# guxm2021/SVT_SpeechBrain

Hardware: AMD Instinct MI355X
Metric: 10s@16kHz clips/sec encoder+CTC forward, wav2vec2-base, 1/2/4/8 MI355X (higher is better)
Workload: dtype bf16; 1 GPU; wav2vec2-base audio-only AMT forward (encoder + 20-way head + frame decode), 32 x 10 s @16 kHz mono clips per GPU; global_batch=32, per_gpu_batch=32, samples_per_clip=160000, frames_per_clip=499, parallelism=clips sharded over 1 rank(s), streams=2, inputs=resident in HBM

## Files before the change

include/svt_mi355.h:

```cpp
#ifndef SVT_MI355_H
#define SVT_MI355_H

#include <stddef.h>
#include <stdint.h>

#ifdef __cplusplus
extern "C" {
#endif

#define SVT_ABI_VERSION 1
#define SVT_MAX_CONV_LAYERS 8

typedef enum {
  SVT_OK = 0,
  SVT_ERR_INVALID = -1,
  SVT_ERR_KEY = -2,
  SVT_ERR_STATE = -3,
  SVT_ERR_WORKSPACE = -4,
  SVT_ERR_HIP = -5,
  SVT_ERR_NO_DEVICE = -6
} svt_status;

typedef enum { SVT_PREC_FP32 = 0, SVT_PREC_BF16 = 1, SVT_PREC_BF16X3 = 2, SVT_PREC_FP16X3 = 3 } svt_precision;
typedef enum { SVT_NORM_GROUP = 0, SVT_NORM_LAYER = 1 } svt_feat_norm;
// ... 12 lines not shown
  int32_t feat_extract_norm;
  int32_t conv_bias;
  int32_t stable_layer_norm;
  int32_t feat_proj_layer_norm;
  int32_t pos_conv_kernel;
  int32_t pos_conv_groups;
  float layer_norm_eps;
  int32_t normalize_wav;
  int32_t output_norm;
  int32_t precision;
  int32_t pos_conv_depth;
  int32_t rel_pos_buckets;
  int32_t rel_pos_max_distance;
  int32_t pos_conv_batch_norm;
} svt_encoder_config;

typedef struct svt_encoder svt_encoder;
typedef struct svt_linear svt_linear;
typedef struct svt_rca svt_rca;

typedef struct svt_frame {
  float p_on;
  float p_off;
  int32_t octave;
  int32_t pitch_class;
} svt_frame;

const char* svt_last_error(void);
int svt_abi_version(void);
int svt_operand_type(void);
int svt_device_count(void);

int svt_encoder_create(const svt_encoder_config* cfg, int device, svt_encoder** out);
void svt_encoder_destroy(svt_encoder* e);

typedef int (*svt_norm_reduce_fn)(double* sums_dev, int32_t n_doubles, void* stream, void* user);
int svt_encoder_set_norm_reduce(svt_encoder* enc, svt_norm_reduce_fn fn, void* user, int64_t global_clips);
int svt_encoder_load_param(svt_encoder* e, const char* key, const void* data_host, int dtype,
                           const int64_t* shape, int ndim);
int svt_encoder_finalize(svt_encoder* e);
int svt_encoder_get_param(svt_encoder* e, const char* key, void* out_host, int64_t capacity_elems);
int64_t svt_encoder_num_frames(const svt_encoder* e, int64_t n_samples);
int64_t svt_encoder_workspace_bytes(const svt_encoder* e, int32_t batch, int64_t n_samples);
int svt_encoder_forward(svt_encoder* e, const float* wav_dev, int32_t batch, int64_t n_samples,
                        float* feats_dev, void* workspace_dev, size_t workspace_bytes, void* stream);
int svt_encoder_forward_ex(svt_encoder* e, const float* wav_dev, int32_t batch, int64_t n_samples,
                           float* feats_dev, void* workspace_dev, size_t workspace_bytes, void* stream,
                           int32_t clips_per_norm_group);

int svt_encoder_forward_head(svt_encoder* enc, const svt_linear* head, const float* wav_dev, int32_t batch,
                             int64_t n_samples, float* logits_out_dev, svt_frame* frames_out_dev, int32_t n_octave,
                             int32_t n_class, void* workspace_dev, size_t workspace_bytes, void* stream,
                             int32_t clips_per_norm_group);

int svt_linear_create(int32_t in_features, int32_t out_features, int has_bias, int device, svt_linear** out);
void svt_linear_destroy(svt_linear* l);
int svt_linear_load(svt_linear* l, const float* weight_host , const float* bias_host );
int svt_linear_forward(svt_linear* l, const float* x_dev, int64_t rows, float* y_dev, void* stream);
int svt_decode_frames(const float* logits_dev, int64_t rows, int32_t n_out, int32_t n_octave,
                      int32_t n_class, svt_frame* frames_dev, int device, void* stream);
int svt_frames_to_notes(const svt_frame* frames_host, int32_t batch, int64_t frames_per_clip, const int64_t* n_frames,
                        float onset_thres, float offset_thres, double frame_size, int32_t n_octave, int32_t n_class,
                        double* t_on, double* t_off, int32_t* pitch, int32_t* lo, int32_t* hi, int64_t capacity_per_clip,
                        int64_t* n_notes);

int svt_rca_create(int32_t d_model, int32_t nhead, int32_t d_ffn, float alpha, int32_t max_len,
                   int32_t precision, int device, svt_rca** out);
void svt_rca_destroy(svt_rca* r);
int svt_rca_load_param(svt_rca* r, const char* key, const void* data_host, int dtype,
                       const int64_t* shape, int ndim);
int svt_rca_finalize(svt_rca* r);
int64_t svt_rca_workspace_bytes(const svt_rca* r, int32_t batch, int32_t t_audio);
int svt_rca_forward(svt_rca* r, const float* audio_dev, int32_t t_audio, const float* video_dev,
                    int32_t t_video, int32_t batch, float* out_dev, void* workspace_dev,
                    size_t workspace_bytes, void* stream);
int svt_rca_refresh_params(svt_rca* r, const float* const* params_dev, int32_t n, void* stream);
int64_t svt_rca_train_workspace_bytes(const svt_rca* r, int32_t batch, int32_t t_audio);
int svt_rca_forward_train(svt_rca* r, const float* audio_dev, int32_t t_audio, const float* video_dev, int32_t t_video, int32_t batch,
                          float* out_dev, void* workspace_dev, size_t workspace_bytes, void* stream);
int svt_rca_backward(svt_rca* r, const float* dout_dev, int32_t batch, int32_t t_audio, float* const* grads_dev, void* workspace_dev,
                     size_t workspace_bytes, void* stream);

int svt_ctc_greedy(const float* probs_dev, int32_t batch, int32_t t, int32_t v, const float* rel_lens_dev,
                   int32_t blank, int32_t* tokens_dev, int32_t* out_lens_dev, int device, void* stream);

int64_t svt_fbank_workspace_bytes(int32_t batch, int64_t n_samples, int32_t n_fft, int32_t hop, int32_t n_mels);
int svt_fbank(const float* wav_dev, int32_t batch, int64_t n_samples, int32_t sample_rate, int32_t n_fft,
              int32_t win_length, int32_t hop_length, int32_t n_mels, float f_min, float f_max, float top_db,
              float* out_dev, void* workspace_dev, size_t workspace_bytes, int device, void* stream);

int svt_debug_gemm(int32_t precision, const void* a_dev, const void* w_dev, void* c_dev, const float* bias_dev,
                   const float* resid_dev, int32_t m, int32_t n, int32_t k, int32_t a_rpb, int64_t a_bstride,
                   int64_t a_rstride, int64_t ldw, int32_t act, int32_t out_f32, int device, void* stream);

int svt_debug_gemm_pairs(int32_t precision, const float* a_dev, int64_t a_elems, const float* w_dev, float* c_dev, const float* bias_dev,
                         int32_t m, int32_t n, int32_t k, int32_t a_rpb, int64_t a_bstride, int64_t a_rstride, int32_t act,
                         int32_t out_kind, int device, void* stream, int32_t time_iters, float* ms_out);

typedef struct svt_video svt_video;
int svt_video_create(int32_t embed_dim, int32_t precision, int device, svt_video** out);
void svt_video_destroy(svt_video* v);
int svt_video_load_param(svt_video* v, const char* key, const void* data_host, int dtype, const int64_t* shape, int ndim);
int svt_video_finalize(svt_video* v);
int64_t svt_video_workspace_bytes(const svt_video* v, int32_t batch, int32_t t, int32_t h, int32_t w);
int svt_video_keep_workspace(svt_video* v, int keep);
int svt_video_forward(svt_video* v, const float* video_dev, int32_t batch, int32_t t, int32_t h, int32_t w, float* out_dev,
                      void* workspace_dev, size_t workspace_bytes, void* stream);
int svt_video_forward_ex(svt_video* v, const float* video_dev, int32_t batch, int32_t t, int32_t h, int32_t w, float* out_dev, int64_t out_ld,
                         int32_t zero_left, void* workspace_dev, size_t workspace_bytes, void* stream);
typedef struct svt_video_transform { double sub0, div0, mean, std; int32_t crop_h, crop_w; } svt_video_transform;
int svt_video_forward_u8(svt_video* v, const uint8_t* roi_dev, int32_t batch, int32_t t, int32_t h_in, int32_t w_in,
                         const svt_video_transform* tf, float* out_dev, int64_t out_ld, int32_t zero_left, void* workspace_dev,
                         size_t workspace_bytes, void* stream);

int svt_deltas(const float* x_dev, int64_t ldx, int32_t batch, int32_t t, int32_t c, int32_t window_length, float* out_dev,
               int64_t ldo, int device, void* stream);
int svt_context_window(const float* x_dev, int32_t batch, int32_t t, int32_t c, int32_t left_frames, int32_t right_frames,
                       float* out_dev, int device, void* stream);

int svt_bce_loss(const float* logits_dev, int64_t batch, int64_t t_pred, const float* targets_dev, int64_t t_tgt,
                 const float* rel_len_dev, const float* pos_weight_dev, int32_t allowed_len_diff, int32_t reduction,
                 float* out_dev, void* workspace_dev, size_t workspace_bytes, int device, void* stream);
int svt_nll_loss(const float* log_probs_dev, int64_t batch, int64_t t_pred, int32_t n_class, const int64_t* targets_dev,
                 int64_t t_tgt, const float* rel_len_dev, float label_smoothing, int32_t allowed_len_diff,
                 int32_t reduction, float* out_dev, void* workspace_dev, size_t workspace_bytes, int device, void* stream);
int svt_softmax(const float* x_dev, int64_t rows, int32_t n, int32_t apply_log, float* y_dev, int device, void* stream);

int svt_amt_objective_grad(const float* logits_dev, int64_t batch, int64_t t_pred, int32_t n_out, int32_t pitch_octave_num,
                           const float* onset_targets_dev, const float* offset_targets_dev, const int64_t* octave_targets_dev,
                           const int64_t* class_targets_dev, int64_t t_tgt, const float* rel_len_dev, float onset_pos_weight,
                           int32_t allowed_len_diff, float label_smoothing, float* terms_dev, float* terms_host, float* dlogits_dev,
                           void* workspace_dev, size_t* workspace_bytes, int device, void* stream);
int svt_linear_backward(const float* x_dev, const float* dy_dev, int64_t rows, int32_t in_features, int32_t out_features,
                        float* dweight_dev, float* dbias_dev, void* workspace_dev, size_t* workspace_bytes, int device, void* stream);
int svt_linear_backward_data(const float* dy_dev, const float* weight_dev, int64_t rows, int32_t in_features, int32_t out_features,
                             float* dx_dev, int device, void* stream);
int svt_clip_adadelta_step(int32_t n_tensors, float* const* params_dev, float* const* grads_dev, float* const* square_avg_dev,
                           float* const* acc_delta_dev, const int64_t* numels, float lr, double rho, float eps, float weight_decay,
                           int32_t maximize, float max_norm, float* total_norm_dev, void* workspace_dev, size_t* workspace_bytes,
                           int device, void* stream);

int svt_debug_attention(int32_t precision, const void* q, const void* k, const void* v, void* o, int32_t batch, int32_t t,
                        int32_t heads, int32_t head_dim, int64_t ldq, int64_t ldkv, int64_t ldo, float scale, int device,
                        void* stream);
int svt_debug_attention_bias(const void* q, const void* k, const void* v, void* o, int32_t batch, int32_t t, int32_t heads, int64_t ldq,
                             int64_t ldkv, int64_t ldo, float scale, const float* gate_dev, const float* pos_bias_dev, int device,
                             void* stream);
int svt_debug_rca_wgrad(int32_t precision, const float* dy0, int64_t ldy0, const void* x0, const float* dy1, int64_t ldy1, const void* x1,
                        int64_t rows, int32_t n_out, int32_t n_in, float* dw, float* db, void* workspace_dev, size_t* workspace_bytes,
                        int device, void* stream);
int svt_debug_rca_attn_bwd(int32_t precision, const void* qkv, const void* qc, const void* o_self, const void* o_cross,
                           const float* dblend, float alpha, int32_t batch, int32_t t, int32_t heads, int32_t head_dim, float* dqkv,
                           float* dqc, void* workspace_dev, size_t* workspace_bytes, int device, void* stream);
int svt_debug_set(int key, int value);

int svt_prof_enable(int on);
int svt_prof_reset(void);
int svt_prof_read(int kind, int64_t* launches, double* total_ms, double* total_flops, double* total_bytes);
int svt_debug_clock(int64_t* out_dev, int device, void* stream);
int svt_debug_alloc(void** out, size_t bytes, int device);
int svt_debug_encoder_layout(const svt_encoder* e, int32_t batch, int64_t n_samples, int64_t* offsets, int n);
int svt_debug_free(void* p, int device);

#ifdef __cplusplus
}
#endif
#endif
```

svt_speechbrain_amd/_lib.py:

```python
from __future__ import annotations

import ctypes as C
import os
from typing import Optional

_HERE = os.path.dirname(os.path.abspath(__file__))
LIB_PATH = os.environ.get("SVT_LIB_PATH") or os.path.join(_HERE, "libsvt_mi355.so")
MAX_CONV = 8


class SvtError(RuntimeError):
    pass


class EncoderConfigC(C.Structure):
    _fields_ = [
        ("struct_size", C.c_int32),
        ("hidden_size", C.c_int32),
        ("num_layers", C.c_int32),
        ("num_heads", C.c_int32),
        ("intermediate_size", C.c_int32),
        ("num_conv_layers", C.c_int32),
        ("conv_dim", C.c_int32 * MAX_CONV),
        ("conv_kernel", C.c_int32 * MAX_CONV),
        ("conv_stride", C.c_int32 * MAX_CONV),
        ("feat_extract_norm", C.c_int32),
        ("conv_bias", C.c_int32),
        ("stable_layer_norm", C.c_int32),
        ("feat_proj_layer_norm", C.c_int32),
        ("pos_conv_kernel", C.c_int32),
        ("pos_conv_groups", C.c_int32),
        ("layer_norm_eps", C.c_float),
        ("normalize_wav", C.c_int32),
        ("output_norm", C.c_int32),
        ("precision", C.c_int32),
        ("pos_conv_depth", C.c_int32),
        ("rel_pos_buckets", C.c_int32),
        ("rel_pos_max_distance", C.c_int32),
        ("pos_conv_batch_norm", C.c_int32),
    ]


class VideoTransformC(C.Structure):
    _fields_ = [("sub0", C.c_double), ("div0", C.c_double), ("mean", C.c_double), ("std", C.c_double), ("crop_h", C.c_int32), ("crop_w", C.c_int32)]


class FrameC(C.Structure):
    _fields_ = [("p_on", C.c_float), ("p_off", C.c_float), ("octave", C.c_int32), ("pitch_class", C.c_int32)]


_P = C.c_void_p
_I64P = C.POINTER(C.c_int64)
NORM_REDUCE_FN = C.CFUNCTYPE(C.c_int, C.c_void_p, C.c_int32, C.c_void_p, C.c_void_p)

SYMBOLS = {
    "svt_last_error": (C.c_char_p, []),
    "svt_abi_version": (C.c_int, []),
    "svt_device_count": (C.c_int, []),
    "svt_encoder_create": (C.c_int, [C.POINTER(EncoderConfigC), C.c_int, C.POINTER(_P)]),
    "svt_encoder_destroy": (None, [_P]),
    "svt_encoder_load_param": (C.c_int, [_P, C.c_char_p, _P, C.c_int, _I64P, C.c_int]),
    "svt_encoder_finalize": (C.c_int, [_P]),
    "svt_encoder_get_param": (C.c_int, [_P, C.c_char_p, _P, C.c_int64]),
    "svt_encoder_num_frames": (C.c_int64, [_P, C.c_int64]),
    "svt_encoder_workspace_bytes": (C.c_int64, [_P, C.c_int32, C.c_int64]),
    "svt_encoder_forward": (C.c_int, [_P, _P, C.c_int32, C.c_int64, _P, _P, C.c_size_t, _P]),
    "svt_encoder_forward_ex": (C.c_int, [_P, _P, C.c_int32, C.c_int64, _P, _P, C.c_size_t, _P, C.c_int32]),
    "svt_encoder_forward_head": (C.c_int, [_P, _P, _P, C.c_int32, C.c_int64, _P, _P, C.c_int32, C.c_int32, _P, C.c_size_t, _P, C.c_int32]),
    "svt_linear_create": (C.c_int, [C.c_int32, C.c_int32, C.c_int, C.c_int, C.POINTER(_P)]),
    "svt_linear_destroy": (None, [_P]),
    "svt_linear_load": (C.c_int, [_P, _P, _P]),
    "svt_linear_forward": (C.c_int, [_P, _P, C.c_int64, _P, _P]),
    "svt_decode_frames": (C.c_int, [_P, C.c_int64, C.c_int32, C.c_int32, C.c_int32, _P, C.c_int, _P]),
    "svt_rca_create": (C.c_int, [C.c_int32, C.c_int32, C.c_int32, C.c_float, C.c_int32, C.c_int32, C.c_int, C.POINTER(_P)]),
    "svt_rca_destroy": (None, [_P]),
    "svt_rca_load_param": (C.c_int, [_P, C.c_char_p, _P, C.c_int, _I64P, C.c_int]),
    "svt_rca_finalize": (C.c_int, [_P]),
    "svt_rca_workspace_bytes": (C.c_int64, [_P, C.c_int32, C.c_int32]),
    "svt_rca_forward": (C.c_int, [_P, _P, C.c_int32, _P, C.c_int32, C.c_int32, _P, _P, C.c_size_t, _P]),
    "svt_rca_refresh_params": (C.c_int, [_P, C.POINTER(_P), C.c_int32, _P]),
    "svt_rca_train_workspace_bytes": (C.c_int64, [_P, C.c_int32, C.c_int32]),
    "svt_rca_forward_train": (C.c_int, [_P, _P, C.c_int32, _P, C.c_int32, C.c_int32, _P, _P, C.c_size_t, _P]),
    "svt_rca_backward": (C.c_int, [_P, _P, C.c_int32, C.c_int32, C.POINTER(_P), _P, C.c_size_t, _P]),
    "svt_ctc_greedy": (C.c_int, [_P, C.c_int32, C.c_int32, C.c_int32, _P, C.c_int32, _P, _P, C.c_int, _P]),
    "svt_fbank_workspace_bytes": (C.c_int64, [C.c_int32, C.c_int64, C.c_int32, C.c_int32, C.c_int32]),
    "svt_fbank": (C.c_int, [_P, C.c_int32, C.c_int64, C.c_int32, C.c_int32, C.c_int32, C.c_int32, C.c_int32,
                            C.c_float, C.c_float, C.c_float, _P, _P, C.c_size_t, C.c_int, _P]),
    "svt_debug_gemm": (C.c_int, [C.c_int32, _P, _P, _P, _P, _P, C.c_int32, C.c_int32, C.c_int32, C.c_int32, C.c_int64,
                                 C.c_int64, C.c_int64, C.c_int32, C.c_int32, C.c_int, _P]),
    "svt_debug_gemm_pairs": (C.c_int, [C.c_int32, _P, C.c_int64, _P, _P, _P, C.c_int32, C.c_int32, C.c_int32, C.c_int32, C.c_int64,
                                       C.c_int64, C.c_int32, C.c_int32, C.c_int, _P, C.c_int32, C.POINTER(C.c_float)]),
    "svt_video_create": (C.c_int, [C.c_int32, C.c_int32, C.c_int, C.POINTER(C.c_void_p)]),
    "svt_video_destroy": (None, [C.c_void_p]),
    "svt_video_load_param": (C.c_int, [C.c_void_p, C.c_char_p, C.c_void_p, C.c_int, C.POINTER(C.c_int64), C.c_int]),
    "svt_video_finalize": (C.c_int, [C.c_void_p]),
    "svt_video_keep_workspace": (C.c_int, [C.c_void_p, C.c_int]),
    "svt_video_workspace_bytes": (C.c_int64, [C.c_void_p, C.c_int32, C.c_int32, C.c_int32, C.c_int32]),
    "svt_video_forward": (C.c_int, [C.c_void_p, C.c_void_p, C.c_int32, C.c_int32, C.c_int32, C.c_int32, C.c_void_p, C.c_void_p,
                                    C.c_size_t, C.c_void_p]),
    "svt_video_forward_ex": (C.c_int, [C.c_void_p, C.c_void_p, C.c_int32, C.c_int32, C.c_int32, C.c_int32, C.c_void_p, C.c_int64, C.c_int32,
                                       C.c_void_p, C.c_size_t, C.c_void_p]),
    "svt_video_forward_u8": (C.c_int, [C.c_void_p, C.c_void_p, C.c_int32, C.c_int32, C.c_int32, C.c_int32, C.POINTER(VideoTransformC),
                                       C.c_void_p, C.c_int64, C.c_int32, C.c_void_p, C.c_size_t, C.c_void_p]),
    "svt_deltas": (C.c_int, [C.c_void_p, C.c_int64, C.c_int32, C.c_int32, C.c_int32, C.c_int32, C.c_void_p, C.c_int64, C.c_int, C.c_void_p]),
    "svt_context_window": (C.c_int, [C.c_void_p, C.c_int32, C.c_int32, C.c_int32, C.c_int32, C.c_int32, C.c_void_p, C.c_int, C.c_void_p]),
    "svt_bce_loss": (C.c_int, [C.c_void_p, C.c_int64, C.c_int64, C.c_void_p, C.c_int64, C.c_void_p, C.c_void_p, C.c_int32,
                               C.c_int32, C.c_void_p, C.c_void_p, C.c_size_t, C.c_int, C.c_void_p]),
    "svt_nll_loss": (C.c_int, [C.c_void_p, C.c_int64, C.c_int64, C.c_int32, C.c_void_p, C.c_int64, C.c_void_p, C.c_float,
                               C.c_int32, C.c_int32, C.c_void_p, C.c_void_p, C.c_size_t, C.c_int, C.c_void_p]),
    "svt_softmax": (C.c_int, [C.c_void_p, C.c_int64, C.c_int32, C.c_int32, C.c_void_p, C.c_int, C.c_void_p]),
    "svt_amt_objective_grad": (C.c_int, [_P, C.c_int64, C.c_int64, C.c_int32, C.c_int32, _P, _P, _P, _P, C.c_int64, _P, C.c_float,
                                         C.c_int32, C.c_float, _P, C.POINTER(C.c_float), _P, _P, C.POINTER(C.c_size_t), C.c_int, _P]),
    "svt_linear_backward": (C.c_int, [_P, _P, C.c_int64, C.c_int32, C.c_int32, _P, _P, _P, C.POINTER(C.c_size_t), C.c_int, _P]),
    "svt_linear_backward_data": (C.c_int, [_P, _P, C.c_int64, C.c_int32, C.c_int32, _P, C.c_int, _P]),
    "svt_clip_adadelta_step": (C.c_int, [C.c_int32, C.POINTER(_P), C.POINTER(_P), C.POINTER(_P), C.POINTER(_P), _I64P, C.c_float,
                                         C.c_double, C.c_float, C.c_float, C.c_int32, C.c_float, _P, _P, C.POINTER(C.c_size_t), C.c_int,
                                         _P]),
    "svt_debug_attention": (C.c_int, [C.c_int32, C.c_void_p, C.c_void_p, C.c_void_p, C.c_void_p, C.c_int32, C.c_int32,
                                      C.c_int32, C.c_int32, C.c_int64, C.c_int64, C.c_int64, C.c_float, C.c_int, C.c_void_p]),
    "svt_debug_attention_bias": (C.c_int, [C.c_void_p, C.c_void_p, C.c_void_p, C.c_void_p, C.c_int32, C.c_int32, C.c_int32, C.c_int64,
                                           C.c_int64, C.c_int64, C.c_float, C.c_void_p, C.c_void_p, C.c_int, C.c_void_p]),
    "svt_debug_rca_wgrad": (C.c_int, [C.c_int32, _P, C.c_int64, _P, _P, C.c_int64, _P, C.c_int64, C.c_int32, C.c_int32, _P, _P, _P,
                                      C.POINTER(C.c_size_t), C.c_int, _P]),
    "svt_debug_rca_attn_bwd": (C.c_int, [C.c_int32, _P, _P, _P, _P, _P, C.c_float, C.c_int32, C.c_int32, C.c_int32, C.c_int32, _P, _P,
                                         _P, C.POINTER(C.c_size_t), C.c_int, _P]),
    "svt_debug_set": (C.c_int, [C.c_int, C.c_int]),
    "svt_debug_clock": (C.c_int, [C.c_void_p, C.c_int, C.c_void_p]),
    "svt_debug_encoder_layout": (C.c_int, [C.c_void_p, C.c_int32, C.c_int64, C.POINTER(C.c_int64), C.c_int]),
    "svt_operand_type": (C.c_int, []),
    "svt_encoder_set_norm_reduce": (C.c_int, [_P, C.c_void_p, C.c_void_p, C.c_int64]),
    "svt_frames_to_notes": (C.c_int, [C.c_void_p, C.c_int32, C.c_int64, C.c_void_p, C.c_float, C.c_float, C.c_double, C.c_int32, C.c_int32,
                                      C.c_void_p, C.c_void_p, C.c_void_p, C.c_void_p, C.c_void_p, C.c_int64, C.c_void_p]),
    "svt_debug_alloc": (C.c_int, [C.POINTER(C.c_void_p), C.c_size_t, C.c_int]),
    "svt_debug_free": (C.c_int, [C.c_void_p, C.c_int]),
    "svt_prof_enable": (C.c_int, [C.c_int]),
    "svt_prof_reset": (C.c_int, []),
    "svt_prof_read": (C.c_int, [C.c_int, _I64P, C.POINTER(C.c_double), C.POINTER(C.c_double), C.POINTER(C.c_double)]),
}

_lib: Optional[C.CDLL] = None
_libs: dict = {}


def load(variant: str = None) -> C.CDLL:
    global _lib
    key = variant or ""
    if key in _libs:
        return _libs[key]
    if not variant and os.environ.get("SVT_LIB_SUFFIX"):
        variant_path = LIB_PATH.replace("libsvt_mi355.so", f"libsvt_mi355_{os.environ['SVT_LIB_SUFFIX']}.so")
        if not os.path.exists(variant_path):
            raise SvtError(f"SVT_LIB_SUFFIX: {variant_path} not found")
        globals()["LIB_PATH"] = variant_path
    root, ext = os.path.splitext(LIB_PATH)
    path = LIB_PATH if not variant else f"{root}_{variant}{ext}"
    if not os.path.exists(path):
        raise SvtError(
            f"{path} not found: build it with `python -c 'import __graft_entry__ as g; g.build()'` "
            "(or `make -C svt_speechbrain_amd/csrc`). The MI355X path has no CPU fallback.")
    lib = C.CDLL(path)
    for name, (res, args) in SYMBOLS.items():
        fn = getattr(lib, name)
        fn.restype = res
        fn.argtypes = args
    if lib.svt_abi_version() != 1:
        raise SvtError(f"{os.path.basename(path)} ABI version mismatch")
    if lib.svt_operand_type() != (1 if variant == "f16" else 0):
        raise SvtError(f"{os.path.basename(path)} was built for another operand type")
    _libs[key] = lib
    if not variant:
        _lib = lib
    return lib


def last_error(lib: C.CDLL = None) -> str:
    return ((lib or load()).svt_last_error() or b"").decode("utf-8", "replace")


def check(rc: int, what: str = "", lib: C.CDLL = None) -> None:
    if rc != 0:
        raise SvtError(f"{what}: {last_error(lib)} (status {rc})")


def require_gpu() -> None:
    lib = load()
    if lib.svt_device_count() < 1:
        raise SvtError("no gfx950 (MI355X) device is visible: the HIP path cannot run and there is no CPU fallback")


def stream_ptr(device) -> int:
    import torch
    return int(torch.cuda.current_stream(device).cuda_stream)


def dev_index(device) -> int:
    import torch
    d = torch.device(device)
    if d.type != "cuda":
        raise SvtError(f"tensors must live on a ROCm device ('cuda:N'), got {d}")
    return d.index if d.index is not None else torch.cuda.current_device()


def ptr(t) -> int:
    return int(t.data_ptr())
```

svt_speechbrain_amd/csrc/api.hip:

```cpp
#include "../../include/svt_mi355.h"
#include "api.h"
#include "common.h"
#include "host.h"

#include <atomic>
#include <cmath>
#include <cstring>
#include <map>
#include <mutex>
#include <string>
#include <vector>

namespace svt {

int hip_fail(hipError_t e, const char* what, const char* file, int line) {
  set_error(std::string("HIP error ") + hipGetErrorName(e) + " (" + hipGetErrorString(e) + ") at " + file + ":" +
          std::to_string(line) + " in " + what);
  return SVT_ERR_HIP;
}

struct ProfState {
  bool on = false;
  int every = 1;
  unsigned tick = 0;
// ... 227 lines not shown
    set_error(std::string(who) + ": workspace too small (need " + std::to_string(need) + " bytes)");
    return SVT_ERR_WORKSPACE;
  }
  return SVT_OK;
}

int g_debug_keep_split = 0;

}

using namespace svt;

extern "C" {

int svt_abi_version(void) { return SVT_ABI_VERSION; }
int svt_operand_type(void) {
#ifdef SVT_OPERAND_F16
  return 1;
#else
  return 0;
#endif
}
int svt_device_count(void) {
  int n = 0;
  if (hipGetDeviceCount(&n) != hipSuccess) return 0;
  int ok = 0;
  for (int i = 0; i < n; ++i) {
    hipDeviceProp_t prop;
    if (hipGetDeviceProperties(&prop, i) == hipSuccess && std::string(prop.gcnArchName).find("gfx950") != std::string::npos) ++ok;
  }
  return ok;
}

int svt_debug_gemm(int32_t precision, const void* a, const void* w, void* c, const float* bias, const float* resid,
                   int32_t m, int32_t n, int32_t k, int32_t a_rpb, int64_t a_bstride, int64_t a_rstride, int64_t ldw,
                   int32_t act, int32_t out_f32, int device, void* stream) {
  if (!a || !w || !c) { set_error("svt_debug_gemm: null argument"); return SVT_ERR_INVALID; }
  SVT_HIP(hipSetDevice(device));
  GemmArgs g;
  g.A = a; g.W = w; g.C = c; g.bias = bias; g.resid = resid;
  g.M = m; g.N = n; g.K = k; g.a_rpb = a_rpb; g.a_bstride = a_bstride; g.a_rstride = a_rstride;
  g.ldw = ldw; g.ldc = n; g.act = act; g.out_f32 = out_f32;
  static const void* s_kept = nullptr;
  const bool split = precision >= 2 && ldw == k && k % 32 == 0;
  if (split && !(g_debug_keep_split && s_kept == w)) {
    if (split_weights_register(w, n, k, precision, (hipStream_t)stream)) return SVT_ERR_HIP;
    s_kept = w;
  }
  const int rc = launch_gemm(precision, g, (hipStream_t)stream);
  if (split && !g_debug_keep_split) {
    SVT_HIP(hipStreamSynchronize((hipStream_t)stream));
    split_weights_forget(w);
    s_kept = nullptr;
  }
  return rc ? SVT_ERR_INVALID : SVT_OK;
}

int svt_debug_gemm_pairs(int32_t precision, const float* a, int64_t a_elems, const float* w, float* c, const float* bias, int32_t m,
                         int32_t n, int32_t k, int32_t a_rpb, int64_t a_bstride, int64_t a_rstride, int32_t act, int32_t out_kind,
                         int device, void* stream, int32_t time_iters, float* ms_out) {
  if (!a || !w || !c) { set_error("svt_debug_gemm_pairs: null argument"); return SVT_ERR_INVALID; }
  if ((precision != SVT_PREC_BF16X3 && precision != SVT_PREC_FP16X3) || !valid_precision(precision)) {
    set_error("svt_debug_gemm_pairs: split-operand precisions only (they live in libsvt_mi355.so, not in the IEEE-half build)"); return SVT_ERR_INVALID; }
  if (out_kind < 0 || out_kind > 2 || a_elems % 32 || ((int64_t)m * n) % 32) { set_error("svt_debug_gemm_pairs: out_kind / sizes"); return SVT_ERR_INVALID; }
  SVT_HIP(hipSetDevice(device));
  hipStream_t s = (hipStream_t)stream;
  void *ap = nullptr, *cp = nullptr;
  hipEvent_t e0 = nullptr, e1 = nullptr;
  static std::mutex s_mu;
  static const void* s_kept = nullptr;
  std::lock_guard<std::mutex> lock(s_mu);
  bool registered = false;
  auto hip_ok = [](hipError_t e, const char* what) -> int {
    if (e == hipSuccess) return 0;
    set_error(std::string(what) + ": " + hipGetErrorString(e));
    return 1;
  };
  int rc = dev_alloc(&ap, (size_t)a_elems * 4);
  if (!rc && out_kind) rc = dev_alloc(&cp, (size_t)m * n * 4);
  if (!rc) rc = launch_f32_to_pairs(precision, a, ap, a_elems, s);
  if (!rc && !(g_debug_keep_split && s_kept == w)) {
    rc = split_weights_register(w, n, k, precision, s);
    if (!rc) { s_kept = w; registered = true; }
  } else if (!rc) {
    registered = true;
  }
  if (!rc) {
    GemmArgs g;
    g.A = ap; g.W = w; g.C = out_kind == 1 ? cp : (void*)c; g.bias = bias;
    g.M = m; g.N = n; g.K = k; g.a_rpb = a_rpb; g.a_bstride = a_bstride; g.a_rstride = a_rstride;
    g.ldw = k; g.ldc = n; g.act = act; g.out_f32 = 1; g.a_pairs = 1; g.c_pairs = out_kind == 1;
    if (out_kind == 2) { g.planes = (unsigned short*)cp; g.plane_stride = (long)m * n; }
    rc = launch_gemm(precision, g, s);
    if (!rc && time_iters > 0 && ms_out) {
      rc = hip_ok(hipEventCreate(&e0), "hipEventCreate") || hip_ok(hipEventCreate(&e1), "hipEventCreate") ||
           hip_ok(hipEventRecord(e0, s), "hipEventRecord");
      for (int i = 0; i < time_iters && !rc; ++i) rc = launch_gemm(precision, g, s);
      float ms = 0.f;
      if (!rc) rc = hip_ok(hipEventRecord(e1, s), "hipEventRecord") || hip_ok(hipEventSynchronize(e1), "hipEventSynchronize") ||
                    hip_ok(hipEventElapsedTime(&ms, e0, e1), "hipEventElapsedTime");
      if (!rc) *ms_out = ms / (float)time_iters;
    }
  }
  if (!rc && out_kind == 1) rc = launch_pairs_to_f32(precision, cp, nullptr, c, (int64_t)m * n, s);
  if (!rc && out_kind == 2) rc = launch_pairs_to_f32(precision, cp, (const unsigned short*)cp + (size_t)m * n, c, (int64_t)m * n, s);
  (void)hipStreamSynchronize(s);
  if (e0) (void)hipEventDestroy(e0);
  if (e1) (void)hipEventDestroy(e1);
  if (registered && !g_debug_keep_split) { split_weights_forget(w); s_kept = nullptr; }
  if (ap) dev_free(ap);
  if (cp) dev_free(cp);
  return rc ? SVT_ERR_INVALID : SVT_OK;
}

int svt_debug_attention(int32_t precision, const void* q, const void* k, const void* v, void* o, int32_t batch, int32_t t,
                        int32_t heads, int32_t head_dim, int64_t ldq, int64_t ldkv, int64_t ldo, float scale, int device,
                        void* stream) {
  if (!q || !k || !v || !o) { set_error("svt_debug_attention: null argument"); return SVT_ERR_INVALID; }
  if (!(precision >= 1 && precision <= 3) || !(head_dim == 64 || head_dim == 128)) {
    set_error("svt_debug_attention: only the fused kernels (bf16, or the split-operand modes on fp32 inputs; head_dim 64 / 128) are exposed"); return SVT_ERR_INVALID; }
  if (int r = check_device(device)) return r;
  SVT_HIP(hipSetDevice(device));
  if (precision >= 2) {
    const long D = (long)heads * head_dim, rows = (long)batch * t;
    if ((const float*)k != (const float*)q + D || (const float*)v != (const float*)q + 2 * D || ldq != 3 * D || ldkv != 3 * D) {
      set_error("svt_debug_attention: the split-operand kernel is exposed for a packed q|k|v projection"); return SVT_ERR_INVALID; }
    void* planes = nullptr;
    if (int r = dev_alloc(&planes, (size_t)rows * 3 * D * 4)) return r;
    AttnBufs ab{};
    ab.pl_qkv = planes;
    const int rc = attention_scores_path(0, q, ldq, k, v, ldkv, batch, t, heads, head_dim, scale, ab, false, o, ldo, (hipStream_t)stream,
                                         nullptr, nullptr, precision);
    (void)hipStreamSynchronize((hipStream_t)stream);
    dev_free(planes);
    return rc ? SVT_ERR_INVALID : SVT_OK;
  }
  if (launch_flash_attention(q, ldq, (long)t * ldq, k, v, ldkv, (long)t * ldkv, o, ldo, (long)t * ldo, batch, t, heads,
                             head_dim, scale, (hipStream_t)stream)) return SVT_ERR_INVALID;
  return SVT_OK;
}

int svt_debug_attention_bias(const void* q, const void* k, const void* v, void* o, int32_t batch, int32_t t, int32_t heads, int64_t ldq,
                             int64_t ldkv, int64_t ldo, float scale, const float* gate_dev, const float* pos_bias_dev, int device,
                             void* stream) {
  if (!q || !k || !v || !o || !gate_dev || !pos_bias_dev) { set_error("svt_debug_attention_bias: null argument"); return SVT_ERR_INVALID; }
  if (batch < 1 || t < 1 || heads < 1) { set_error("svt_debug_attention_bias: batch, t and heads must be positive"); return SVT_ERR_INVALID; }
  if (int r = check_device(device)) return r;
  SVT_HIP(hipSetDevice(device));
  if (launch_flash_attention(q, ldq, (long)t * ldq, k, v, ldkv, (long)t * ldkv, o, ldo, (long)t * ldo, batch, t, heads, 64, scale,
                             (hipStream_t)stream, gate_dev, pos_bias_dev)) return SVT_ERR_INVALID;
  return SVT_OK;
}

int svt_debug_set(int key, int value) {
  if (key == 0) g_gemm_dbg = value;
  else if (key == 1) g_gemm_force_bm = value;
  else if (key == 2) g_gemm_ring = value;
  else if (key == 3) g_gemm_variant = value;
  else if (key == 5) {  }
  else if (key == 6) g_gemm_skinny = value;
  else if (key == 7) g_gemm_skinny_max_tiles = value;
  else if (key == 8) g_flash_wide = value;
  else if (key == 9) g_conv_ln_bf16 = value;
  else if (key == 10) {  }
  else if (key == 11) g_gemm_x3 = value;
  else if (key == 12) g_debug_keep_split = value;
  else if (key == 13) g_guard_alloc = value;
  else if (key == 15) g_stamp_ends = value;
  else if (key == 16) {  }
  else if (key == 18) {  }
  else if (key == 19) g_x3_pairs = value;
  else if (key == 20) g_ln_two_rows = value;
  else if (key == 21) {
    if (value != 0 && value != 3) { set_error("svt_debug_set(21): the attention A/B arms are retired"); return SVT_ERR_INVALID; }
  }
  else if (key == 22) g_conv0_mfma = value;
  else if (key == 23) g_conv3x3_c64 = value;
  else if (key == 24) return g_conv3x3_c64_launches;
  else if (key == 25) g_conv3x3_c64_form = value;
  else if (key == 26) g_stem_pool_fused = value;
  else if (key == 27) g_conv_down_fused = value;
  else if (key == 28) {
    if (value != 0) { set_error("svt_debug_set(28): the two-slot schedule is retired"); return SVT_ERR_INVALID; }
  }
  else if (key == 29) g_gemm_p1w = value;
  else if (key == 30) {
#ifndef SVT_DIAG
    if (value != 0) { set_error("svt_debug_set(30): gemm_p1x_kernel is built by `make DIAG=1` only"); return SVT_ERR_INVALID; }
#endif
    g_gemm_p1x = value;
  }
  else if (key == 31) return g_dev_frees.load(std::memory_order_relaxed);
  else if (key == 32) return set_ticket_fenced(value);
  else if (key == 33) g_gemm_skinny_small_tiles = value;
  else if (key == 34) g_gemm_walk = value;
  else if (key == 35) g_conv_kperm = value;
  else if (key == 36) g_ffn2_ksplit = value;
  else if (key == 37) { if (value < 8 || value > 256 || value % 8) { set_error("svt_debug_set(37): 8 .. 256, a multiple of 8"); return SVT_ERR_INVALID; } g_gemm_persist_wgs = value; }
  else if (key == 38) return g_flash_kernel_id;
  else if (key == 39) return g_gemm_kernel_id;
  else { set_error("svt_debug_set: unknown key"); return SVT_ERR_INVALID; }
  return SVT_OK;
}

int svt_debug_alloc(void** out, size_t bytes, int device) {
  if (!out) { set_error("svt_debug_alloc: null argument"); return SVT_ERR_INVALID; }
  if (int r = check_device(device)) return r;
  SVT_HIP(hipSetDevice(device));
  return dev_alloc(out, bytes);
}
int svt_debug_free(void* p, int device) {
  if (int r = check_device(device)) return r;
  SVT_HIP(hipSetDevice(device));
  dev_free(p);
  return SVT_OK;
}

int svt_debug_clock(int64_t* out_dev, int device, void* stream) {
  if (!out_dev) { set_error("svt_debug_clock: null argument"); return SVT_ERR_INVALID; }
  SVT_HIP(hipSetDevice(device));
  return launch_clock_stamp((long long*)out_dev, (hipStream_t)stream) ? SVT_ERR_HIP : SVT_OK;
}

int svt_prof_enable(int on) { g_prof.on = on != 0; g_prof.every = on > 1 ? on : 1; g_prof.tick = 0; return SVT_OK; }
int svt_prof_reset(void) {
  g_prof.used = 0;
  for (int k = 0; k < 3; ++k) g_prof.flops[k] = g_prof.bytes[k] = 0;
  return SVT_OK;
}
int svt_prof_read(int kind, int64_t* launches, double* total_ms, double* total_flops, double* total_bytes) {
  if (kind < 0 || kind > 2) { set_error("svt_prof_read: kind must be 0..2"); return SVT_ERR_INVALID; }
  double ms = 0;
  int64_t n = 0;
  for (size_t i = 0; i < g_prof.used; ++i) {
    if (g_prof.kind[i] != kind) continue;
    SVT_HIP(hipEventSynchronize(g_prof.ev[i].second));
    float t = 0;
    SVT_HIP(hipEventElapsedTime(&t, g_prof.ev[i].first, g_prof.ev[i].second));
    ms += t;
    ++n;
  }
  if (launches) *launches = n;
  if (total_ms) *total_ms = ms;
  if (total_flops) *total_flops = g_prof.flops[kind];
  if (total_bytes) *total_bytes = g_prof.bytes[kind];
  return SVT_OK;
}

}
```

svt_speechbrain_amd/csrc/api_encoder.hip:

```cpp
#include "../../include/svt_mi355.h"
#include "api.h"
#include "common.h"
#include "host.h"

#include <cmath>
#include <cstring>
#include <string>
#include <vector>

using namespace svt;

int svt::g_conv_ln_bf16 = 1;

struct ConvLayerW {
  DevBuf w;
  DevBuf w_kperm;
  DevBuf bias;
  DevBuf gamma, beta;
};
struct EncLayerW {
  DevBuf wqkv, bqkv, wo, bo, ln1g, ln1b, w1, b1, w2, b2, ln2g, ln2b;
  DevBuf g_wab, g_bab, g_const;
};

// ... 379 lines not shown
  const svt_linear* head = nullptr;
  float* logits = nullptr;
  svt_frame* frames = nullptr;
  int n_oct = 0, n_cls = 0;
};

}

extern "C" {

int svt_debug_encoder_layout(const svt_encoder* e, int32_t batch, int64_t n_samples, int64_t* offsets, int n) {
  if (!e || batch < 1 || !offsets || n < 1) { set_error("svt_debug_encoder_layout: bad argument"); return SVT_ERR_INVALID; }
  if (svt_encoder_num_frames(e, n_samples) < 1) { set_error("waveform shorter than the receptive field"); return SVT_ERR_INVALID; }
  char* const fake = (char*)(uintptr_t)(1ull << 40);
  const EncWs w = carve_encoder(e, batch, n_samples, fake);
  const void* r[24] = {w.mom, w.coef, w.c0tab, w.act[0], w.act[1], w.convF, w.xln, w.hF, w.preF, w.xb, w.xF, w.xlo, w.posg, w.posy, w.qkv,
                       w.ab.S, w.ab.P, w.ab.Vt, w.ab.pl_qkv, w.attn_o, w.ffn, w.gate, w.relpb, w.dots};
  int k = 0;
  for (; k < 24 && k < n; ++k) offsets[k] = r[k] == nullptr ? -1 : (int64_t)((const char*)r[k] - fake);
  if (k < n) offsets[k++] = (int64_t)w.total;
  return k;
}

int64_t svt_encoder_workspace_bytes(const svt_encoder* e, int32_t batch, int64_t n_samples) {
  if (!e || batch < 1) { set_error("workspace_bytes: bad argument"); return -1; }
  if (svt_encoder_num_frames(e, n_samples) < 1) { set_error("waveform shorter than the receptive field"); return -1; }
  return (int64_t)carve_encoder(e, batch, n_samples, nullptr).total;
}

}

static int encoder_forward_impl(svt_encoder* e, const float* wav, int32_t B, int64_t L, const TailSpec& tail, void* workspace,
                                size_t workspace_bytes, void* stream, int32_t clips_per_norm_group);

extern "C" {

int svt_encoder_forward(svt_encoder* e, const float* wav, int32_t B, int64_t L, float* feats, void* workspace,
                        size_t workspace_bytes, void* stream) {
  return svt_encoder_forward_ex(e, wav, B, L, feats, workspace, workspace_bytes, stream, 0);
}

int svt_encoder_forward_ex(svt_encoder* e, const float* wav, int32_t B, int64_t L, float* feats, void* workspace,
                           size_t workspace_bytes, void* stream, int32_t clips_per_norm_group) {
  if (!feats) { set_error("encoder_forward: null argument"); return SVT_ERR_INVALID; }
  TailSpec t;
  t.feats = feats;
  return encoder_forward_impl(e, wav, B, L, t, workspace, workspace_bytes, stream, clips_per_norm_group);
}

int svt_encoder_forward_head(svt_encoder* e, const svt_linear* head, const float* wav, int32_t B, int64_t L, float* logits,
                             svt_frame* frames, int32_t n_octave, int32_t n_class, void* workspace, size_t workspace_bytes,
                             void* stream, int32_t clips_per_norm_group) {
  if (!head || !logits) { set_error("encoder_forward_head: null argument"); return SVT_ERR_INVALID; }
  if (!head->loaded) { set_error("encoder_forward_head: head weights not loaded"); return SVT_ERR_STATE; }
  if (!e || head->in_f != e->cfg.hidden_size || head->device != e->device) {
    set_error("encoder_forward_head: the head must take hidden_size inputs and live on the encoder's device"); return SVT_ERR_INVALID; }
  if (!linear_head_eligible(head->in_f, head->out_f)) {
    set_error("encoder_forward_head: the fused tail is built for hidden sizes 512 / 768 / 1024 and at most 32 outputs"); return SVT_ERR_INVALID; }
  if (frames && head->out_f != 2 + n_octave + 1 + n_class + 1) {
    set_error("encoder_forward_head: n_out != 2 + (n_octave+1) + (n_class+1)"); return SVT_ERR_INVALID; }
  TailSpec t;
  t.head = head; t.logits = logits; t.frames = frames; t.n_oct = n_octave; t.n_cls = n_class;
  return encoder_forward_impl(e, wav, B, L, t, workspace, workspace_bytes, stream, clips_per_norm_group);
}

}

static int encoder_forward_impl(svt_encoder* e, const float* wav, int32_t B, int64_t L, const TailSpec& tail, void* workspace,
                                size_t workspace_bytes, void* stream, int32_t clips_per_norm_group) {
  float* feats = tail.feats;
  if (!e || !wav || !workspace) { set_error("encoder_forward: null argument"); return SVT_ERR_INVALID; }
  if (!e->finalized) { set_error("encoder_forward: parameters not finalized"); return SVT_ERR_STATE; }
  if (B < 1) { set_error("encoder_forward: batch < 1"); return SVT_ERR_INVALID; }
  const int64_t T = svt_encoder_num_frames(e, L);
  if (T < 1) { set_error("encoder_forward: waveform shorter than the receptive field"); return SVT_ERR_INVALID; }
  const svt_encoder_config& c = e->cfg;
  const int prec = storage_prec(c.precision);
  const int gp = c.precision;
  EncWs w = carve_encoder(e, B, L, workspace);
  if (w.total > workspace_bytes) { set_error("encoder_forward: workspace too small (" + std::to_string(workspace_bytes) + " < " + std::to_string(w.total) + ")"); return SVT_ERR_WORKSPACE; }
  hipStream_t s = (hipStream_t)stream;
  SVT_HIP(hipSetDevice(e->device));
  const int cpg = clips_per_norm_group > 0 ? clips_per_norm_group : B;
  if (B % cpg) { set_error("encoder_forward: batch must be a multiple of clips_per_norm_group"); return SVT_ERR_INVALID; }
  const int groups = B / cpg;
  if (groups > 1 && c.num_conv_layers > 0 && (L & 3)) {
    set_error("encoder_forward: norm groups need a waveform length that is a multiple of 4 samples");
    return SVT_ERR_INVALID;
  }
  if (groups > 1 && c.num_conv_layers == 0 && c.normalize_wav) {
    set_error("encoder_forward: features-in mode has no input norm to group");
    return SVT_ERR_INVALID;
  }
  if (launch_zero_bytes(w.mom, w.mom_zero, s)) return SVT_ERR_HIP;
  double* wav_mom = c.normalize_wav ? w.mom : nullptr;
  double* out_mom = w.mom + 2 * (size_t)B;
  double* wm = w.mom + 4 * (size_t)B;
  int64_t n_wav = (int64_t)cpg * L;
  if (c.normalize_wav)
    if (int r = launch_moments(wav, n_wav, wav_mom, (char*)w.mom + w.mom_scr[0], B, s, groups)) return r;
  struct ReduceCtx { svt_encoder* e; double* mom; hipStream_t s; } rctx{e, nullptr, s};
  auto reduce_now = [](void* a) -> int {
    ReduceCtx* rc = (ReduceCtx*)a;
    if (rc->e->reduce_fn(rc->mom, 2, (void*)rc->s, rc->e->reduce_user)) { set_error("encoder_forward: the norm-reduce callback reported an error"); return SVT_ERR_INVALID; }
    return 0;
  };
  const bool global_norm = e->reduce_fn != nullptr;
  if (global_norm) {
    if (groups != 1) { set_error("encoder_forward: the cross-rank norm reduction applies to whole-batch norms (clips_per_norm_group = 0)"); return SVT_ERR_INVALID; }
    if (e->reduce_global_clips < B) { set_error("encoder_forward: global_clips of the norm reduction is smaller than this batch"); return SVT_ERR_INVALID; }
    if (c.normalize_wav) {
      rctx.mom = wav_mom;
      if (int r = reduce_now(&rctx)) return r;
      n_wav = e->reduce_global_clips * L;
    }
  }

  const int pk_mode = (gp >= 2 && g_x3_pairs && g_gemm_x3) ? gp : 0;
  auto x3q_fits = [&](const void* A, int M, int N, int K, int a_rpb, long a_bstride, long a_rstride, const void* Wp, int c_pairs, long ldc) -> bool {
    GemmArgs g;
    g.A = A; g.W = Wp; g.C = const_cast<void*>(A); g.M = M; g.N = N; g.K = K; g.a_rpb = a_rpb; g.a_bstride = a_bstride; g.a_rstride = a_rstride;
    g.ldw = K; g.ldc = ldc; g.a_pairs = 1; g.c_pairs = c_pairs;
    return gemm_x3q_eligible(g);
  };
  bool pk_front_ok = pk_mode != 0 && c.num_conv_layers >= 2 && c.conv_dim[0] % 32 == 0 && c.conv_dim[0] <= 512 && c.conv_stride[0] <= 5;
  if (pk_front_ok) {
    int64_t ti_ = (L - c.conv_kernel[0]) / c.conv_stride[0] + 1;
    for (int i = 1; i < c.num_conv_layers && pk_front_ok; ++i) {
      const int cin = c.conv_dim[i - 1], co = c.conv_dim[i], k = c.conv_kernel[i], st = c.conv_stride[i];
      const int64_t to_ = (ti_ - k) / st + 1;
      if ((int64_t)B * to_ > 2147483647LL) { pk_front_ok = false; break; }
      pk_front_ok = x3q_fits(w.act[0], (int)((int64_t)B * to_), co, k * cin, (int)to_, ti_ * cin, (long)st * cin, e->conv[i].w.p, 1, co) &&
                    (c.feat_extract_norm != SVT_NORM_LAYER || co == 512 || co == 768 || co == 1024);
      ti_ = to_;
    }
    const int Cl = c.conv_dim[c.num_conv_layers - 1];
    const int64_t rows_ = (int64_t)B * T;
    pk_front_ok = pk_front_ok && x3q_fits(w.xln, (int)rows_, c.hidden_size, Cl, (int)rows_, 0, Cl, e->proj_w.p, 0, c.hidden_size) &&
                  (!c.feat_proj_layer_norm || Cl == 512 || Cl == 768 || Cl == 1024);
  }
  const int pk_front = pk_front_ok ? pk_mode : 0;

  int64_t tin = L;
  int cur = 0;
  if (c.num_conv_layers == 0) {
    const int64_t n = (int64_t)B * L * c.conv_dim[0];
    if (prec) { if (int r = launch_f32_to_bf16(wav, (bf16_t*)w.act[0], n, s)) return r; }
    else if (launch_copy_f32(wav, (float*)w.act[0], n, s)) return SVT_ERR_HIP;
  } else {
  int64_t t1 = (L - c.conv_kernel[0]) / c.conv_stride[0] + 1;
  const ConvLayerW& c0 = e->conv[0];
  if (c.feat_extract_norm == SVT_NORM_GROUP) {
    if (int r = launch_conv0_window_moments(wav, B, L, c.conv_kernel[0], c.conv_stride[0], t1, wm, (char*)w.mom + w.mom_scr[2], s)) return r;
    if (int r = launch_conv0_group_coef(wav_mom, n_wav, wm, B, t1, c.conv_dim[0], c.conv_kernel[0], c0.w.as<float>(),
                                        c.conv_bias ? c0.bias.as<float>() : nullptr, c0.gamma.as<float>(),
                                        c0.beta.as<float>(), 1e-5f, 1e-5f, w.coef, s, cpg)) return r;
    if (conv0_mfma_ok(prec, pk_front, c.conv_kernel[0], c.conv_stride[0], c.conv_dim[0]) && w.c0tab) {
      if (int r = launch_conv0_mfma_group(wav, B, L, c.conv_stride[0], t1, w.coef, w.c0tab, w.act[0], s, pk_front)) return r;
    } else
    if (int r = launch_conv0_group_apply(prec, wav, B, L, c.conv_kernel[0], c.conv_stride[0], t1, c.conv_dim[0], w.coef,
                                         w.act[0], s, pk_front)) return r;
  } else {
    if (conv0_mfma_ok(prec, pk_front, c.conv_kernel[0], c.conv_stride[0], c.conv_dim[0]) && w.c0tab) {
      if (int r = launch_conv0_mfma_layer(wav, B, L, c.conv_stride[0], t1, wav_mom, n_wav, 1e-5f, c0.w.as<float>(),
                                          c.conv_bias ? c0.bias.as<float>() : nullptr, c0.gamma.as<float>(), c0.beta.as<float>(), 1e-5f,
                                          w.c0tab, w.act[0], s, cpg, pk_front)) return r;
    } else
    if (int r = launch_conv0_layer(prec, wav, B, L, c.conv_kernel[0], c.conv_stride[0], t1, c.conv_dim[0], wav_mom, n_wav,
                                   1e-5f, c0.w.as<float>(), c.conv_bias ? c0.bias.as<float>() : nullptr,
                                   c0.gamma.as<float>(), c0.beta.as<float>(), 1e-5f, w.act[0], s, cpg, pk_front)) return r;
  }
  tin = t1;
  }
  for (int i = 1; i < c.num_conv_layers; ++i) {
    const int cin = c.conv_dim[i - 1], co = c.conv_dim[i], k = c.conv_kernel[i], st = c.conv_stride[i];
    const int64_t tout = (tin - k) / st + 1;
    const ConvLayerW& Lw = e->conv[i];
    GemmArgs g;
    g.A = w.act[cur]; g.W = Lw.w.p;
    g.M = (int)((int64_t)B * tout); g.N = co; g.K = k * cin;
    g.a_rpb = (int)tout; g.a_bstride = tin * cin; g.a_rstride = (long)st * cin;
    g.ldw = g.K; g.ldc = co;
    if (Lw.w_kperm.p) { g.W_kperm = Lw.w_kperm.p; g.kperm_taps = k; g.kperm_cin = cin; }
    g.bias = c.conv_bias ? Lw.bias.as<float>() : nullptr;
    if ((int64_t)B * tout > 2147483647LL) { set_error("encoder_forward: batch*frames exceeds 2^31"); return SVT_ERR_INVALID; }
    g.a_pairs = pk_front ? 1 : 0;
    const bool pairs_out = pk_front && !(i + 1 == c.num_conv_layers && c.feat_proj_layer_norm);
    if (pk_front && c.feat_extract_norm == SVT_NORM_LAYER) {
      g.C = w.convF; g.out_f32 = 1; g.act = ACT_NONE;
      if (int r = launch_gemm(gp, g, s)) return r;
      if (int r = launch_layernorm(prec, w.convF, 1, (int64_t)B * tout, co, Lw.gamma.as<float>(), Lw.beta.as<float>(), 1e-5f, 1,
                                   pairs_out ? nullptr : w.act[cur ^ 1], nullptr, s, nullptr, nullptr, pairs_out ? w.act[cur ^ 1] : nullptr,
                                   pk_front)) return r;
    } else if (pk_front) {
      g.C = w.act[cur ^ 1]; g.act = ACT_GELU; g.out_f32 = 1; g.c_pairs = pairs_out ? 1 : 0;
      if (int r = launch_gemm(gp, g, s)) return r;
    } else
    if (c.feat_extract_norm == SVT_NORM_LAYER && prec && co == 512 && g_conv_ln_bf16) {
      g.C = w.act[cur ^ 1]; g.out_f32 = 0; g.act = ACT_NONE;
      if (int r = launch_gemm(gp, g, s)) return r;
      if (int r = launch_layernorm(prec, w.act[cur ^ 1], 0, (int64_t)B * tout, co, Lw.gamma.as<float>(), Lw.beta.as<float>(),
                                   1e-5f, 1, w.act[cur ^ 1], nullptr, s)) return r;
    } else if (c.feat_extract_norm == SVT_NORM_LAYER) {
      g.C = w.convF; g.out_f32 = 1; g.act = ACT_NONE;
      if (int r = launch_gemm(gp, g, s)) return r;
      if (int r = launch_layernorm(prec, w.convF, 1, (int64_t)B * tout, co, Lw.gamma.as<float>(), Lw.beta.as<float>(),
                                   1e-5f, 1, w.act[cur ^ 1], nullptr, s)) return r;
    } else {
      g.C = w.act[cur ^ 1]; g.act = ACT_GELU;
      if (int r = launch_gemm(gp, g, s)) return r;
    }
    cur ^= 1;
    tin = tout;
  }
  const int C = c.conv_dim[c.num_conv_layers > 0 ? c.num_conv_layers - 1 : 0];
  const int D = c.hidden_size, F = c.intermediate_size, H = c.num_heads, dh = D / H;
  const int64_t rows = (int64_t)B * T;
  const float eps = c.layer_norm_eps;

  const void* proj_in = w.act[cur];
  if (c.feat_proj_layer_norm) {
    if (int r = launch_layernorm(prec, w.act[cur], prec ? 0 : 1, rows, C, e->fp_g.as<float>(), e->fp_b.as<float>(), eps, 0,
                                 pk_front ? nullptr : w.xln, nullptr, s, nullptr, nullptr, pk_front ? w.xln : nullptr, pk_front)) return r;
    proj_in = w.xln;
  }
  {
    GemmArgs g;
    g.A = proj_in; g.W = e->proj_w.p; g.C = w.hF; g.bias = e->proj_b.as<float>();
    g.M = (int)rows; g.N = D; g.K = C; g.a_rpb = (int)rows; g.a_rstride = C; g.ldw = C; g.ldc = D; g.out_f32 = 1;
    g.a_pairs = pk_front ? 1 : 0;
    if (int r = launch_gemm(gp, g, s)) return r;
  }
  {
    const int kp = c.pos_conv_kernel, G = c.pos_conv_groups, cg = D / G;
    const int Pf = e->pos_P;
    const float* bn_sc = c.pos_conv_batch_norm ? e->pos_bn_sc.as<float>() : nullptr;
    const float* bn_sh = c.pos_conv_batch_norm ? e->pos_bn_sh.as<float>() : nullptr;
    if (c.pos_conv_depth > 1) {
      const float* cur = w.hF;
      float* lnout = w.xF;
      for (int i = 0; i < c.pos_conv_depth; ++i) {
        if (int r = launch_posconv_gather(prec, cur, B, (int)T, D, G, kp, (int)T + kp, w.posg, s)) return r;
        GemmArgs g;
        g.A = w.posg; g.W = e->pos_ws[i].p; g.C = w.preF; g.bias = e->pos_bs[i].as<float>();
        g.M = (int)T; g.N = cg; g.K = kp * cg;
        g.a_rpb = (int)T; g.a_rstride = cg;
        g.ldw = g.K; g.ldc = D;
        g.nz = B * G; g.nz2 = G;
        g.a_z1 = (long)G * (T + kp) * cg; g.a_z2 = (long)(T + kp) * cg;
        g.w_z1 = 0; g.w_z2 = (long)cg * g.K;
        g.c_z1 = (long)T * D; g.c_z2 = cg; g.bias_z2 = cg;
        g.act = ACT_NONE; g.out_f32 = 1;
        if (int r = launch_gemm(gp, g, s)) return r;
        if (int r = launch_layernorm(prec, w.preF, 1, rows, D, e->ones.as<float>(), e->zeros.as<float>(), 1e-5f, 1, nullptr,
                                     lnout, s)) return r;
        cur = lnout;
      }
      if (int r = launch_add_f32(w.hF, cur, w.preF, rows * (int64_t)D, s)) return r;
    } else if (Pf && (int64_t)B * ((T + Pf - 1) / Pf) >= 128) {
      const int Tq = (int)((T + Pf - 1) / Pf), Tp = Tq * Pf + kp;
      if (int r = launch_posconv_gather(prec, w.hF, B, (int)T, D, G, kp, Tp, w.posg, s, bn_sc, bn_sh)) return r;
      GemmArgs g;
      g.A = w.posg; g.W = e->pos_wP.p; g.C = w.posy; g.bias = e->pos_bP.as<float>();
      g.M = B * Tq; g.N = Pf * cg; g.K = (kp + Pf - 1) * cg;
      g.a_rpb = Tq; g.a_bstride = (long)G * Tp * cg; g.a_rstride = (long)Pf * cg;
      g.ldw = g.K; g.ldc = g.N;
      g.nz = G; g.nz2 = G;
      g.a_z2 = (long)Tp * cg; g.w_z2 = (long)g.N * g.K; g.c_z2 = (long)B * Tq * g.N; g.bias_z2 = g.N;
      g.act = ACT_GELU; g.out_f32 = 0;
      if (int r = launch_gemm(gp, g, s)) return r;
      if (int r = launch_posconv_scatter_add(w.hF, w.posy, B, (int)T, D, G, Pf, Tq, w.preF, s, prec ? 0 : 1)) return r;
    } else {
    if (int r = launch_posconv_gather(prec, w.hF, B, (int)T, D, G, kp, (int)T + kp, w.posg, s, bn_sc, bn_sh)) return r;
    GemmArgs g;
    g.A = w.posg; g.W = e->pos_w.p; g.C = w.preF; g.bias = e->pos_b.as<float>(); g.resid = w.hF;
    g.M = (int)T; g.N = cg; g.K = kp * cg;
    g.a_rpb = (int)T; g.a_rstride = cg;
    g.ldw = g.K; g.ldc = D;
    g.nz = B * G; g.nz2 = G;
    g.a_z1 = (long)G * (T + kp) * cg; g.a_z2 = (long)(T + kp) * cg;
    g.w_z1 = 0; g.w_z2 = (long)cg * g.K;
    g.c_z1 = (long)T * D; g.c_z2 = cg; g.bias_z2 = cg;
    g.act = ACT_GELU; g.out_f32 = 1;
    if (int r = launch_gemm(gp, g, s)) return r;
    }
  }
  const float scale = 1.0f / std::sqrt((float)dh);
  if (c.rel_pos_buckets)
    if (int r = launch_relpos_table(e->rel_embed.as<float>(), H, (int)T, c.rel_pos_buckets, c.rel_pos_max_distance, w.relpb, s)) return r;
  const bool qkv_planes = gp >= 2 && !c.rel_pos_buckets && flash_attention_x3_ok(dh) && w.ab.pl_qkv != nullptr;
  unsigned short* const qkv_pl = qkv_planes ? (unsigned short*)w.ab.pl_qkv : nullptr;
  const bool pk_enc_ok = pk_mode != 0 && qkv_planes && c.num_layers > 0 && (D == 512 || D == 768 || D == 1024) && dh % 32 == 0 &&
                         x3q_fits(w.xb, (int)rows, 3 * D, D, (int)rows, 0, D, e->layers[0].wqkv.p, 0, 3 * D) &&
                         x3q_fits(w.attn_o, (int)rows, D, D, (int)rows, 0, D, e->layers[0].wo.p, 0, D) &&
                         x3q_fits(w.xb, (int)rows, F, D, (int)rows, 0, D, e->layers[0].w1.p, 1, F) &&
                         x3q_fits(w.ffn, (int)rows, D, F, (int)rows, 0, F, e->layers[0].w2.p, 0, D);
  const int pk_enc = pk_enc_ok ? pk_mode : 0;
  if (!prec && !pk_enc) w.xF = (float*)w.xb;
  int cur_layer = 0;
  auto attention = [&](void) -> int {
    const float* gate = nullptr;
    if (c.rel_pos_buckets) {
      const EncLayerW& Lg = e->layers[cur_layer];
      if (int r = launch_relpos_gate(prec, w.xb, rows, (int)T, H, dh, Lg.g_wab.as<float>(), Lg.g_bab.as<float>(),
                                     Lg.g_const.as<float>(), w.gate, s)) return r;
      gate = w.gate;
    }
    ++cur_layer;
    return attention_scores_path(prec, w.qkv, 3L * D, (const char*)w.qkv + (size_t)D * esize(prec),
                                 (const char*)w.qkv + (size_t)2 * D * esize(prec), 3L * D, B, (int)T, H, dh, scale, w.ab,
                                 qkv_planes, w.attn_o, D, s, gate, w.relpb, gp, pk_enc ? 1 : 0);
  };
  auto gemm_rows = [&](const void* A, int K, const DevBuf& W, const DevBuf& bias, int N, void* Cout, int out_f32, int act,
                       const float* resid, unsigned short* planes = nullptr, int c_pairs = 0) -> int {
    GemmArgs g;
    g.A = A; g.W = W.p; g.C = Cout; g.bias = bias.as<float>(); g.resid = resid;
    g.M = (int)rows; g.N = N; g.K = K; g.a_rpb = (int)rows; g.a_rstride = K; g.ldw = K; g.ldc = N;
    g.out_f32 = out_f32; g.act = act;
    g.planes = planes; g.plane_stride = (long)rows * N;
    g.a_pairs = pk_enc ? 1 : 0; g.c_pairs = c_pairs;
    return launch_gemm(gp, g, s);
  };

  float* final_x = nullptr;
  float* tmp = w.hF;
  const bool vecD = (D == 512 || D == 768 || D == 1024);
  const int tmp_f32 = (prec && vecD) ? 0 : 1;
  if (!c.stable_layer_norm && prec && layernorm_hilo_ok(D) && c.num_layers > 0) {
    bf16_t* xh = (bf16_t*)w.xb;
    bf16_t* xl = (bf16_t*)w.xlo;
    if (int r = launch_layernorm_hilo(nullptr, nullptr, nullptr, w.preF, rows, D, e->enc_g.as<float>(), e->enc_b.as<float>(), eps,
                                      xh, xl, nullptr, s)) return r;
    bool ffn2_split = false;
    if (g_ffn2_ksplit && w.ksplit && gp == 1 && F % 256 == 0 && F >= 2048 && g_ln_two_rows) {
      GemmArgs g;
      g.A = w.ffn; g.W = e->layers[0].w2.p; g.C = tmp; g.M = (int)rows; g.N = D; g.K = F; g.a_rpb = (int)rows; g.a_rstride = F; g.ldw = F; g.ldc = D;
      ffn2_split = g_gemm_skinny && gemm_skinny_eligible(g) && (long)((rows + 31) / 32) * (D / 32) <= 256;
    }
    for (int l = 0; l < c.num_layers; ++l) {
      const EncLayerW& Lw = e->layers[l];
      const bool last = l + 1 == c.num_layers;
      if (int r = gemm_rows(w.xb, D, Lw.wqkv, Lw.bqkv, 3 * D, w.qkv, 0, ACT_NONE, nullptr, qkv_pl)) return r;
      if (int r = attention()) return r;
      if (int r = gemm_rows(w.attn_o, D, Lw.wo, Lw.bo, D, tmp, 0, ACT_NONE, nullptr)) return r;
      if (int r = launch_layernorm_hilo((const bf16_t*)tmp, xh, xl, nullptr, rows, D, Lw.ln1g.as<float>(), Lw.ln1b.as<float>(), eps,
                                        xh, xl, nullptr, s)) return r;
      if (int r = gemm_rows(w.xb, D, Lw.w1, Lw.b1, F, w.ffn, 0, ACT_GELU, nullptr)) return r;
      if (ffn2_split) {
        GemmArgs g;
        g.A = w.ffn; g.W = Lw.w2.p; g.C = w.ksplit; g.M = (int)rows; g.N = D; g.K = F; g.a_rpb = (int)rows; g.a_rstride = F; g.ldw = F; g.ldc = D;
        g.out_f32 = 1; g.ksplit = 4; g.ksplit_stride = (long)rows * D;
        if (int r = launch_gemm_skinny(g, s)) return r;
        if (int r = launch_layernorm_hilo_parts(w.ksplit, 4, (long)rows * D, Lw.b2.as<float>(), xh, xl, rows, D, Lw.ln2g.as<float>(), Lw.ln2b.as<float>(),
                                                eps, xh, xl, last ? w.xF : nullptr, s)) return r;
        continue;
      }
      if (int r = gemm_rows(w.ffn, F, Lw.w2, Lw.b2, D, tmp, 0, ACT_NONE, nullptr)) return r;
      if (int r = launch_layernorm_hilo((const bf16_t*)tmp, xh, xl, nullptr, rows, D, Lw.ln2g.as<float>(), Lw.ln2b.as<float>(), eps,
                                        xh, xl, last ? w.xF : nullptr, s)) return r;
    }
    final_x = w.xF;
  } else if (!c.stable_layer_norm && pk_enc) {
    const bool pair_resid = pk_enc == 3;
    float* const keepF = pair_resid ? nullptr : w.xF;
    if (int r = launch_layernorm(prec, w.preF, 1, rows, D, e->enc_g.as<float>(), e->enc_b.as<float>(), eps, 0, nullptr, keepF, s, nullptr,
                                 nullptr, w.xb, pk_enc)) return r;
    auto ln_resid = [&](const float* g_, const float* b_, bool want_f32) -> int {
      if (pair_resid)
        return launch_layernorm(prec, tmp, 1, rows, D, g_, b_, eps, 0, nullptr, want_f32 ? w.xF : nullptr, s, nullptr, nullptr, w.xb,
                                pk_enc, w.xb);
      return launch_layernorm(prec, tmp, 1, rows, D, g_, b_, eps, 0, nullptr, w.xF, s, w.xF, nullptr, w.xb, pk_enc, nullptr);
    };
    for (int l = 0; l < c.num_layers; ++l) {
      const EncLayerW& Lw = e->layers[l];
      const bool last = l + 1 == c.num_layers;
      if (int r = gemm_rows(w.xb, D, Lw.wqkv, Lw.bqkv, 3 * D, w.qkv, 0, ACT_NONE, nullptr, qkv_pl)) return r;
      if (int r = attention()) return r;
      if (int r = gemm_rows(w.attn_o, D, Lw.wo, Lw.bo, D, tmp, 1, ACT_NONE, nullptr)) return r;
      if (int r = ln_resid(Lw.ln1g.as<float>(), Lw.ln1b.as<float>(), false)) return r;
      if (int r = gemm_rows(w.xb, D, Lw.w1, Lw.b1, F, w.ffn, 1, ACT_GELU, nullptr, nullptr, 1)) return r;
      if (int r = gemm_rows(w.ffn, F, Lw.w2, Lw.b2, D, tmp, 1, ACT_NONE, nullptr)) return r;
      if (int r = ln_resid(Lw.ln2g.as<float>(), Lw.ln2b.as<float>(), last)) return r;
    }
    final_x = w.xF;
  } else if (!c.stable_layer_norm) {
    if (int r = launch_layernorm(prec, w.preF, 1, rows, D, e->enc_g.as<float>(), e->enc_b.as<float>(), eps, 0, w.xb,
                                 prec ? w.xF : nullptr, s)) return r;
    for (int l = 0; l < c.num_layers; ++l) {
      const EncLayerW& Lw = e->layers[l];
      if (int r = gemm_rows(w.xb, D, Lw.wqkv, Lw.bqkv, 3 * D, w.qkv, 0, ACT_NONE, nullptr, qkv_pl)) return r;
      if (int r = attention()) return r;
      if (int r = gemm_rows(w.attn_o, D, Lw.wo, Lw.bo, D, tmp, tmp_f32, ACT_NONE, nullptr)) return r;
      if (int r = launch_layernorm(prec, tmp, tmp_f32, rows, D, Lw.ln1g.as<float>(), Lw.ln1b.as<float>(), eps, 0, w.xb,
                                   prec ? w.xF : nullptr, s, w.xF)) return r;
      if (int r = gemm_rows(w.xb, D, Lw.w1, Lw.b1, F, w.ffn, 0, ACT_GELU, nullptr)) return r;
      if (int r = gemm_rows(w.ffn, F, Lw.w2, Lw.b2, D, tmp, tmp_f32, ACT_NONE, nullptr)) return r;
      if (int r = launch_layernorm(prec, tmp, tmp_f32, rows, D, Lw.ln2g.as<float>(), Lw.ln2b.as<float>(), eps, 0, w.xb,
                                   prec ? w.xF : nullptr, s, w.xF)) return r;
    }
    final_x = w.xF;
  } else {
    float* h = w.preF;
    const void* pending = nullptr;
    auto ln_add = [&](const float* g_, const float* b_, const void* branch, void* y_op, float* y_f32) -> int {
      if (pk_enc && y_op)
        return launch_layernorm(prec, h, 1, rows, D, g_, b_, eps, 0, nullptr, nullptr, s, (const float*)branch, branch ? h : nullptr, y_op, pk_enc);
      if (!branch) return launch_layernorm(prec, h, 1, rows, D, g_, b_, eps, 0, y_op, y_f32, s, nullptr, nullptr);
      if (!tmp_f32)
        return launch_layernorm(prec, branch, 0, rows, D, g_, b_, eps, 0, y_op, y_f32, s, h, y_op ? h : nullptr);
      return launch_layernorm(y_op ? prec : 0, h, 1, rows, D, g_, b_, eps, 0, y_op ? y_op : (void*)y_f32, nullptr, s,
                              (const float*)branch, y_op ? h : nullptr);
    };
    for (int l = 0; l < c.num_layers; ++l) {
      const EncLayerW& Lw = e->layers[l];
      if (int r = ln_add(Lw.ln1g.as<float>(), Lw.ln1b.as<float>(), pending, w.xb, nullptr)) return r;
      if (int r = gemm_rows(w.xb, D, Lw.wqkv, Lw.bqkv, 3 * D, w.qkv, 0, ACT_NONE, nullptr, qkv_pl)) return r;
      if (int r = attention()) return r;
      if (int r = gemm_rows(w.attn_o, D, Lw.wo, Lw.bo, D, tmp, tmp_f32, ACT_NONE, nullptr)) return r;
      if (int r = ln_add(Lw.ln2g.as<float>(), Lw.ln2b.as<float>(), tmp, w.xb, nullptr)) return r;
      if (int r = gemm_rows(w.xb, D, Lw.w1, Lw.b1, F, w.ffn, 0, ACT_GELU, nullptr, nullptr, pk_enc ? 1 : 0)) return r;
      if (int r = gemm_rows(w.ffn, F, Lw.w2, Lw.b2, D, tmp, tmp_f32, ACT_NONE, nullptr)) return r;
      pending = tmp;
    }
    float* fin = (float*)w.qkv;
    if (int r = ln_add(e->enc_g.as<float>(), e->enc_b.as<float>(), pending, nullptr, fin)) return r;
    final_x = fin;
  }
  const int64_t n_out = rows * D;
  const double n_out_stat = global_norm ? (double)e->reduce_global_clips * (double)(rows / B) * (double)D : 0.0;
  rctx.mom = out_mom;
  if (tail.head) {
    static_assert(sizeof(svt_frame) == sizeof(FrameOut), "frame layout");
    if (launch_head_fused(final_x, rows, D, tail.head->w.as<float>(), tail.head->wsum.as<float>(),
                          tail.head->has_bias ? tail.head->b.as<float>() : nullptr, tail.head->out_f, w.dots,
                          c.output_norm ? out_mom : nullptr, rows / groups, 1e-5f, tail.logits, (FrameOut*)tail.frames, tail.n_oct,
                          tail.n_cls, s, n_out_stat, global_norm && c.output_norm ? +reduce_now : nullptr, &rctx,
                          (char*)w.mom + w.mom_scr[3])) return SVT_ERR_HIP;
    return SVT_OK;
  }
  if (c.output_norm) {
    if (int r = launch_moments(final_x, n_out / groups, out_mom, (char*)w.mom + w.mom_scr[1], B, s, groups)) return r;
    if (global_norm) { if (int r = reduce_now(&rctx)) return r; }
    if (int r = launch_global_norm(final_x, feats, n_out / groups, out_mom, 1e-5f, s, groups, n_out_stat)) return r;
  } else {
    if (launch_copy_f32(final_x, feats, n_out, s)) return SVT_ERR_HIP;
  }
  return SVT_OK;
}
```

svt_speechbrain_amd/csrc/common.h:

```cpp
#pragma once
#include <hip/hip_runtime.h>
#include <stdint.h>
#include <string>

typedef __bf16 real_bf16x8 __attribute__((ext_vector_type(8)));
#ifdef SVT_OPERAND_F16
typedef _Float16 bf16_t;
#define SVT_MFMA_16x16x32(a, b, c) __builtin_amdgcn_mfma_f32_16x16x32_f16(a, b, c, 0, 0, 0)
#define SVT_MFMA_32x32x16(a, b, c) __builtin_amdgcn_mfma_f32_32x32x16_f16(a, b, c, 0, 0, 0)
#else
typedef __bf16 bf16_t;
#define SVT_MFMA_16x16x32(a, b, c) __builtin_amdgcn_mfma_f32_16x16x32_bf16(a, b, c, 0, 0, 0)
#define SVT_MFMA_32x32x16(a, b, c) __builtin_amdgcn_mfma_f32_32x32x16_bf16(a, b, c, 0, 0, 0)
#endif
typedef bf16_t bf16x8 __attribute__((ext_vector_type(8)));
typedef bf16_t bf16x4 __attribute__((ext_vector_type(4)));
typedef float f32x4 __attribute__((ext_vector_type(4)));

namespace svt {

#if defined(__HIPCC__)
__device__ __forceinline__ float gelu_fast(float x) {
  const float z = fabsf(x) * 0.70710678118654752440f;
  const float t = __builtin_amdgcn_rcpf(fmaf(0.3275911f, z, 1.0f));
// ... 103 lines not shown
    t[i].y = __builtin_amdgcn_fmed3f(x[i].y, -3.8f, 3.8f);
  }
#pragma unroll
  for (int i = 0; i < NP; ++i) u[i] = t[i] * t[i];
#pragma unroll
  for (int i = 0; i < NP; ++i) q[i] = u[i] * SVT_GELU_C6 + SVT_GELU_C5;
  constexpr float c[5] = {SVT_GELU_C4, SVT_GELU_C3, SVT_GELU_C2, SVT_GELU_C1, SVT_GELU_C0};
#pragma unroll
  for (int k = 0; k < 5; ++k) {
#pragma unroll
    for (int i = 0; i < NP; ++i) q[i] = q[i] * u[i] + c[k];
  }
#pragma unroll
  for (int i = 0; i < NP; ++i) x[i] = x[i] * (t[i] * q[i] + SVT_GELU_HALF);
}
#endif
__device__ __forceinline__ void gelu_bf16x2_x4(f32x2_t (&x)[4]) { gelu_bf16x2_xn<4>(x); }
#endif

void set_error(const std::string& msg);
int hip_fail(hipError_t e, const char* what, const char* file, int line);

#define SVT_HIP(expr)                                                        \
  do {                                                                       \
    hipError_t _e = (expr);                                                  \
    if (_e != hipSuccess) return svt::hip_fail(_e, #expr, __FILE__, __LINE__); \
  } while (0)

#define SVT_LAUNCH_CHECK() SVT_HIP(hipGetLastError())

enum Act { ACT_NONE = 0, ACT_GELU = 1, ACT_RELU = 2, ACT_PRELU = 3 };

struct GemmArgs {
  const void* A = nullptr;
  const void* W = nullptr;
  void* C = nullptr;
  const float* bias = nullptr;
  const float* resid = nullptr;
  int M = 0, N = 0, K = 0;
  int a_rpb = 1;
  long a_bstride = 0, a_rstride = 0;
  long ldw = 0, ldc = 0;
  int nz = 1, nz2 = 1;
  long a_z1 = 0, a_z2 = 0, w_z1 = 0, w_z2 = 0, c_z1 = 0, c_z2 = 0, bias_z2 = 0;
  float alpha = 1.f;
  int act = ACT_NONE;
  int out_f32 = 0;
  int dbg = 0;
  int k_taps = 1, k_cin = 0;
  const void* W_kperm = nullptr;
  int kperm_taps = 0, kperm_cin = 0;
  int ksplit = 1;
  long ksplit_stride = 0;
  int walk_pm = 0;
  int c_vec = 1;
  int raster_gm = 8;
  int gen = 0;
  int a_d1 = 1, a_d2 = 1;
  long a_e1 = 0, a_e2 = 0;
  int kseg = 0;
  long kseg_stride = 0;
  int c_d1 = 1, c_d2 = 1;
  long c_e1 = 0, c_e2 = 0, c_base = 0;
  int c_nsplit = 0;
  long c_nstride = 0;
  const float* slope = nullptr;
  int resid_first = 0;
  int resid_op_type = 0;
  unsigned short* planes = nullptr;
  long plane_stride = 0;
  int planes_f16 = 0;
  int a_pairs = 0;
  int c_pairs = 0;
  int stamp_ends = 0;
  long long* trace = nullptr;
};

int launch_gemm(int prec, const GemmArgs& a, hipStream_t s);
int launch_gemm_skinny(const GemmArgs& a, hipStream_t s);

bool gemm_dma_eligible(const GemmArgs& a);
bool gemm_pps_eligible(const GemmArgs& a);
int launch_gemm_pps(const GemmArgs& a, int bm, hipStream_t s);
int launch_gemm_p1w(const GemmArgs& a, int bm, hipStream_t s);
bool gemm_skinny_eligible(const GemmArgs& a);
int split_weights_register(const void* w_f32_dev, long n_rows, int K, int kind, hipStream_t s);
void split_weights_forget(const void* w_f32_dev);
bool gemm_x3p_eligible(const GemmArgs& a);
int launch_gemm_x3p(int kind, const GemmArgs& a, const void* packed, hipStream_t s);
bool gemm_x3q_eligible(const GemmArgs& a);
int launch_gemm_x3q(int kind, const GemmArgs& a, const void* packed, int bm, hipStream_t s);
int launch_gemm_p1x(int kind, const GemmArgs& a, const void* packed, int bm, hipStream_t s);
#pragma GCC visibility push(hidden)
int launch_gemm_staged(int prec, const GemmArgs& a, int bn, hipStream_t s);
int launch_gemm_pp8(const GemmArgs& a, int bm, int bn, hipStream_t s);
int launch_gemm_pers(const GemmArgs& a, int bm, hipStream_t s);
int launch_gemm_skinny_tile(const GemmArgs& a, int tile, hipStream_t s);
const void* split_weights_find(const void* W, int kind, int K, long rows_needed);
int launch_gemm_x3s(int kind, const GemmArgs& a, const void* packed, int nbs, int form, hipStream_t s);
inline bool tile_span_fits(const GemmArgs& a) {
  const unsigned long clips = 255 / (unsigned long)(a.a_rpb > 0 ? a.a_rpb : 1) + 1;
  const unsigned long bs = (unsigned long)(a.a_bstride > 0 ? a.a_bstride : 0), rs = (unsigned long)(a.a_rstride > 0 ? a.a_rstride : 0);
  return a.a_bstride >= 0 && a.a_rstride > 0 && (clips * bs + 256ul * rs + (unsigned long)a.K) * 4 < 0xF0000000ul &&
         (unsigned long)a.N * a.K * 4 < 0xF0000000ul;
}
inline int persistent_blocks(int ntiles, int cap) { return ntiles < cap ? ((ntiles + 7) / 8) * 8 : cap; }
#pragma GCC visibility pop

__device__ __forceinline__ void tile_walk(int logical, int tiles_m, int tiles_n, int pm, int& tile_m, int& tile_n) {
  if (pm <= 0) { tile_n = logical % tiles_n; tile_m = logical / tiles_n; return; }
  const int per_panel = pm * tiles_n;
  const int pnl = logical / per_panel, rem = logical - pnl * per_panel;
  const int rows = min(pm, tiles_m - pnl * pm);
  tile_n = rem / rows;
  tile_m = pnl * pm + (rem - tile_n * rows);
}

extern int g_gemm_dbg;
extern int g_gemm_force_bm;
extern int g_gemm_ring;
extern int g_gemm_variant;
extern int g_gemm_skinny;
extern int g_gemm_skinny_max_tiles;
extern int g_gemm_x3;
extern int g_stamp_ends;
extern int g_x3_pairs;
extern int g_gemm_p1w;
extern int g_gemm_p1x;
extern int g_gemm_skinny_small_tiles;
extern int g_gemm_walk;
extern int g_conv_kperm;
extern int g_gemm_persist_wgs;
extern int g_gemm_kernel_id;

extern int g_ln_two_rows;
extern int g_flash_wide;
extern int g_flash_kernel_id;
extern int g_ffn2_ksplit;
#pragma GCC visibility push(hidden)
extern int g_conv_ln_bf16;
extern int g_debug_keep_split;
extern int g_conv_down_fused;
#pragma GCC visibility pop

int ensure_dyn_lds(const void* kernel, int bytes);

int dev_alloc(void** out, size_t bytes);
void dev_free(void* p);
extern int g_guard_alloc;

void prof_begin(hipStream_t s);
void prof_end(hipStream_t s, double flops, double bytes, int kind = 1);

int set_ticket_fenced(int on);
int launch_moments(const float* x, int64_t n, double* moments, void* scratch, int groups_max, hipStream_t s, int groups = 1);
size_t moments_scratch_bytes(int groups_max);
int launch_global_norm(const float* x, float* y, int64_t n, const double* moments, float eps, hipStream_t s, int groups = 1,
                       double n_stat = 0);
int launch_conv0_window_moments(const float* wav, int B, int64_t L, int k, int stride, int64_t T1,
                                double* wm , void* scratch , hipStream_t s);
size_t conv0_window_moments_scratch_bytes(int B, int64_t T1);
int launch_conv0_group_coef(const double* wav_moments , int64_t n_wav, const double* wm, int B,
                            int64_t T1, int C, int k, const float* w0 , const float* b0 ,
                            const float* gamma, const float* beta, float eps_wav, float eps_gn,
                            float* coef , hipStream_t s, int clips_per_norm_group);
struct FrameOut { float p_on, p_off; int32_t octave, pitch_class; };
int launch_head_fused(const float* x, int64_t rows, int K, const float* w, const float* wsum, const float* b, int N, float* dots,
                      double* mom, int64_t rows_per_group, float eps, float* logits, FrameOut* frames, int n_oct, int n_cls,
                      hipStream_t s,
                      double n_stat = 0, int (*between)(void*) = nullptr, void* between_arg = nullptr, void* scratch = nullptr);
size_t head_scratch_bytes(int64_t rows, int groups_max);

int launch_layernorm(int prec, const void* x, int x_is_f32, int64_t rows, int D, const float* gamma,
                     const float* beta, float eps, int gelu, void* yT, float* yF, hipStream_t s,
                     const float* add = nullptr, float* sumF = nullptr,
                     void* yP = nullptr, int pair_kind = 0,
                     const void* addP = nullptr);
bool layernorm_hilo_ok(int D);
int launch_layernorm_hilo_parts(const float* parts, int nparts, long part_stride, const float* pbias, const bf16_t* rh, const bf16_t* rl, int64_t rows,
                                int D, const float* gamma, const float* beta, float eps, bf16_t* yh, bf16_t* yl, float* yF, hipStream_t s);
int launch_layernorm_hilo(const bf16_t* branch, const bf16_t* rh, const bf16_t* rl, const float* x32, int64_t rows, int D,
                          const float* gamma, const float* beta, float eps, bf16_t* yh, bf16_t* yl, float* yF, hipStream_t s);

int launch_conv0_group_apply(int prec, const float* wav, int B, int64_t L, int k, int stride, int64_t T1, int C,
                             const float* coef, void* out , hipStream_t s, int pair_kind = 0);
int launch_conv0_layer(int prec, const float* wav, int B, int64_t L, int k, int stride, int64_t T1, int C,
                       const double* wav_moments, int64_t n_wav, float eps_wav, const float* w0, const float* b0,
                       const float* gamma, const float* beta, float eps, void* out, hipStream_t s, int clips_per_norm_group,
                       int pair_kind = 0);
int launch_f32_to_pairs(int kind, const float* x, void* out, int64_t n, hipStream_t s);
int launch_pairs_to_f32(int kind, const void* in, const void* lo_plane, float* y, int64_t n, hipStream_t s);

bool conv0_mfma_ok(int prec, int pair_kind, int k, int stride, int C);
size_t conv0_mfma_table_bytes(int B);
int launch_conv0_mfma_group(const float* wav, int B, int64_t L, int stride, int64_t T1, const float* coef, void* table_ws, void* out,
                            hipStream_t s, int pair_kind = 0);
int launch_conv0_mfma_layer(const float* wav, int B, int64_t L, int stride, int64_t T1, const double* wav_moments, int64_t n_wav,
                            float eps_wav, const float* w0, const float* b0, const float* gamma, const float* beta, float eps, void* table_ws,
                            void* out, hipStream_t s, int clips_per_norm_group, int pair_kind = 0);
extern int g_conv0_mfma;

int launch_f32_to_bf16(const float* in, bf16_t* out, int64_t n, hipStream_t s);
int launch_zero_bytes(void* p, size_t bytes, hipStream_t s);
int launch_copy_f32(const float* in, float* out, int64_t n, hipStream_t s);
int launch_zero_cols(float* p, int64_t rows, int cols, int64_t ld, hipStream_t s);
int launch_posconv_gather(int prec, const float* h, int B, int T, int D, int G, int kp, int Tp, void* out, hipStream_t s,
                          const float* sc = nullptr, const float* sh = nullptr);
int launch_posconv_scatter_add(const float* h, const void* y, int B, int T, int D, int G, int P, int Tq, float* pre, hipStream_t s,
                               int y_f32 = 0);
int launch_softmax_rows(int prec, const float* S, int64_t rows, int T, int Tp, void* P, hipStream_t s);
int launch_transpose_v(int prec, const void* qkv, int B, int T, int H, int dh, long ld, long voff, int Tp,
                       void* Vt, hipStream_t s);
int launch_axpby(int prec, const void* x, const void* y, float a, float b, void* out, int64_t n, hipStream_t s);
int launch_add_pe(int prec, const float* x, int B, int T, int Tsrc, int D, const float* pe, float* outF, void* outT,
                  hipStream_t s);
int launch_add_f32(const float* a, const float* b, float* out, int64_t n, hipStream_t s);
int launch_relpos_table(const float* embed, int H, int T, int num_buckets, int max_distance, float* pb, hipStream_t s);
int launch_relpos_gate(int prec, const void* u, int64_t rows, int T, int H, int dh, const float* wab, const float* bab,
                       const float* cst, float* gate, hipStream_t s);
int launch_scores_add_relbias(float* S, int64_t BH, int H, int T, int Tp, const float* gate, const float* pb, hipStream_t s);
int launch_clock_stamp(long long* out16, hipStream_t s);

int launch_flash_attention(const void* Q, long ldq, long q_bstride, const void* K, const void* V, long ldk, long k_bstride,
                           void* O, long ldo, long o_bstride, int B, int T, int H, int dh, float scale, hipStream_t s,
                           const float* gate = nullptr, const float* pb = nullptr);

int launch_split_planes(int kind, const float* src, long ld_src, long rows, int cols, void* dst, long ld_dst, long plane, hipStream_t s);
bool flash_attention_x3_ok(int dh);
int launch_flash_attention_x3(int kind, const void* Q, long ldq, long q_bstride, long q_plane, const void* K, const void* V, long ldk,
                              long k_bstride, long k_plane, float* O, long ldo, long o_bstride, int B, int T, int H, int dh, float scale,
                              hipStream_t s, int o_pairs = 0);

int launch_linear_f32(const float* x, int64_t rows, int K, const float* w, const float* b, int N, float* y,
                      hipStream_t s);
bool linear_head_eligible(int K, int N);
int launch_linear_head(const float* x, int64_t rows, int K, const float* w, const float* b, int N, float* y, hipStream_t s);
int launch_bce_loss(const float* x, int64_t B, int64_t t_pred, const float* y, int64_t t_tgt, int64_t T, const float* rel_len,
                    const float* pos_weight, float* per_frame, double* sums, hipStream_t s);
int launch_nll_loss(const float* logp, int64_t B, int64_t t_pred, int C, const int64_t* tgt, int64_t t_tgt, int64_t T,
                    const float* rel_len, float* per_frame, double* sums, int* bad_target, hipStream_t s);
int launch_loss_reduce(const double* sums, int B, int reduction, float smoothing, float* out, hipStream_t s);
int launch_softmax_small(const float* x, int64_t rows, int n, int apply_log, float* y, hipStream_t s);
int launch_deltas(const float* x, long ldx, int B, int T, int C, int n, float inv_denom, float* out, long ldo, hipStream_t s);
int launch_context_window(const float* x, int B, int T, int C, int ctx, int lag, int pad, float* out, hipStream_t s);
int launch_fbank_frames(const float* wav, int B, int64_t L, int n_fft, int hop, int64_t nframes, const float* window,
                        float* frames , hipStream_t s);
int launch_power_spectrum(const float* reim , int64_t rows, int nb,
                          int imoff, int ld, float* power , int ldp, hipStream_t s);
int launch_fbank_db(float* fb, int B, int64_t per_seq, float top_db, hipStream_t s);
int launch_decode_frames(const float* logits, int64_t rows, int n_out, int n_oct, int n_cls, FrameOut* out,
                         hipStream_t s);
int launch_ctc_greedy(const float* probs, int B, int T, int V, const float* rel_lens, int blank, int32_t* tokens,
                      int32_t* out_lens, hipStream_t s);

int launch_video_pad(int prec, const float* v, int B, int T, int H, int W, int Hp, int Wp, void* out, hipStream_t s);
struct VideoTransform { double sub0, div0, mean, std; };
int launch_video_pad_u8(int prec, const unsigned char* v, int B, int T, int Hin, int Win, int dy, int dx, int H, int W, int Hp, int Wp,
                        const VideoTransform& tf, void* out, hipStream_t s);
int launch_conv3d_front(int prec, const void* vp, const void* w, const float* bias, const float* slope, long F, int T, int Hp,
                        int Wp, int H0, int W0, void* out, hipStream_t s);
int launch_maxpool_3x3s2(int prec, const void* in, long F, int H0, int W0, int C, int H1, int W1, void* out, hipStream_t s);
extern int g_stem_pool_fused;
bool conv3d_front_pool_ok(int prec, int Hp, int Wp, int W0);
int launch_conv3d_front_pool(const void* vp, const void* w, const float* bias, const float* slope, long F, int T, int Hp, int Wp, int H0,
                             int W0, int H1, int W1, void* out, hipStream_t s);
int launch_zero_halo(int prec, void* buf, long F, int Hp, int Wp, int C, hipStream_t s);
int launch_avgpool_interior(int prec, const void* in, long F, int H, int W, int C, void* out, hipStream_t s);
extern int g_conv3x3_c64, g_conv3x3_c64_launches, g_conv3x3_c64_form;
bool conv3x3_c64_ok(int prec, int Hs, int Ws);
int launch_conv3x3_c64(const void* in, const void* wimg, const float* bias, const float* slope, const void* resid, void* out, long F,
                       int Hs, int Ws, hipStream_t s);
bool conv3x3_c128_ok(int prec, int Hs, int Ws);
int launch_conv3x3_c128(const void* in, const void* wimg, const float* bias, const float* slope, const void* resid, void* out, long F,
                        int Hs, int Ws, hipStream_t s);
int launch_amt_objective_grad(const float* x, int64_t B, int64_t t_pred, int n_out, int n_oct_cols, const float* on_t,
                              const float* off_t, const int64_t* oct_t, const int64_t* cls_t, int64_t t_tgt, int64_t T,
                              const float* rel_len, float pos_weight, float smoothing, float* dx, float* terms, void* ws,
                              hipStream_t s);
size_t amt_objective_status_offset(int64_t B);
size_t amt_objective_workspace_bytes(int64_t B);
int64_t linear_wgrad_slabs(int64_t rows, int D);
size_t linear_wgrad_workspace_bytes(int64_t rows, int D, int N);
int launch_linear_wgrad(const float* x, const float* dy, int64_t rows, int D, int N, float* dw, float* db, void* ws, hipStream_t s);
constexpr int kAdaMaxTensors = 32;
constexpr int64_t kAdaChunk = 4096;
size_t ada_workspace_bytes(const int64_t* numels, int count);
int launch_clip_adadelta(int count, float* const* params, float* const* grads, float* const* square_avg, float* const* acc_delta,
                         const int64_t* numels, float lr, float rho, float one_minus_rho, float eps, float weight_decay, int maximize,
                         float max_norm, float* total_norm, void* ws, hipStream_t s);
struct RcaRefreshJob {
  const float* src;
  void* dst;
  int64_t rows, cols;
  int transpose, f32;
};
constexpr int kRcaMaxRefreshJobs = 32;
struct RcaRefreshJobs {
  RcaRefreshJob j[kRcaMaxRefreshJobs];
  int n;
};
int launch_rca_refresh(int prec, const RcaRefreshJobs& jobs, hipStream_t s);
int launch_rca_attn_lse(int prec, const void* Q, long ldq, const void* K, long ldk, int B, int T, int H, int dh, float scale, float* lse,
                        hipStream_t s);
struct RcaAttnBwd {
  const void *q[2], *k, *v, *o[2];
  long ldq[2], ldkv;
  const float* dbl;
  float coef[2];
  const float* lse;
  float* delta;
  float* dq[2];
  long lddq[2];
  float *dk, *dv;
  long lddkv;
  int B, T, H, dh;
  float scale;
};
int launch_rca_attn_bwd(int prec, const RcaAttnBwd& p, hipStream_t s);
size_t rca_ln_bwd_scratch_bytes(int64_t rows, int D);
int launch_rca_ln_bwd(int prec, const float* x, const float* add, const float* gamma, const float* dy, int64_t rows, int D, float eps,
                      float* dxF, void* dxT, float* dgamma, float* dbeta, void* scratch, hipStream_t s);
int launch_rca_relu_mask(int prec, float* dh, const void* h, int64_t n, void* dhT, hipStream_t s);
struct RcaWgrad {
  const float* dy[2];
  const void* x[2];
  long ldy[2], ldx[2];
  int nseg;
  int64_t rows;
  int N, C;
};
size_t rca_wgrad_scratch_bytes(int64_t vrows, int N, int C);
int launch_rca_wgrad(int prec, const RcaWgrad& w, float* dw, float* db, void* scratch, hipStream_t s);
int launch_linear_dgrad(const float* dy, const float* w, int64_t rows, int D, int N, float* dx, hipStream_t s);

}
```

svt_speechbrain_amd/csrc/conv0_mfma.hip:

```cpp
#include "common.h"

namespace svt {
namespace {

constexpr int K0 = 10, C0 = 512, TBL16 = 2048;

template <int PK> struct C0T { typedef bf16_t piece; };
template <> struct C0T<2> { typedef __bf16 piece; };
template <> struct C0T<3> { typedef _Float16 piece; };
template <int PK> __device__ __forceinline__ f32x4 c0_mma(const typename C0T<PK>::piece __attribute__((ext_vector_type(8))) & a, const uint4& b, const f32x4& c) {
  typedef typename C0T<PK>::piece P;
  typedef P P8 __attribute__((ext_vector_type(8)));
  if constexpr (PK == 3) return __builtin_amdgcn_mfma_f32_16x16x32_f16(a, __builtin_bit_cast(P8, b), c, 0, 0, 0);
  else if constexpr (PK == 2) return __builtin_amdgcn_mfma_f32_16x16x32_bf16(a, __builtin_bit_cast(P8, b), c, 0, 0, 0);
  else return SVT_MFMA_16x16x32(a, __builtin_bit_cast(P8, b), c);
}
template <int PK> __device__ __forceinline__ void c0_store8(void* out, int64_t e, f32x2_t (&p)[4]) {
  typedef typename C0T<PK>::piece P;
  typedef P P8 __attribute__((ext_vector_type(8)));
  if constexpr (PK == 0) {
    gelu_bf16x2_x4(p);
    P8 o;
#pragma unroll
    for (int i = 0; i < 4; ++i) { o[2 * i] = (P)p[i].x; o[2 * i + 1] = (P)p[i].y; }
    *(P8*)((P*)out + e) = o;
  } else {
    P8 hi, lo;
#pragma unroll
    for (int i = 0; i < 4; ++i) {
      const f32x2_t y = gelu_fast2(p[i]);
      hi[2 * i] = (P)y.x; lo[2 * i] = (P)(y.x - (float)hi[2 * i]);
      hi[2 * i + 1] = (P)y.y; lo[2 * i + 1] = (P)(y.y - (float)hi[2 * i + 1]);
    }
    char* d = (char*)out + (e >> 5) * 128 + (e & 31) * 2;
    *(P8*)d = hi;
    *(P8*)(d + 64) = lo;
  }
}

__global__ __launch_bounds__(256) void conv0_coef_exp_kernel(const float* __restrict__ coef, int* __restrict__ exps) {
  const int b = blockIdx.x;
  float mx = 0.f;
  for (int i = threadIdx.x; i < C0 * K0; i += 256) mx = fmaxf(mx, fabsf(coef[((long)b * C0 + i / K0) * (K0 + 1) + i % K0]));
#pragma unroll
  for (int o = 32; o > 0; o >>= 1) mx = fmaxf(mx, __shfl_xor(mx, o, 64));
  __shared__ float part[4];
  if ((threadIdx.x & 63) == 0) part[threadIdx.x >> 6] = mx;
  __syncthreads();
  if (threadIdx.x == 0) {
    mx = fmaxf(fmaxf(part[0], part[1]), fmaxf(part[2], part[3]));
    int e = 0;
    if (mx > 0.f && mx < 3e38f) (void)frexpf(mx, &e);
    exps[b] = e > 100 ? 100 : (e < -100 ? -100 : e);
  }
}

template <int PK>
__global__ void conv0_table_kernel(const float* __restrict__ w, long w_clip_stride, int w_row, const float* __restrict__ bias,
                                   void* __restrict__ table_, const int* __restrict__ tap_exp) {
  typedef typename C0T<PK>::piece bf16_t;
  typedef bf16_t bf16x8 __attribute__((ext_vector_type(8)));
  bf16_t* table = (bf16_t*)table_;
  const int b = blockIdx.y;
  const int idx = blockIdx.x * blockDim.x + threadIdx.x;
  if (idx >= TBL16) return;
  const int blk = idx >> 6, lane = idx & 63, q = blk >> 3, nb = blk & 7, g = lane >> 4, j = lane & 15;
  const int c = 128 * q + 8 * j + nb;
  const float* wc = w + (long)b * w_clip_stride + (long)c * w_row;
  const float bv = bias ? bias[c] : (w_row == K0 + 1 ? wc[K0] : 0.f);
  const float tap_scale = tap_exp ? ldexpf(1.f, -tap_exp[b]) : 1.f;
  bf16x8 o;
#pragma unroll
  for (int i = 0; i < 8; ++i) {
    const int k = 8 * g + i;
    const float src = k < 30 ? wc[k % 10] * tap_scale : bv;
    const bf16_t hi = (bf16_t)src;
    const bf16_t lo = (bf16_t)(src - (float)hi);
    o[i] = (k < 20 || k == 30) ? hi : lo;
  }
  *(bf16x8*)(table + ((long)b * TBL16 + idx) * 8) = o;
}

template <int MODE, int PK = 0>
__global__ __launch_bounds__(256) void conv0_mfma_kernel(const float* __restrict__ wav, int64_t L, int stride, int64_t T1,
                                                         const void* __restrict__ table_, long table_clip_stride,
                                                         const double* __restrict__ wav_mom, int64_t n_wav, float eps_wav,
                                                         const float* __restrict__ gamma, const float* __restrict__ beta, float eps, int cpg,
                                                         void* __restrict__ out, const int* __restrict__ tap_exp) {
  typedef typename C0T<PK>::piece bf16_t;
  typedef bf16_t bf16x8 __attribute__((ext_vector_type(8)));
  const bf16_t* table = (const bf16_t*)table_;
  constexpr int FPW = 64;
  __shared__ __attribute__((aligned(16))) uint4 tbl[TBL16];
  __shared__ float xs[4][FPW * 5 + 16];
  const int tid = threadIdx.x, lane = tid & 63, wave = tid >> 6;
  const int b = blockIdx.y;
  {
    const uint4* tg = (const uint4*)(table + (long)b * table_clip_stride);
    for (int i = tid; i < TBL16; i += 256) tbl[i] = tg[i];
  }
  float mu = 0.f, rn = 1.f, xscale = 1.f, bscale = 1.f;
  if (MODE == 1 && wav_mom) {
    const double* wm = wav_mom + 2 * (b / cpg);
    const double m = wm[0] / (double)n_wav;
    const double var = wm[1] / (double)n_wav - m * m;
    mu = (float)m;
    rn = (float)(1.0 / sqrt(var + (double)eps_wav));
  }
  const int64_t t0 = ((int64_t)blockIdx.x * 4 + wave) * FPW;
  const int64_t left = T1 - t0;
  const int nfr = left >= FPW ? FPW : (left > 0 ? (int)left : 0);
  if (nfr > 0) {
    const float* x = wav + (int64_t)b * L + t0 * stride;
    const int ns = (nfr - 1) * stride + K0;
    float amax = 0.f;
    for (int i = lane; i < ns; i += 64) {
      const float v = MODE == 1 ? (x[i] - mu) * rn : x[i];
      xs[wave][i] = v;
      amax = fmaxf(amax, fabsf(v));
    }
    if constexpr (MODE == 0) {
#pragma unroll
      for (int o = 32; o > 0; o >>= 1) amax = fmaxf(amax, __shfl_xor(amax, o, 64));
      int e = 0;
      if (amax > 0.f && amax < 3e38f) { (void)frexpf(amax, &e); }
      e = e > 100 ? 100 : (e < -100 ? -100 : e);
      int tot = -e - (tap_exp ? tap_exp[b] : 0);
      tot = tot > 15 ? 15 : (tot < -14 ? -14 : tot);
      xscale = ldexpf(1.f, -e);
      bscale = ldexpf(1.f, tot);
      xscale = ldexpf(1.f, tot + (tap_exp ? tap_exp[b] : 0));
    }
  }
  __syncthreads();
  if (nfr <= 0) return;
  const float unscale = 1.f / bscale;
  const int g = lane >> 4, j = lane & 15;
  const bf16_t one = (bf16_t)bscale;
  for (int chunk = 0; chunk * 16 < nfr; ++chunk) {
    bf16x8 a;
    {
      int f = chunk * 16 + j;
      if (f > nfr - 1) f = nfr - 1;
      const float* xp = &xs[wave][f * stride];
      bf16_t h[K0], l[K0];
#pragma unroll
      for (int i = 0; i < K0; ++i) {
        const float v = xp[i] * xscale;
        h[i] = (bf16_t)v;
        l[i] = (bf16_t)(v - (float)h[i]);
      }
      const bf16x8 a0 = {h[0], h[1], h[2], h[3], h[4], h[5], h[6], h[7]};
      const bf16x8 a1 = {h[8], h[9], l[0], l[1], l[2], l[3], l[4], l[5]};
      const bf16x8 a2 = {l[6], l[7], l[8], l[9], h[0], h[1], h[2], h[3]};
      const bf16x8 a3 = {h[4], h[5], h[6], h[7], h[8], h[9], one, one};
      a = g == 0 ? a0 : (g == 1 ? a1 : (g == 2 ? a2 : a3));
    }
    const int64_t e0 = ((int64_t)b * T1 + t0 + chunk * 16 + 4 * g) * C0 + 8 * j;
    const int fr0 = chunk * 16 + 4 * g;
    if constexpr (MODE == 0) {
#pragma unroll 1
      for (int q = 0; q < 4; ++q) {
        f32x4 acc[8];
#pragma unroll
        for (int nb = 0; nb < 8; ++nb) {
          acc[nb] = f32x4{0.f, 0.f, 0.f, 0.f};
          acc[nb] = c0_mma<PK>(a, tbl[(q * 8 + nb) * 64 + lane], acc[nb]);
        }
#pragma unroll
        for (int r = 0; r < 4; ++r) {
          f32x2_t p[4];
#pragma unroll
          for (int i = 0; i < 4; ++i) p[i] = f32x2_t{acc[2 * i][r], acc[2 * i + 1][r]} * unscale;
          if (fr0 + r < nfr) c0_store8<PK>(out, e0 + (int64_t)r * C0 + 128 * q, p);
        }
      }
    } else {
      f32x4 acc[32];
#pragma unroll
      for (int blk = 0; blk < 32; ++blk) {
        acc[blk] = f32x4{0.f, 0.f, 0.f, 0.f};
        acc[blk] = c0_mma<PK>(a, tbl[blk * 64 + lane], acc[blk]);
      }
      float mean[4], rstd[4];
#pragma unroll
      for (int r = 0; r < 4; ++r) {
        float s = 0.f;
#pragma unroll
        for (int blk = 0; blk < 32; ++blk) s += acc[blk][r];
#pragma unroll
        for (int o = 8; o > 0; o >>= 1) s += __shfl_xor(s, o, 64);
        mean[r] = s * (1.f / C0);
      }
#pragma unroll
      for (int r = 0; r < 4; ++r) {
        float qq = 0.f;
#pragma unroll
        for (int blk = 0; blk < 32; ++blk) { const float d = acc[blk][r] - mean[r]; qq = fmaf(d, d, qq); }
#pragma unroll
        for (int o = 8; o > 0; o >>= 1) qq += __shfl_xor(qq, o, 64);
        rstd[r] = rsqrtf(qq * (1.f / C0) + eps);
      }
#pragma unroll
      for (int q = 0; q < 4; ++q) {
        __builtin_amdgcn_sched_barrier(0);
        const float4 g0 = *(const float4*)(gamma + 128 * q + 8 * j), g1 = *(const float4*)(gamma + 128 * q + 8 * j + 4);
        const float4 b0 = *(const float4*)(beta + 128 * q + 8 * j), b1 = *(const float4*)(beta + 128 * q + 8 * j + 4);
        const float gg[8] = {g0.x, g0.y, g0.z, g0.w, g1.x, g1.y, g1.z, g1.w}, bb[8] = {b0.x, b0.y, b0.z, b0.w, b1.x, b1.y, b1.z, b1.w};
#pragma unroll
        for (int r = 0; r < 4; ++r) {
          f32x2_t p[4];
#pragma unroll
          for (int i = 0; i < 4; ++i)
            p[i] = f32x2_t{fmaf((acc[q * 8 + 2 * i][r] - mean[r]) * rstd[r], gg[2 * i], bb[2 * i]),
                           fmaf((acc[q * 8 + 2 * i + 1][r] - mean[r]) * rstd[r], gg[2 * i + 1], bb[2 * i + 1])};
          if (fr0 + r < nfr) c0_store8<PK>(out, e0 + (int64_t)r * C0 + 128 * q, p);
        }
      }
    }
  }
}

}

int g_conv0_mfma = 1;

bool conv0_mfma_ok(int prec, int pair_kind, int k, int stride, int C) {
  return g_conv0_mfma && (prec == 1 || pair_kind == 2 || pair_kind == 3) && k == K0 && stride >= 1 && stride <= 5 && C == C0;
}
size_t conv0_mfma_table_bytes(int B) { return (size_t)B * TBL16 * 16 + (((size_t)B * 4 + 255) & ~(size_t)255); }

#define SVT_C0_DISPATCH(PKV, STMT)                 \
  if ((PKV) == 3) { constexpr int PK_ = 3; STMT }  \
  else if ((PKV) == 2) { constexpr int PK_ = 2; STMT } \
  else { constexpr int PK_ = 0; STMT }

int launch_conv0_mfma_group(const float* wav, int B, int64_t L, int stride, int64_t T1, const float* coef, void* table_ws, void* out,
                            hipStream_t s, int pair_kind) {
  if (((uintptr_t)table_ws & 15) || ((uintptr_t)out & 127)) { set_error("conv0_mfma: alignment"); return -1; }
  dim3 grid((unsigned)((T1 + 255) / 256), B);
  int* exps = (int*)((char*)table_ws + (size_t)B * TBL16 * 16);
  hipLaunchKernelGGL(conv0_coef_exp_kernel, dim3(B), dim3(256), 0, s, coef, exps);
  SVT_C0_DISPATCH(pair_kind,
    hipLaunchKernelGGL((conv0_table_kernel<PK_>), dim3(TBL16 / 256, B), dim3(256), 0, s, coef, (long)C0 * (K0 + 1), K0 + 1, (const float*)nullptr,
                       table_ws, (const int*)exps);
    hipLaunchKernelGGL((conv0_mfma_kernel<0, PK_>), grid, dim3(256), 0, s, wav, L, stride, T1, (const void*)table_ws, (long)TBL16 * 8,
                       (const double*)nullptr, (int64_t)1, 0.f, (const float*)nullptr, (const float*)nullptr, 0.f, 1, out, (const int*)exps);)
  SVT_LAUNCH_CHECK();
  return 0;
}

int launch_conv0_mfma_layer(const float* wav, int B, int64_t L, int stride, int64_t T1, const double* wav_moments, int64_t n_wav,
                            float eps_wav, const float* w0, const float* b0, const float* gamma, const float* beta, float eps, void* table_ws,
                            void* out, hipStream_t s, int cpg, int pair_kind) {
  if (((uintptr_t)table_ws & 15) || ((uintptr_t)out & 127) || ((uintptr_t)gamma & 15) || ((uintptr_t)beta & 15)) { set_error("conv0_mfma: alignment"); return -1; }
  dim3 grid((unsigned)((T1 + 255) / 256), B);
  SVT_C0_DISPATCH(pair_kind,
    hipLaunchKernelGGL((conv0_table_kernel<PK_>), dim3(TBL16 / 256, 1), dim3(256), 0, s, w0, 0L, K0, b0, table_ws, (const int*)nullptr);
    hipLaunchKernelGGL((conv0_mfma_kernel<1, PK_>), grid, dim3(256), 0, s, wav, L, stride, T1, (const void*)table_ws, 0L, wav_moments, n_wav,
                       eps_wav, gamma, beta, eps, cpg, out, (const int*)nullptr);)
  SVT_LAUNCH_CHECK();
  return 0;
}
#undef SVT_C0_DISPATCH

}
```

svt_speechbrain_amd/csrc/device_util.h:

```cpp
#pragma once
#include "common.h"

namespace svt {
namespace {

template <typename V>
__device__ __forceinline__ V wave_sum(V v) {
#pragma unroll
  for (int o = 32; o > 0; o >>= 1) v += __shfl_xor(v, o, 64);
  return v;
}
__device__ __forceinline__ float wave_max(float v) {
#pragma unroll
  for (int o = 32; o > 0; o >>= 1) v = fmaxf(v, __shfl_xor(v, o, 64));
  return v;
}

template <typename T> __device__ __forceinline__ float ld(const T* p, long i);
template <> __device__ __forceinline__ float ld<float>(const float* p, long i) { return p[i]; }
template <> __device__ __forceinline__ float ld<bf16_t>(const bf16_t* p, long i) { return (float)p[i]; }
template <typename T> __device__ __forceinline__ void st(T* p, long i, float v);
template <> __device__ __forceinline__ void st<float>(float* p, long i, float v) { p[i] = v; }
template <> __device__ __forceinline__ void st<bf16_t>(bf16_t* p, long i, float v) { p[i] = (bf16_t)v; }

template <int PK> __device__ __forceinline__ void cut_piece(float x, unsigned short& hi, unsigned short& lo) {
  if constexpr (PK == 3) {
    const _Float16 a = (_Float16)x, b = (_Float16)(x - (float)a);
    hi = __builtin_bit_cast(unsigned short, a); lo = __builtin_bit_cast(unsigned short, b);
  } else {
    const __bf16 a = (__bf16)x, b = (__bf16)(x - (float)a);
    hi = __builtin_bit_cast(unsigned short, a); lo = __builtin_bit_cast(unsigned short, b);
  }
}
template <int PK, int N> __device__ __forceinline__ void store_pairs(void* base, int64_t e, const float (&v)[N]) {
  static_assert(N == 4 || N == 8, "pieces of 4 or 8 elements");
  unsigned short h[N], l[N];
#pragma unroll
  for (int i = 0; i < N; ++i) cut_piece<PK>(v[i], h[i], l[i]);
  char* d = (char*)base + (e >> 5) * 128 + (e & 31) * 2;
  if constexpr (N == 8) {
    *(uint4*)d = uint4{(unsigned)h[0] | ((unsigned)h[1] << 16), (unsigned)h[2] | ((unsigned)h[3] << 16), (unsigned)h[4] | ((unsigned)h[5] << 16), (unsigned)h[6] | ((unsigned)h[7] << 16)};
    *(uint4*)(d + 64) = uint4{(unsigned)l[0] | ((unsigned)l[1] << 16), (unsigned)l[2] | ((unsigned)l[3] << 16), (unsigned)l[4] | ((unsigned)l[5] << 16), (unsigned)l[6] | ((unsigned)l[7] << 16)};
  } else {
    *(uint2*)d = uint2{(unsigned)h[0] | ((unsigned)h[1] << 16), (unsigned)h[2] | ((unsigned)h[3] << 16)};
    *(uint2*)(d + 64) = uint2{(unsigned)l[0] | ((unsigned)l[1] << 16), (unsigned)l[2] | ((unsigned)l[3] << 16)};
  }
}

constexpr int K0 = 10;
constexpr int NWM = K0 + K0 * (K0 + 1) / 2;

inline int grid_for(int64_t n, int block = 256, int cap = 8192) {
  int64_t g = (n + block - 1) / block;
  if (g > cap) g = cap;
  if (g < 1) g = 1;
  return (int)g;
}
template <class... P> inline bool aligned(unsigned mask, P... p) { return !((... | (uintptr_t)p) & mask); }

}
}
```

svt_speechbrain_amd/csrc/layernorm.hip:

```cpp
#include "device_util.h"
#include <type_traits>

namespace svt {
namespace {
template <typename TI, typename TO>
__global__ __launch_bounds__(256) void layernorm_kernel(const TI* x, const float* add, float* sumF, int64_t rows, int D,
                                                        const float* gamma, const float* beta, float eps, int gelu,
                                                        TO* yT, float* yF) {
  const int lane = threadIdx.x & 63;
  const int64_t row = (int64_t)blockIdx.x * 4 + (threadIdx.x >> 6);
  if (row >= rows) return;
  const TI* xr = x + row * D;
  const float* ar = add ? add + row * D : nullptr;
  float s = 0.f;
  for (int i = lane; i < D; i += 64) s += ld<TI>(xr, i) + (ar ? ar[i] : 0.f);
  const float mean = wave_sum(s) / (float)D;
  float q = 0.f;
  for (int i = lane; i < D; i += 64) { const float d = ld<TI>(xr, i) + (ar ? ar[i] : 0.f) - mean; q += d * d; }
  const float rstd = rsqrtf(wave_sum(q) / (float)D + eps);
  for (int i = lane; i < D; i += 64) {
    const float xv = ld<TI>(xr, i) + (ar ? ar[i] : 0.f);
    if (sumF) sumF[row * D + i] = xv;
    float v = (xv - mean) * rstd * gamma[i] + beta[i];
    if (gelu) v = gelu_erf(v);
// ... 173 lines not shown
  }
  SVT_LAUNCH_CHECK();
  return 0;
}

namespace {
template <int VPT>
__global__ __launch_bounds__(256) void layernorm_hilo_kernel(const bf16_t* branch, const bf16_t* rh, const bf16_t* rl,
                                                             int64_t rows, const float* gamma, const float* beta, float eps,
                                                             bf16_t* yh, bf16_t* yl, float* yF) {
  constexpr int D = 64 * VPT, NV = VPT / 4;
  const int lane = threadIdx.x & 63;
  const int64_t row = (int64_t)blockIdx.x * 4 + (threadIdx.x >> 6);
  if (row >= rows) return;
  float v[VPT];
  float s = 0.f;
#pragma unroll
  for (int j = 0; j < NV; ++j) {
    const long o = row * D + (lane + 64 * j) * 4;
    const bf16x4 h = *(const bf16x4*)(rh + o), l = *(const bf16x4*)(rl + o);
    float4 t = float4{(float)h[0] + (float)l[0], (float)h[1] + (float)l[1], (float)h[2] + (float)l[2], (float)h[3] + (float)l[3]};
    if (branch) {
      const bf16x4 a = *(const bf16x4*)(branch + o);
      t.x += (float)a[0]; t.y += (float)a[1]; t.z += (float)a[2]; t.w += (float)a[3];
    }
    v[4 * j] = t.x; v[4 * j + 1] = t.y; v[4 * j + 2] = t.z; v[4 * j + 3] = t.w;
    s += (t.x + t.y) + (t.z + t.w);
  }
  const float mean = wave_sum(s) * (1.f / D);
  float q = 0.f;
#pragma unroll
  for (int i = 0; i < VPT; ++i) { v[i] -= mean; q = fmaf(v[i], v[i], q); }
  const float rstd = rsqrtf(wave_sum(q) * (1.f / D) + eps);
#pragma unroll
  for (int j = 0; j < NV; ++j) {
    const int c = (lane + 64 * j) * 4;
    const float4 g = *(const float4*)(gamma + c), b = *(const float4*)(beta + c);
    const float o[4] = {fmaf(v[4 * j] * rstd, g.x, b.x), fmaf(v[4 * j + 1] * rstd, g.y, b.y),
                        fmaf(v[4 * j + 2] * rstd, g.z, b.z), fmaf(v[4 * j + 3] * rstd, g.w, b.w)};
    bf16x4 oh, ol;
#pragma unroll
    for (int i = 0; i < 4; ++i) { oh[i] = (bf16_t)o[i]; ol[i] = (bf16_t)(o[i] - (float)oh[i]); }
    *(bf16x4*)(yh + row * D + c) = oh;
    *(bf16x4*)(yl + row * D + c) = ol;
    if (yF) *(float4*)(yF + row * D + c) = float4{o[0], o[1], o[2], o[3]};
  }
}

template <int D, bool PARTS = false>
__global__ __launch_bounds__(256) void layernorm_hilo2_kernel(const bf16_t* branch, const bf16_t* rh, const bf16_t* rl,
                                                              int64_t rows, const float* gamma, const float* beta, float eps,
                                                              bf16_t* yh, bf16_t* yl, float* yF, const float* parts = nullptr, int nparts = 0,
                                                              long part_stride = 0, const float* pbias = nullptr) {
  constexpr int NC = D / 256;
  const int lane = threadIdx.x & 63, sub = lane & 31;
  const int64_t row = (int64_t)blockIdx.x * 8 + (threadIdx.x >> 6) * 2 + (lane >> 5);
  if (row >= rows) return;
  float v[NC][8];
  float s = 0.f;
#pragma unroll
  for (int j = 0; j < NC; ++j) {
    const long o = row * D + (sub + 32 * j) * 8;
    const bf16x8 h = *(const bf16x8*)(rh + o), l = *(const bf16x8*)(rl + o);
#pragma unroll
    for (int i = 0; i < 8; ++i) v[j][i] = (float)h[i] + (float)l[i];
    if constexpr (PARTS) {
      float a[8];
      {
        const float4 t0 = *(const float4*)(parts + o), t1 = *(const float4*)(parts + o + 4);
        a[0] = t0.x; a[1] = t0.y; a[2] = t0.z; a[3] = t0.w; a[4] = t1.x; a[5] = t1.y; a[6] = t1.z; a[7] = t1.w;
      }
      for (int k = 1; k < nparts; ++k) {
        const float4 t0 = *(const float4*)(parts + k * part_stride + o), t1 = *(const float4*)(parts + k * part_stride + o + 4);
        a[0] += t0.x; a[1] += t0.y; a[2] += t0.z; a[3] += t0.w; a[4] += t1.x; a[5] += t1.y; a[6] += t1.z; a[7] += t1.w;
      }
      const int c = (sub + 32 * j) * 8;
      const float4 b0 = *(const float4*)(pbias + c), b1 = *(const float4*)(pbias + c + 4);
      const float bb[8] = {b0.x, b0.y, b0.z, b0.w, b1.x, b1.y, b1.z, b1.w};
#pragma unroll
      for (int i = 0; i < 8; ++i) v[j][i] += (float)(bf16_t)(a[i] + bb[i]);
    } else if (branch) {
      const bf16x8 a = *(const bf16x8*)(branch + o);
#pragma unroll
      for (int i = 0; i < 8; ++i) v[j][i] += (float)a[i];
    }
    s += ((v[j][0] + v[j][1]) + (v[j][2] + v[j][3])) + ((v[j][4] + v[j][5]) + (v[j][6] + v[j][7]));
  }
#pragma unroll
  for (int o = 16; o > 0; o >>= 1) s += __shfl_xor(s, o, 64);
  const float mean = s * (1.f / D);
  float q = 0.f;
#pragma unroll
  for (int j = 0; j < NC; ++j)
#pragma unroll
    for (int i = 0; i < 8; ++i) { v[j][i] -= mean; q = fmaf(v[j][i], v[j][i], q); }
#pragma unroll
  for (int o = 16; o > 0; o >>= 1) q += __shfl_xor(q, o, 64);
  const float rstd = rsqrtf(q * (1.f / D) + eps);
#pragma unroll
  for (int j = 0; j < NC; ++j) {
    const int c = (sub + 32 * j) * 8;
    const float4 g0 = *(const float4*)(gamma + c), g1 = *(const float4*)(gamma + c + 4);
    const float4 b0 = *(const float4*)(beta + c), b1 = *(const float4*)(beta + c + 4);
    const float gg[8] = {g0.x, g0.y, g0.z, g0.w, g1.x, g1.y, g1.z, g1.w}, bb[8] = {b0.x, b0.y, b0.z, b0.w, b1.x, b1.y, b1.z, b1.w};
    float o[8];
    bf16x8 oh, ol;
#pragma unroll
    for (int i = 0; i < 8; ++i) {
      o[i] = fmaf(v[j][i] * rstd, gg[i], bb[i]);
      oh[i] = (bf16_t)o[i];
      ol[i] = (bf16_t)(o[i] - (float)oh[i]);
    }
    *(bf16x8*)(yh + row * D + c) = oh;
    *(bf16x8*)(yl + row * D + c) = ol;
    if (yF) {
      *(float4*)(yF + row * D + c) = float4{o[0], o[1], o[2], o[3]};
      *(float4*)(yF + row * D + c + 4) = float4{o[4], o[5], o[6], o[7]};
    }
  }
}
template <int VPT>
__global__ __launch_bounds__(256) void layernorm_f32_to_hilo_kernel(const float* x, int64_t rows, const float* gamma,
                                                                    const float* beta, float eps, bf16_t* yh, bf16_t* yl) {
  constexpr int D = 64 * VPT, NV = VPT / 4;
  const int lane = threadIdx.x & 63;
  const int64_t row = (int64_t)blockIdx.x * 4 + (threadIdx.x >> 6);
  if (row >= rows) return;
  float v[VPT];
  float s = 0.f;
#pragma unroll
  for (int j = 0; j < NV; ++j) {
    const float4 t = ((const float4*)(x + row * D))[lane + 64 * j];
    v[4 * j] = t.x; v[4 * j + 1] = t.y; v[4 * j + 2] = t.z; v[4 * j + 3] = t.w;
    s += (t.x + t.y) + (t.z + t.w);
  }
  const float mean = wave_sum(s) * (1.f / D);
  float q = 0.f;
#pragma unroll
  for (int i = 0; i < VPT; ++i) { v[i] -= mean; q = fmaf(v[i], v[i], q); }
  const float rstd = rsqrtf(wave_sum(q) * (1.f / D) + eps);
#pragma unroll
  for (int j = 0; j < NV; ++j) {
    const int c = (lane + 64 * j) * 4;
    const float4 g = *(const float4*)(gamma + c), b = *(const float4*)(beta + c);
    const float o[4] = {fmaf(v[4 * j] * rstd, g.x, b.x), fmaf(v[4 * j + 1] * rstd, g.y, b.y),
                        fmaf(v[4 * j + 2] * rstd, g.z, b.z), fmaf(v[4 * j + 3] * rstd, g.w, b.w)};
    bf16x4 oh, ol;
#pragma unroll
    for (int i = 0; i < 4; ++i) { oh[i] = (bf16_t)o[i]; ol[i] = (bf16_t)(o[i] - (float)oh[i]); }
    *(bf16x4*)(yh + row * D + c) = oh;
    *(bf16x4*)(yl + row * D + c) = ol;
  }
}
}
bool layernorm_hilo_ok(int D) { return D == 512 || D == 768 || D == 1024; }
int launch_layernorm_hilo_parts(const float* parts, int nparts, long part_stride, const float* pbias, const bf16_t* rh, const bf16_t* rl, int64_t rows,
                                int D, const float* gamma, const float* beta, float eps, bf16_t* yh, bf16_t* yl, float* yF, hipStream_t s) {
  if (!parts || nparts < 1 || !pbias || !(D == 512 || D == 768 || D == 1024) || (part_stride & 3) || !aligned(15, parts, pbias, rh, rl, yh, yl, yF, gamma, beta)) { set_error("layernorm (K-split branch): D in {512, 768, 1024} and 16-byte aligned buffers"); return -1; }
  const dim3 grid2((unsigned)((rows + 7) / 8)), block(256);
  ln_width(D, [&](auto vpt) {
    hipLaunchKernelGGL((layernorm_hilo2_kernel<64 * decltype(vpt)::value, true>), grid2, block, 0, s, nullptr, rh, rl, rows, gamma, beta, eps, yh, yl, yF, parts, nparts, part_stride, pbias);
  });
  SVT_LAUNCH_CHECK();
  return 0;
}
int launch_layernorm_hilo(const bf16_t* branch, const bf16_t* rh, const bf16_t* rl, const float* x32, int64_t rows, int D,
                          const float* gamma, const float* beta, float eps, bf16_t* yh, bf16_t* yl, float* yF, hipStream_t s) {
  const dim3 grid((unsigned)((rows + 3) / 4)), grid2((unsigned)((rows + 7) / 8)), block(256);
  ln_width(D, [&](auto vpt) {
    constexpr int VPT = decltype(vpt)::value;
    if (x32) hipLaunchKernelGGL((layernorm_f32_to_hilo_kernel<VPT>), grid, block, 0, s, x32, rows, gamma, beta, eps, yh, yl);
    else if (g_ln_two_rows && aligned(15, branch, rh, rl, yh, yl, yF, gamma, beta)) hipLaunchKernelGGL((layernorm_hilo2_kernel<64 * VPT>), grid2, block, 0, s, branch, rh, rl, rows, gamma, beta, eps, yh, yl, yF);
    else hipLaunchKernelGGL((layernorm_hilo_kernel<VPT>), grid, block, 0, s, branch, rh, rl, rows, gamma, beta, eps, yh, yl, yF);
  });
  SVT_LAUNCH_CHECK();
  return 0;
}

}
```

svt_speechbrain_amd/csrc/stats.hip:

```cpp
#include "device_util.h"

namespace svt {
namespace {
__device__ __forceinline__ void st_partial(double* p, double v) {
  __hip_atomic_store((unsigned long long*)p, __builtin_bit_cast(unsigned long long, v), __ATOMIC_RELAXED, __HIP_MEMORY_SCOPE_AGENT);
}
__device__ int d_ticket_fenced = 0;
__device__ __forceinline__ bool last_workgroup(unsigned* ticket, unsigned n_groups) {
  __shared__ unsigned s_last;
  asm volatile("s_waitcnt vmcnt(0)" ::: "memory");
  __syncthreads();
  if (threadIdx.x == 0) {
    const unsigned t = d_ticket_fenced ? __hip_atomic_fetch_add(ticket, 1u, __ATOMIC_ACQ_REL, __HIP_MEMORY_SCOPE_AGENT)
                                       : __hip_atomic_fetch_add(ticket, 1u, __ATOMIC_RELAXED, __HIP_MEMORY_SCOPE_AGENT);
    s_last = t == n_groups - 1 ? 1u : 0u;
    if (s_last) __hip_atomic_store(ticket, 0u, __ATOMIC_RELAXED, __HIP_MEMORY_SCOPE_AGENT);
  }
  __syncthreads();
  return s_last != 0;
}
__device__ __forceinline__ double ld_partial(const double* p) {
  return __builtin_bit_cast(double, __hip_atomic_load((const unsigned long long*)p, __ATOMIC_RELAXED, __HIP_MEMORY_SCOPE_AGENT));
}
}
int set_ticket_fenced(int on) {
  const int v = on ? 1 : 0;
  SVT_HIP(hipMemcpyToSymbol(HIP_SYMBOL(d_ticket_fenced), &v, sizeof(int)));
  return 0;
}

namespace {
__global__ __launch_bounds__(256) void moments_kernel(const float* x, int64_t n, double* mom, double* part, unsigned* ticket) {
  __shared__ double sh[2][4];
  x += (int64_t)blockIdx.y * n;
  mom += 2 * blockIdx.y;
  part += (size_t)blockIdx.y * gridDim.x * 2;
  double s = 0.0, ss = 0.0;
  const int64_t n4 = n >> 2;
  const float4* x4 = (const float4*)x;
  int64_t i = (int64_t)blockIdx.x * blockDim.x + threadIdx.x;
  const int64_t stride = (int64_t)gridDim.x * blockDim.x;
  for (; i < n4; i += stride) {
    const float4 v = x4[i];
    const float a = (v.x + v.y) + (v.z + v.w);
    const float b = (v.x * v.x + v.y * v.y) + (v.z * v.z + v.w * v.w);
    s += (double)a;
    ss += (double)b;
  }
  if (blockIdx.x == 0 && threadIdx.x == 0) {
    for (int64_t j = n4 << 2; j < n; ++j) { s += (double)x[j]; ss += (double)x[j] * (double)x[j]; }
  }
  s = wave_sum(s);
  ss = wave_sum(ss);
  const int lane = threadIdx.x & 63, wave = threadIdx.x >> 6;
  if (lane == 0) { sh[0][wave] = s; sh[1][wave] = ss; }
  __syncthreads();
  if (threadIdx.x == 0) {
    st_partial(part + blockIdx.x * 2, sh[0][0] + sh[0][1] + sh[0][2] + sh[0][3]);
    st_partial(part + blockIdx.x * 2 + 1, sh[1][0] + sh[1][1] + sh[1][2] + sh[1][3]);
  }
  if (!last_workgroup(ticket + blockIdx.y, gridDim.x)) return;
  s = 0.0; ss = 0.0;
  for (unsigned b = threadIdx.x; b < gridDim.x; b += 256) { s += ld_partial(part + b * 2); ss += ld_partial(part + b * 2 + 1); }
  s = wave_sum(s);
  ss = wave_sum(ss);
  if (lane == 0) { sh[0][wave] = s; sh[1][wave] = ss; }
  __syncthreads();
  if (threadIdx.x == 0) {
    mom[0] = sh[0][0] + sh[0][1] + sh[0][2] + sh[0][3];
    mom[1] = sh[1][0] + sh[1][1] + sh[1][2] + sh[1][3];
  }
}

__global__ void global_norm_kernel(const float* x, float* y, int64_t n, const double* mom, float eps, double n_stat) {
  x += (int64_t)blockIdx.y * n;
  y += (int64_t)blockIdx.y * n;
  mom += 2 * blockIdx.y;
  const double mean = mom[0] / n_stat;
  const double var = mom[1] / n_stat - mean * mean;
  const float mu = (float)mean;
  const float rs = (float)(1.0 / sqrt(var + (double)eps));
  const int64_t n4 = n >> 2;
  int64_t i = (int64_t)blockIdx.x * blockDim.x + threadIdx.x;
  const int64_t stride = (int64_t)gridDim.x * blockDim.x;
  for (; i < n4; i += stride) {
    float4 v = ((const float4*)x)[i];
    v.x = (v.x - mu) * rs; v.y = (v.y - mu) * rs; v.z = (v.z - mu) * rs; v.w = (v.w - mu) * rs;
    ((float4*)y)[i] = v;
  }
  if (blockIdx.x == 0 && threadIdx.x == 0)
    for (int64_t j = n4 << 2; j < n; ++j) y[j] = (x[j] - mu) * rs;
}
}
static int moments_grid(int64_t n, int groups) {
  return groups > 1 ? grid_for(n / 4 + 1, 256, 512 / (groups < 64 ? groups : 64) + 1) : grid_for(n / 4 + 1, 256, 512);
}
static size_t moments_ticket_bytes(int groups) { return ((size_t)groups * 4 + 255) & ~(size_t)255; }
size_t moments_scratch_bytes(int groups_max) {
  const size_t wgs = (size_t)(groups_max < 64 ? 512 + groups_max : 576) + 9 * (size_t)groups_max;
  return moments_ticket_bytes(groups_max) + wgs * 2 * sizeof(double);
}

int launch_moments(const float* x, int64_t n, double* moments, void* scratch, int groups_max, hipStream_t s, int groups) {
  if (groups > 1 && (n & 3)) { set_error("moments: per-group length must be a multiple of 4 elements"); return -1; }
  if (groups > groups_max || !scratch || ((uintptr_t)scratch & 7)) { set_error("moments: scratch"); return -1; }
  const int gx = moments_grid(n, groups);
  if (moments_ticket_bytes(groups_max) + (size_t)gx * groups * 2 * sizeof(double) > moments_scratch_bytes(groups_max)) { set_error("moments: scratch too small"); return -1; }
  unsigned* ticket = (unsigned*)scratch;
  double* part = (double*)((char*)scratch + moments_ticket_bytes(groups_max));
  hipLaunchKernelGGL(moments_kernel, dim3(gx, groups), dim3(256), 0, s, x, n, moments, part, ticket);
  SVT_LAUNCH_CHECK();
  return 0;
}

int launch_global_norm(const float* x, float* y, int64_t n, const double* moments, float eps, hipStream_t s, int groups, double n_stat) {
  if (groups > 1 && (n & 3)) { set_error("global_norm: per-group length must be a multiple of 4 elements"); return -1; }
  hipLaunchKernelGGL(global_norm_kernel, dim3(grid_for(n / 4 + 1), groups), dim3(256), 0, s, x, y, n, moments, eps,
                     n_stat > 0 ? n_stat : (double)n);
  SVT_LAUNCH_CHECK();
  return 0;
}

namespace {
__global__ __launch_bounds__(256) void conv0_window_moments_kernel(const float* wav, int64_t L, int stride, int64_t T1,
                                                                   double* wm, double* part, unsigned* ticket) {
  __shared__ double sh[4][NWM];
  const int b = blockIdx.y;
  const float* x = wav + (int64_t)b * L;
  double acc[NWM];
#pragma unroll
  for (int i = 0; i < NWM; ++i) acc[i] = 0.0;
  constexpr int WPT = 8;
  const int64_t t0 = ((int64_t)blockIdx.x * blockDim.x + threadIdx.x) * WPT;
  for (int w = 0; w < WPT; ++w) {
    const int64_t t = t0 + w;
    if (t >= T1) break;
    float v[K0];
#pragma unroll
    for (int j = 0; j < K0; ++j) v[j] = x[t * stride + j];
    int idx = K0;
#pragma unroll
    for (int j = 0; j < K0; ++j) {
      acc[j] += (double)v[j];
#pragma unroll
      for (int j2 = j; j2 < K0; ++j2) acc[idx++] += (double)(v[j] * v[j2]);
    }
  }
  const int lane = threadIdx.x & 63, wave = threadIdx.x >> 6;
#pragma unroll
  for (int i = 0; i < NWM; ++i) {
    const double r = wave_sum(acc[i]);
    if (lane == 0) sh[wave][i] = r;
  }
  __syncthreads();
  part += (size_t)b * gridDim.x * NWM;
  if (threadIdx.x < NWM)
    st_partial(part + blockIdx.x * NWM + threadIdx.x, sh[0][threadIdx.x] + sh[1][threadIdx.x] + sh[2][threadIdx.x] + sh[3][threadIdx.x]);
  if (!last_workgroup(ticket + b, gridDim.x)) return;
  if (threadIdx.x < NWM) {
    double t = 0.0;
    unsigned k = 0;
    for (; k + 8 <= gridDim.x; k += 8) {
      double v[8];
#pragma unroll
      for (int j = 0; j < 8; ++j) v[j] = ld_partial(part + (k + j) * NWM + threadIdx.x);
#pragma unroll
      for (int j = 0; j < 8; ++j) t += v[j];
    }
    for (; k < gridDim.x; ++k) t += ld_partial(part + k * NWM + threadIdx.x);
    wm[b * NWM + threadIdx.x] = t;
  }
}

__global__ void conv0_group_coef_kernel(const double* wav_mom, int64_t n_wav, const double* wm, int64_t T1, int C,
                                        const float* w0, const float* b0, const float* gamma, const float* beta,
                                        float eps_wav, float eps_gn, float* coef, int cpg) {
  const int b = blockIdx.y;
  if (wav_mom) wav_mom += 2 * (b / cpg);
  const int c = blockIdx.x * blockDim.x + threadIdx.x;
  if (c >= C) return;
  double mu = 0.0, r = 1.0;
  if (wav_mom) {
    mu = wav_mom[0] / (double)n_wav;
    const double var = wav_mom[1] / (double)n_wav - mu * mu;
    r = 1.0 / sqrt(var + (double)eps_wav);
  }
  const double* m = wm + b * NWM;
  const double invT = 1.0 / (double)T1;
  double w[K0], mn[K0];
  double wsum = 0.0;
  for (int j = 0; j < K0; ++j) { w[j] = (double)w0[c * K0 + j]; wsum += w[j]; mn[j] = r * (m[j] * invT - mu); }
  const double bias = b0 ? (double)b0[c] : 0.0;
  double dot = 0.0;
  for (int j = 0; j < K0; ++j) dot += w[j] * mn[j];
  double quad = 0.0;
  int idx = K0;
  for (int j = 0; j < K0; ++j)
    for (int j2 = j; j2 < K0; ++j2) {
      const double R = r * r * (m[idx] * invT - mu * m[j] * invT - mu * m[j2] * invT + mu * mu);
      quad += (j == j2 ? 1.0 : 2.0) * w[j] * w[j2] * R;
      ++idx;
    }
  const double mean = dot + bias;
  const double e2 = quad + 2.0 * bias * dot + bias * bias;
  double var = e2 - mean * mean;
  if (var < 0.0) var = 0.0;
  const double a = (double)gamma[c] / sqrt(var + (double)eps_gn);
  const double shift = (double)beta[c] - mean * a;
  float* o = coef + ((int64_t)b * C + c) * (K0 + 1);
  for (int j = 0; j < K0; ++j) o[j] = (float)(a * r * w[j]);
  o[K0] = (float)(a * (bias - r * mu * wsum) + shift);
}
}
size_t conv0_window_moments_scratch_bytes(int B, int64_t T1) {
  const size_t gx = (size_t)((T1 + 2047) / 2048);
  return moments_ticket_bytes(B) + (size_t)B * gx * NWM * sizeof(double);
}

int launch_conv0_window_moments(const float* wav, int B, int64_t L, int k, int stride, int64_t T1, double* wm, void* scratch,
                                hipStream_t s) {
  if (k != K0) { set_error("conv layer 0 kernel size must be 10"); return -1; }
  if (!scratch || ((uintptr_t)scratch & 7)) { set_error("conv0 window moments: scratch"); return -1; }
  const int per_block = 256 * 8;
  dim3 grid((unsigned)((T1 + per_block - 1) / per_block), B);
  unsigned* ticket = (unsigned*)scratch;
  double* part = (double*)((char*)scratch + moments_ticket_bytes(B));
  hipLaunchKernelGGL(conv0_window_moments_kernel, grid, dim3(256), 0, s, wav, L, stride, T1, wm, part, ticket);
  SVT_LAUNCH_CHECK();
  return 0;
}

int launch_conv0_group_coef(const double* wav_moments, int64_t n_wav, const double* wm, int B, int64_t T1, int C,
                            int k, const float* w0, const float* b0, const float* gamma, const float* beta,
                            float eps_wav, float eps_gn, float* coef, hipStream_t s, int cpg) {
  if (k != K0) { set_error("conv layer 0 kernel size must be 10"); return -1; }
  dim3 grid((C + 63) / 64, B);
  hipLaunchKernelGGL(conv0_group_coef_kernel, grid, dim3(64), 0, s, wav_moments, n_wav, wm, T1, C, w0, b0, gamma, beta,
                     eps_wav, eps_gn, coef, cpg);
  SVT_LAUNCH_CHECK();
  return 0;
}

namespace {
template <int KC>
__global__ __launch_bounds__(256) void head_dots_kernel(const float* __restrict__ x, int64_t rows, const float* __restrict__ w, int N,
                                                        float* __restrict__ dots, double* __restrict__ mom, int64_t rows_per_group,
                                                        double* __restrict__ slots, unsigned* __restrict__ ticket, int slots_per_group) {
  constexpr int K = KC * 256;
  extern __shared__ __attribute__((aligned(16))) float wl[];
  for (int i = threadIdx.x * 4; i < N * K; i += 1024) *(float4*)(wl + i) = *(const float4*)(w + i);
  __syncthreads();
  const int lane = threadIdx.x & 63, wave = threadIdx.x >> 6;
  const bool hi32 = (lane & 32) != 0, hi16 = (lane & 16) != 0;
  const int myrow = (hi32 ? 2 : 0) + (hi16 ? 1 : 0);
  const int NW = (int)gridDim.x * 4, W = (int)blockIdx.x * 4 + wave;
  int64_t cur_g = -1, g_end = 0;
  float la = 0.f, lq = 0.f;
  auto flush = [&]() {
    if (cur_g < 0) return;
    const double sa = wave_sum((double)la), sq = wave_sum((double)lq);
    if (lane == 0) {
      const int64_t ja = (cur_g * rows_per_group) >> 2;
      const int p = (int)(((W - ja) % NW + NW) % NW);
      double* sl = slots + ((size_t)cur_g * slots_per_group + p) * 2;
      st_partial(sl, sa);
      st_partial(sl + 1, sq);
    }
    la = 0.f; lq = 0.f;
  };
  for (int64_t r0 = ((int64_t)blockIdx.x * 4 + wave) * 4; r0 < rows; r0 += (int64_t)gridDim.x * 16) {
    float4 xv[4][KC];
#pragma unroll
    for (int rr = 0; rr < 4; ++rr) {
      const int64_t row = r0 + rr < rows ? r0 + rr : rows - 1;
      const auto xrs = __builtin_amdgcn_make_buffer_rsrc((void*)x, 0, 0x7FFFFFF0, 0x00020000);
#pragma unroll
      for (int c = 0; c < KC; ++c) {
        typedef float f4v __attribute__((ext_vector_type(4)));
        const f4v t = __builtin_bit_cast(f4v, __builtin_amdgcn_raw_buffer_load_b128(xrs, (unsigned)((row * K + c * 256 + lane * 4) * 4), 0, 0));
        xv[rr][c] = float4{t[0], t[1], t[2], t[3]};
      }
    }
    if (mom) {
#pragma unroll
      for (int rr = 0; rr < 4; ++rr) {
        if (r0 + rr >= rows) break;
        if (r0 + rr >= g_end || cur_g < 0) {
          flush();
          cur_g = (r0 + rr) / rows_per_group;
          g_end = (cur_g + 1) * rows_per_group;
        }
        float a = 0.f, q = 0.f;
#pragma unroll
        for (int c = 0; c < KC; ++c) {
          const float4 v = xv[rr][c];
          a += (v.x + v.y) + (v.z + v.w);
          q += (v.x * v.x + v.y * v.y) + (v.z * v.z + v.w * v.w);
        }
        la += a;
        lq += q;
      }
    }
    float out0 = 0.f, out1 = 0.f;
    for (int n = 0; n < N; ++n) {
      float sacc[4] = {0.f, 0.f, 0.f, 0.f};
#pragma unroll
      for (int c = 0; c < KC; ++c) {
        const float4 wv = *(const float4*)(wl + n * K + c * 256 + lane * 4);
#pragma unroll
        for (int rr = 0; rr < 4; ++rr) {
          sacc[rr] = fmaf(xv[rr][c].x, wv.x, sacc[rr]);
          sacc[rr] = fmaf(xv[rr][c].y, wv.y, sacc[rr]);
          sacc[rr] = fmaf(xv[rr][c].z, wv.z, sacc[rr]);
          sacc[rr] = fmaf(xv[rr][c].w, wv.w, sacc[rr]);
        }
      }
      float k0 = hi32 ? sacc[2] : sacc[0], k1 = hi32 ? sacc[3] : sacc[1];
      const float g0 = hi32 ? sacc[0] : sacc[2], g1 = hi32 ? sacc[1] : sacc[3];
      k0 += __shfl_xor(g0, 32, 64);
      k1 += __shfl_xor(g1, 32, 64);
      float v = hi16 ? k1 : k0;
      v += __shfl_xor(hi16 ? k0 : k1, 16, 64);
#pragma unroll
      for (int o = 8; o > 0; o >>= 1) v += __shfl_xor(v, o, 64);
      if ((lane & 15) == (n & 15)) { if (n < 16) out0 = v; else out1 = v; }
    }
    const int64_t row = r0 + myrow;
    if (row < rows) {
      const int n0 = lane & 15;
      if (n0 < N) dots[row * N + n0] = out0;
      if (n0 + 16 < N) dots[row * N + n0 + 16] = out1;
    }
  }
  if (mom) {
    flush();
    if (!last_workgroup(ticket, gridDim.x)) return;
    const int64_t n_groups = (rows + rows_per_group - 1) / rows_per_group;
    for (int64_t g = wave; g < n_groups; g += 4) {
      const int64_t a = g * rows_per_group, b = (g + 1) * rows_per_group < rows ? (g + 1) * rows_per_group : rows;
      const int64_t nj = ((b - 1) >> 2) - (a >> 2) + 1;
      const int n = (int)(nj < NW ? nj : NW);
      const double* sl = slots + (size_t)g * slots_per_group * 2;
      double ta = 0.0, tq = 0.0;
      int i = lane;
      for (; i + 3 * 64 < n; i += 4 * 64) {
        double va[4], vq[4];
#pragma unroll
        for (int j = 0; j < 4; ++j) { va[j] = ld_partial(sl + 2 * (i + 64 * j)); vq[j] = ld_partial(sl + 2 * (i + 64 * j) + 1); }
#pragma unroll
        for (int j = 0; j < 4; ++j) { ta += va[j]; tq += vq[j]; }
      }
      for (; i < n; i += 64) { ta += ld_partial(sl + 2 * i); tq += ld_partial(sl + 2 * i + 1); }
      ta = wave_sum(ta);
      tq = wave_sum(tq);
      if (lane == 0) { mom[2 * g] = ta; mom[2 * g + 1] = tq; }
    }
  }
}

__global__ void head_finish_kernel(const float* __restrict__ dots, int64_t rows, int N, const float* __restrict__ wsum,
                                   const float* __restrict__ bias, const double* __restrict__ mom, int64_t rows_per_group,
                                   double group_elems, float eps, float* __restrict__ logits, FrameOut* __restrict__ frames,
                                   int n_oct, int n_cls) {
  const int64_t r = (int64_t)blockIdx.x * blockDim.x + threadIdx.x;
  if (r >= rows) return;
  float mu = 0.f, rs = 1.f;
  if (mom) {
    const int64_t g = r / rows_per_group;
    const double mean = mom[2 * g] / group_elems;
    const double var = mom[2 * g + 1] / group_elems - mean * mean;
    mu = (float)mean;
    rs = (float)(1.0 / sqrt(var + (double)eps));
  }
  float l[32];
#pragma unroll
  for (int j = 0; j < 32; ++j)
    if (j < N) {
      l[j] = fmaf(dots[r * N + j] - mu * wsum[j], rs, bias ? bias[j] : 0.f);
      logits[r * N + j] = l[j];
    }
  if (frames) {
    FrameOut f;
    f.p_on = 1.f / (1.f + expf(-l[0]));
    f.p_off = 1.f / (1.f + expf(-l[1]));
    int bo = 0;
    float bv = l[2];
#pragma unroll
    for (int j = 3; j < 32; ++j)
      if (j <= 2 + n_oct && l[j] > bv) { bv = l[j]; bo = j - 2; }
    int bc = 0;
    const int c0 = 2 + n_oct + 1;
    bv = -3.4e38f;
#pragma unroll
    for (int j = 3; j < 32; ++j)
      if (j >= c0 && j <= c0 + n_cls) {
        if (j == c0) { bv = l[j]; bc = 0; }
        else if (l[j] > bv) { bv = l[j]; bc = j - c0; }
      }
    f.octave = bo;
    f.pitch_class = bc;
    frames[r] = f;
  }
}
}
static unsigned head_dots_grid(int64_t rows) {
  const int64_t blocks = (rows + 15) / 16;
  return (unsigned)(blocks < 512 ? blocks : 512);
}
static int head_slots_per_group(int64_t rows, int64_t rpg) {
  const int64_t nw = (int64_t)head_dots_grid(rows) * 4, per = (rpg + 3) / 4 + 1;
  return (int)(per < nw ? per : nw);
}
size_t head_scratch_bytes(int64_t rows, int groups_max) {
  return 256 + ((size_t)rows / 4 + 2 * (size_t)groups_max + 8) * 2 * sizeof(double);
}

template <int KC>
static int launch_head_dots_kc(const float* x, int64_t rows, const float* w, int N, float* dots, double* mom, int64_t rpg, void* scratch,
                               hipStream_t s) {
  const size_t lds = (size_t)N * KC * 256 * 4;
  if (int r_ = ensure_dyn_lds((const void*)head_dots_kernel<KC>, 32 * KC * 256 * 4)) return r_;
  const unsigned grid = head_dots_grid(rows);
  if (mom && (!scratch || ((uintptr_t)scratch & 7))) { set_error("head_fused: scratch"); return -1; }
  if ((unsigned long)rows * KC * 256 * 4 > 0x7FFFFFF0ul) { set_error("head_fused: more than 2 GiB of encoder output (32-bit buffer offsets)"); return -1; }
  unsigned* ticket = (unsigned*)scratch;
  double* slots = scratch ? (double*)((char*)scratch + 256) : nullptr;
  hipLaunchKernelGGL((head_dots_kernel<KC>), dim3(grid), dim3(256), lds, s, x, rows, w, N, dots, mom, rpg, slots, ticket,
                     mom ? head_slots_per_group(rows, rpg) : 0);
  SVT_LAUNCH_CHECK();
  return 0;
}
int launch_head_fused(const float* x, int64_t rows, int K, const float* w, const float* wsum, const float* b, int N, float* dots,
                      double* mom , int64_t rows_per_group, float eps, float* logits,
                      FrameOut* frames, int n_oct, int n_cls, hipStream_t s, double n_stat, int (*between)(void*), void* between_arg,
                      void* scratch ) {
  if (!linear_head_eligible(K, N)) { set_error("head_fused: unsupported head geometry"); return -1; }
  if (frames && (N != 2 + n_oct + 1 + n_cls + 1 || N > 32)) { set_error("head_fused: n_out != 2 + (n_octave+1) + (n_class+1)"); return -1; }
  if (mom) {
    const int64_t groups = (rows + rows_per_group - 1) / rows_per_group;
    if (256 + (size_t)groups * head_slots_per_group(rows, rows_per_group) * 16 > head_scratch_bytes(rows, (int)groups)) { set_error("head_fused: scratch too small"); return -1; }
  }
  int r = K == 512 ? launch_head_dots_kc<2>(x, rows, w, N, dots, mom, rows_per_group, scratch, s)
        : K == 768 ? launch_head_dots_kc<3>(x, rows, w, N, dots, mom, rows_per_group, scratch, s)
                   : launch_head_dots_kc<4>(x, rows, w, N, dots, mom, rows_per_group, scratch, s);
  if (r) return r;
  if (between) { if (int rb = between(between_arg)) return rb; }
  hipLaunchKernelGGL(head_finish_kernel, dim3((unsigned)((rows + 255) / 256)), dim3(256), 0, s, dots, rows, N, wsum, b, mom,
                     rows_per_group, n_stat > 0 ? n_stat : (double)rows_per_group * (double)K, eps, logits, frames, n_oct, n_cls);
  SVT_LAUNCH_CHECK();
  return 0;
}

}
```

Measured before the change: 6182 clips/s.

## Fuse conv0 setup, posconv add+layernorm, pipeline head dots, batch stats

Several independent fusions are added, each behind a debug flag that defaults on. The conv0 group coefficient and table setup become a single kernel. The positional-conv scatter-add is fused into the encoder-input hi/lo layernorm. The head dot-product kernel gets a software-pipelined variant that prefetches the next rows while computing the current ones. The intent is to cut kernel launches and intermediate HBM round trips in the front end and the head, at the cost of more code paths and more register pressure in the pipelined head kernel.

```diff
diff --git a/include/svt_mi355.h b/include/svt_mi355.h
--- a/include/svt_mi355.h
+++ b/include/svt_mi355.h
@@ -188,6 +188,9 @@
 int svt_debug_rca_attn_bwd(int32_t precision, const void* qkv, const void* qc, const void* o_self, const void* o_cross,
                            const float* dblend, float alpha, int32_t batch, int32_t t, int32_t heads, int32_t head_dim, float* dqkv,
                            float* dqc, void* workspace_dev, size_t* workspace_bytes, int device, void* stream);
+int svt_debug_posconv_layernorm(const float* h, const void* y, int32_t batch, int32_t t, int32_t d, int32_t groups, int32_t p,
+                                const float* gamma, const float* beta, float eps, void* y_hi, void* y_lo, float* pre, int device,
+                                void* stream);
 int svt_debug_set(int key, int value);
 
 int svt_prof_enable(int on);
diff --git a/svt_speechbrain_amd/_lib.py b/svt_speechbrain_amd/_lib.py
--- a/svt_speechbrain_amd/_lib.py
+++ b/svt_speechbrain_amd/_lib.py
@@ -125,6 +125,8 @@
     "svt_debug_rca_attn_bwd": (C.c_int, [C.c_int32, _P, _P, _P, _P, _P, C.c_float, C.c_int32, C.c_int32, C.c_int32, C.c_int32, _P, _P,
                                          _P, C.POINTER(C.c_size_t), C.c_int, _P]),
     "svt_debug_set": (C.c_int, [C.c_int, C.c_int]),
+    "svt_debug_posconv_layernorm": (C.c_int, [_P, _P, C.c_int32, C.c_int32, C.c_int32, C.c_int32, C.c_int32, _P, _P, C.c_float, _P, _P, _P,
+                                              C.c_int, _P]),
     "svt_debug_clock": (C.c_int, [C.c_void_p, C.c_int, C.c_void_p]),
     "svt_debug_encoder_layout": (C.c_int, [C.c_void_p, C.c_int32, C.c_int64, C.POINTER(C.c_int64), C.c_int]),
     "svt_operand_type": (C.c_int, []),
diff --git a/svt_speechbrain_amd/csrc/api.hip b/svt_speechbrain_amd/csrc/api.hip
--- a/svt_speechbrain_amd/csrc/api.hip
+++ b/svt_speechbrain_amd/csrc/api.hip
@@ -403,6 +403,25 @@
   return SVT_OK;
 }
 
+int svt_debug_posconv_layernorm(const float* h, const void* y, int32_t batch, int32_t t, int32_t d, int32_t groups, int32_t p,
+                                const float* gamma, const float* beta, float eps, void* y_hi, void* y_lo, float* pre, int device,
+                                void* stream) {
+  if (!h || !y || !gamma || !beta || !y_hi || !y_lo || !pre) { set_error("svt_debug_posconv_layernorm: null argument"); return SVT_ERR_INVALID; }
+  if (batch < 1 || t < 1 || p < 1 || groups < 1 || !layernorm_hilo_ok(d) || d % groups || (d / groups) % 8) {
+    set_error("svt_debug_posconv_layernorm: d in {512, 768, 1024}, groups of a multiple of 8 channels"); return SVT_ERR_INVALID; }
+  if (int r = check_device(device)) return r;
+  SVT_HIP(hipSetDevice(device));
+  const int tq = (t + p - 1) / p;
+  hipStream_t s = (hipStream_t)stream;
+  if (posconv_layernorm_hilo_ok(d, groups))
+    return launch_posconv_add_layernorm_hilo(h, (const bf16_t*)y, batch, t, d, groups, p, tq, gamma, beta, eps, (bf16_t*)y_hi, (bf16_t*)y_lo, s)
+               ? SVT_ERR_INVALID : SVT_OK;
+  if (launch_posconv_scatter_add(h, y, batch, t, d, groups, p, tq, pre, s, 0)) return SVT_ERR_INVALID;
+  if (launch_layernorm_hilo(nullptr, nullptr, nullptr, pre, (int64_t)batch * t, d, gamma, beta, eps, (bf16_t*)y_hi, (bf16_t*)y_lo, nullptr, s))
+    return SVT_ERR_INVALID;
+  return SVT_OK;
+}
+
 int svt_debug_set(int key, int value) {
   if (key == 0) g_gemm_dbg = value;
   else if (key == 1) g_gemm_force_bm = value;
@@ -450,6 +469,10 @@
   else if (key == 37) { if (value < 8 || value > 256 || value % 8) { set_error("svt_debug_set(37): 8 .. 256, a multiple of 8"); return SVT_ERR_INVALID; } g_gemm_persist_wgs = value; }
   else if (key == 38) return g_flash_kernel_id;
   else if (key == 39) return g_gemm_kernel_id;
+  else if (key == 40) g_stats_batched = value;
+  else if (key == 41) g_conv0_setup_fused = value;
+  else if (key == 42) g_posconv_ln_fused = value;
+  else if (key == 43) g_head_dots_pipe = value;
   else { set_error("svt_debug_set: unknown key"); return SVT_ERR_INVALID; }
   return SVT_OK;
 }
diff --git a/svt_speechbrain_amd/csrc/api_encoder.hip b/svt_speechbrain_amd/csrc/api_encoder.hip
--- a/svt_speechbrain_amd/csrc/api_encoder.hip
+++ b/svt_speechbrain_amd/csrc/api_encoder.hip
@@ -555,11 +555,16 @@
   const ConvLayerW& c0 = e->conv[0];
   if (c.feat_extract_norm == SVT_NORM_GROUP) {
     if (int r = launch_conv0_window_moments(wav, B, L, c.conv_kernel[0], c.conv_stride[0], t1, wm, (char*)w.mom + w.mom_scr[2], s)) return r;
+    const bool c0_mfma = conv0_mfma_ok(prec, pk_front, c.conv_kernel[0], c.conv_stride[0], c.conv_dim[0]) && w.c0tab;
+    const Conv0GroupCoefArgs gc{wav_mom, n_wav, wm, c0.w.as<float>(), c.conv_bias ? c0.bias.as<float>() : nullptr, c0.gamma.as<float>(),
+                                c0.beta.as<float>(), 1e-5f, 1e-5f, cpg};
+    const bool setup_fused = c0_mfma && g_conv0_setup_fused;
+    if (!setup_fused)
     if (int r = launch_conv0_group_coef(wav_mom, n_wav, wm, B, t1, c.conv_dim[0], c.conv_kernel[0], c0.w.as<float>(),
                                         c.conv_bias ? c0.bias.as<float>() : nullptr, c0.gamma.as<float>(),
                                         c0.beta.as<float>(), 1e-5f, 1e-5f, w.coef, s, cpg)) return r;
-    if (conv0_mfma_ok(prec, pk_front, c.conv_kernel[0], c.conv_stride[0], c.conv_dim[0]) && w.c0tab) {
-      if (int r = launch_conv0_mfma_group(wav, B, L, c.conv_stride[0], t1, w.coef, w.c0tab, w.act[0], s, pk_front)) return r;
+    if (c0_mfma) {
+      if (int r = launch_conv0_mfma_group(wav, B, L, c.conv_stride[0], t1, w.coef, w.c0tab, w.act[0], s, pk_front, setup_fused ? &gc : nullptr)) return r;
     } else
     if (int r = launch_conv0_group_apply(prec, wav, B, L, c.conv_kernel[0], c.conv_stride[0], t1, c.conv_dim[0], w.coef,
                                          w.act[0], s, pk_front)) return r;
@@ -634,6 +639,8 @@
     g.a_pairs = pk_front ? 1 : 0;
     if (int r = launch_gemm(gp, g, s)) return r;
   }
+  bool pos_ln_fused = false;
+  int pos_P = 0, pos_Tq = 0;
   {
     const int kp = c.pos_conv_kernel, G = c.pos_conv_groups, cg = D / G;
     const int Pf = e->pos_P;
@@ -672,6 +679,9 @@
       g.a_z2 = (long)Tp * cg; g.w_z2 = (long)g.N * g.K; g.c_z2 = (long)B * Tq * g.N; g.bias_z2 = g.N;
       g.act = ACT_GELU; g.out_f32 = 0;
       if (int r = launch_gemm(gp, g, s)) return r;
+      pos_ln_fused = !c.stable_layer_norm && prec && c.num_layers > 0 && posconv_layernorm_hilo_ok(D, G);
+      pos_P = Pf; pos_Tq = Tq;
+      if (!pos_ln_fused)
       if (int r = launch_posconv_scatter_add(w.hF, w.posy, B, (int)T, D, G, Pf, Tq, w.preF, s, prec ? 0 : 1)) return r;
     } else {
     if (int r = launch_posconv_gather(prec, w.hF, B, (int)T, D, G, kp, (int)T + kp, w.posg, s, bn_sc, bn_sh)) return r;
@@ -732,6 +742,10 @@
   if (!c.stable_layer_norm && prec && layernorm_hilo_ok(D) && c.num_layers > 0) {
     bf16_t* xh = (bf16_t*)w.xb;
     bf16_t* xl = (bf16_t*)w.xlo;
+    if (pos_ln_fused) {
+      if (int r = launch_posconv_add_layernorm_hilo(w.hF, (const bf16_t*)w.posy, B, (int)T, D, c.pos_conv_groups, pos_P, pos_Tq,
+                                                    e->enc_g.as<float>(), e->enc_b.as<float>(), eps, xh, xl, s)) return r;
+    } else
     if (int r = launch_layernorm_hilo(nullptr, nullptr, nullptr, w.preF, rows, D, e->enc_g.as<float>(), e->enc_b.as<float>(), eps,
                                       xh, xl, nullptr, s)) return r;
     bool ffn2_split = false;
diff --git a/svt_speechbrain_amd/csrc/common.h b/svt_speechbrain_amd/csrc/common.h
--- a/svt_speechbrain_amd/csrc/common.h
+++ b/svt_speechbrain_amd/csrc/common.h
@@ -279,6 +279,8 @@
 void prof_begin(hipStream_t s);
 void prof_end(hipStream_t s, double flops, double bytes, int kind = 1);
 
+extern int g_stats_batched;
+extern int g_head_dots_pipe;
 int set_ticket_fenced(int on);
 int launch_moments(const float* x, int64_t n, double* moments, void* scratch, int groups_max, hipStream_t s, int groups = 1);
 size_t moments_scratch_bytes(int groups_max);
@@ -306,6 +308,10 @@
 bool layernorm_hilo_ok(int D);
 int launch_layernorm_hilo_parts(const float* parts, int nparts, long part_stride, const float* pbias, const bf16_t* rh, const bf16_t* rl, int64_t rows,
                                 int D, const float* gamma, const float* beta, float eps, bf16_t* yh, bf16_t* yl, float* yF, hipStream_t s);
+extern int g_posconv_ln_fused;
+bool posconv_layernorm_hilo_ok(int D, int G);
+int launch_posconv_add_layernorm_hilo(const float* h, const bf16_t* y, int B, int T, int D, int G, int P, int Tq, const float* gamma,
+                                      const float* beta, float eps, bf16_t* yh, bf16_t* yl, hipStream_t s);
 int launch_layernorm_hilo(const bf16_t* branch, const bf16_t* rh, const bf16_t* rl, const float* x32, int64_t rows, int D,
                           const float* gamma, const float* beta, float eps, bf16_t* yh, bf16_t* yl, float* yF, hipStream_t s);
 
@@ -320,8 +326,13 @@
 
 bool conv0_mfma_ok(int prec, int pair_kind, int k, int stride, int C);
 size_t conv0_mfma_table_bytes(int B);
-int launch_conv0_mfma_group(const float* wav, int B, int64_t L, int stride, int64_t T1, const float* coef, void* table_ws, void* out,
-                            hipStream_t s, int pair_kind = 0);
+struct Conv0GroupCoefArgs {
+  const double* wav_mom; int64_t n_wav; const double* wm; const float* w0; const float* b0; const float* gamma; const float* beta;
+  float eps_wav, eps_gn; int cpg;
+};
+extern int g_conv0_setup_fused;
+int launch_conv0_mfma_group(const float* wav, int B, int64_t L, int stride, int64_t T1, float* coef, void* table_ws, void* out,
+                            hipStream_t s, int pair_kind = 0, const Conv0GroupCoefArgs* gc = nullptr);
 int launch_conv0_mfma_layer(const float* wav, int B, int64_t L, int stride, int64_t T1, const double* wav_moments, int64_t n_wav,
                             float eps_wav, const float* w0, const float* b0, const float* gamma, const float* beta, float eps, void* table_ws,
                             void* out, hipStream_t s, int clips_per_norm_group, int pair_kind = 0);
diff --git a/svt_speechbrain_amd/csrc/conv0_mfma.hip b/svt_speechbrain_amd/csrc/conv0_mfma.hip
--- a/svt_speechbrain_amd/csrc/conv0_mfma.hip
+++ b/svt_speechbrain_amd/csrc/conv0_mfma.hip
@@ -1,9 +1,9 @@
-#include "common.h"
+#include "device_util.h"
 
 namespace svt {
 namespace {
 
-constexpr int K0 = 10, C0 = 512, TBL16 = 2048;
+constexpr int C0 = 512, TBL16 = 2048;
 
 template <int PK> struct C0T { typedef bf16_t piece; };
 template <> struct C0T<2> { typedef __bf16 piece; };
@@ -79,6 +79,59 @@
     o[i] = (k < 20 || k == 30) ? hi : lo;
   }
   *(bf16x8*)(table + ((long)b * TBL16 + idx) * 8) = o;
+}
+
+template <int PK>
+__global__ __launch_bounds__(C0) void conv0_group_setup_kernel(const double* __restrict__ wav_mom, int64_t n_wav, const double* __restrict__ wm,
+                                                               int64_t T1, const float* __restrict__ w0, const float* __restrict__ b0,
+                                                               const float* __restrict__ gamma, const float* __restrict__ beta,
+                                                               float eps_wav, float eps_gn, int cpg, float* __restrict__ coef,
+                                                               void* __restrict__ table_, int* __restrict__ exps) {
+  typedef typename C0T<PK>::piece bf16_t;
+  typedef bf16_t bf16x8 __attribute__((ext_vector_type(8)));
+  __shared__ float cf[C0 * (K0 + 1)];
+  __shared__ float part[C0 / 64];
+  __shared__ int s_exp;
+  const int b = blockIdx.x, c = threadIdx.x;
+  float o[K0 + 1];
+  conv0_group_coef_one(wav_mom ? wav_mom + 2 * (b / cpg) : nullptr, n_wav, wm + b * NWM, T1, w0 + c * K0, b0, gamma, beta, c, eps_wav,
+                       eps_gn, o);
+  float mx = 0.f;
+#pragma unroll
+  for (int j = 0; j <= K0; ++j) {
+    coef[((long)b * C0 + c) * (K0 + 1) + j] = o[j];
+    cf[c * (K0 + 1) + j] = o[j];
+    if (j < K0) mx = fmaxf(mx, fabsf(o[j]));
+  }
+  mx = wave_max(mx);
+  if ((c & 63) == 0) part[c >> 6] = mx;
+  __syncthreads();
+  if (c == 0) {
+#pragma unroll
+    for (int i = 1; i < C0 / 64; ++i) mx = fmaxf(mx, part[i]);
+    int e = 0;
+    if (mx > 0.f && mx < 3e38f) (void)frexpf(mx, &e);
+    e = e > 100 ? 100 : (e < -100 ? -100 : e);
+    exps[b] = e;
+    s_exp = e;
+  }
+  __syncthreads();
+  const float tap_scale = ldexpf(1.f, -s_exp);
+  bf16_t* table = (bf16_t*)table_;
+  for (int idx = c; idx < TBL16; idx += C0) {
+    const int blk = idx >> 6, lane = idx & 63, q = blk >> 3, nb = blk & 7, g = lane >> 4, j = lane & 15;
+    const float* wc = cf + (128 * q + 8 * j + nb) * (K0 + 1);
+    bf16x8 ov;
+#pragma unroll
+    for (int i = 0; i < 8; ++i) {
+      const int k = 8 * g + i;
+      const float src = k < 30 ? wc[k % 10] * tap_scale : wc[K0];
+      const bf16_t hi = (bf16_t)src;
+      const bf16_t lo = (bf16_t)(src - (float)hi);
+      ov[i] = (k < 20 || k == 30) ? hi : lo;
+    }
+    *(bf16x8*)(table + ((long)b * TBL16 + idx) * 8) = ov;
+  }
 }
 
 template <int MODE, int PK = 0>
@@ -235,13 +288,17 @@
   else if ((PKV) == 2) { constexpr int PK_ = 2; STMT } \
   else { constexpr int PK_ = 0; STMT }
 
-int launch_conv0_mfma_group(const float* wav, int B, int64_t L, int stride, int64_t T1, const float* coef, void* table_ws, void* out,
-                            hipStream_t s, int pair_kind) {
+int g_conv0_setup_fused = 1;
+int launch_conv0_mfma_group(const float* wav, int B, int64_t L, int stride, int64_t T1, float* coef, void* table_ws, void* out,
+                            hipStream_t s, int pair_kind, const Conv0GroupCoefArgs* gc) {
   if (((uintptr_t)table_ws & 15) || ((uintptr_t)out & 127)) { set_error("conv0_mfma: alignment"); return -1; }
   dim3 grid((unsigned)((T1 + 255) / 256), B);
   int* exps = (int*)((char*)table_ws + (size_t)B * TBL16 * 16);
-  hipLaunchKernelGGL(conv0_coef_exp_kernel, dim3(B), dim3(256), 0, s, coef, exps);
+  if (!gc) hipLaunchKernelGGL(conv0_coef_exp_kernel, dim3(B), dim3(256), 0, s, coef, exps);
   SVT_C0_DISPATCH(pair_kind,
+    if (gc) hipLaunchKernelGGL((conv0_group_setup_kernel<PK_>), dim3(B), dim3(C0), 0, s, gc->wav_mom, gc->n_wav, gc->wm, T1, gc->w0, gc->b0, gc->gamma,
+                               gc->beta, gc->eps_wav, gc->eps_gn, gc->cpg, coef, table_ws, exps);
+    else
     hipLaunchKernelGGL((conv0_table_kernel<PK_>), dim3(TBL16 / 256, B), dim3(256), 0, s, coef, (long)C0 * (K0 + 1), K0 + 1, (const float*)nullptr,
                        table_ws, (const int*)exps);
     hipLaunchKernelGGL((conv0_mfma_kernel<0, PK_>), grid, dim3(256), 0, s, wav, L, stride, T1, (const void*)table_ws, (long)TBL16 * 8,
diff --git a/svt_speechbrain_amd/csrc/device_util.h b/svt_speechbrain_amd/csrc/device_util.h
--- a/svt_speechbrain_amd/csrc/device_util.h
+++ b/svt_speechbrain_amd/csrc/device_util.h
@@ -50,6 +50,40 @@
 constexpr int K0 = 10;
 constexpr int NWM = K0 + K0 * (K0 + 1) / 2;
 
+__device__ __forceinline__ void conv0_group_coef_one(const double* wav_mom, int64_t n_wav, const double* m, int64_t T1, const float* w0c,
+                                                     const float* b0, const float* gamma, const float* beta, int c, float eps_wav,
+                                                     float eps_gn, float (&o)[K0 + 1]) {
+  double mu = 0.0, r = 1.0;
+  if (wav_mom) {
+    mu = wav_mom[0] / (double)n_wav;
+    const double var = wav_mom[1] / (double)n_wav - mu * mu;
+    r = 1.0 / sqrt(var + (double)eps_wav);
+  }
+  const double invT = 1.0 / (double)T1;
+  double w[K0], mn[K0];
+  double wsum = 0.0;
+  for (int j = 0; j < K0; ++j) { w[j] = (double)w0c[j]; wsum += w[j]; mn[j] = r * (m[j] * invT - mu); }
+  const double bias = b0 ? (double)b0[c] : 0.0;
+  double dot = 0.0;
+  for (int j = 0; j < K0; ++j) dot += w[j] * mn[j];
+  double quad = 0.0;
+  int idx = K0;
+  for (int j = 0; j < K0; ++j)
+    for (int j2 = j; j2 < K0; ++j2) {
+      const double R = r * r * (m[idx] * invT - mu * m[j] * invT - mu * m[j2] * invT + mu * mu);
+      quad += (j == j2 ? 1.0 : 2.0) * w[j] * w[j2] * R;
+      ++idx;
+    }
+  const double mean = dot + bias;
+  const double e2 = quad + 2.0 * bias * dot + bias * bias;
+  double var = e2 - mean * mean;
+  if (var < 0.0) var = 0.0;
+  const double a = (double)gamma[c] / sqrt(var + (double)eps_gn);
+  const double shift = (double)beta[c] - mean * a;
+  for (int j = 0; j < K0; ++j) o[j] = (float)(a * r * w[j]);
+  o[K0] = (float)(a * (bias - r * mu * wsum) + shift);
+}
+
 inline int grid_for(int64_t n, int block = 256, int cap = 8192) {
   int64_t g = (n + block - 1) / block;
   if (g > cap) g = cap;
diff --git a/svt_speechbrain_amd/csrc/layernorm.hip b/svt_speechbrain_amd/csrc/layernorm.hip
--- a/svt_speechbrain_amd/csrc/layernorm.hip
+++ b/svt_speechbrain_amd/csrc/layernorm.hip
@@ -349,6 +349,47 @@
     *(bf16x4*)(yl + row * D + c) = ol;
   }
 }
+template <int VPT>
+__global__ __launch_bounds__(256) void posconv_add_layernorm_hilo_kernel(const float* h, const bf16_t* y, int B, int T, int G, int P, int Tq,
+                                                                         int64_t rows, const float* gamma, const float* beta, float eps,
+                                                                         bf16_t* yh, bf16_t* yl) {
+  constexpr int D = 64 * VPT, NV = VPT / 4;
+  const int lane = threadIdx.x & 63;
+  const int64_t row = (int64_t)blockIdx.x * 4 + (threadIdx.x >> 6);
+  if (row >= rows) return;
+  const int cg = D / G;
+  const int t = (int)(row % T), b = (int)(row / T);
+  const int q = t / P, j = t - q * P;
+  float v[VPT];
+  float s = 0.f;
+#pragma unroll
+  for (int jj = 0; jj < NV; ++jj) {
+    const int ch = (lane + 64 * jj) * 4;
+    const int g = ch / cg, c = ch - g * cg;
+    const bf16x4 a = *(const bf16x4*)(y + (((int64_t)g * B + b) * Tq + q) * (P * cg) + j * cg + c);
+    const float4 hv = *(const float4*)(h + row * D + ch);
+    const float4 tt = float4{hv.x + (float)a[0], hv.y + (float)a[1], hv.z + (float)a[2], hv.w + (float)a[3]};
+    v[4 * jj] = tt.x; v[4 * jj + 1] = tt.y; v[4 * jj + 2] = tt.z; v[4 * jj + 3] = tt.w;
+    s += (tt.x + tt.y) + (tt.z + tt.w);
+  }
+  const float mean = wave_sum(s) * (1.f / D);
+  float qq = 0.f;
+#pragma unroll
+  for (int i = 0; i < VPT; ++i) { v[i] -= mean; qq = fmaf(v[i], v[i], qq); }
+  const float rstd = rsqrtf(wave_sum(qq) * (1.f / D) + eps);
+#pragma unroll
+  for (int jj = 0; jj < NV; ++jj) {
+    const int c = (lane + 64 * jj) * 4;
+    const float4 g = *(const float4*)(gamma + c), bb = *(const float4*)(beta + c);
+    const float o[4] = {fmaf(v[4 * jj] * rstd, g.x, bb.x), fmaf(v[4 * jj + 1] * rstd, g.y, bb.y),
+                        fmaf(v[4 * jj + 2] * rstd, g.z, bb.z), fmaf(v[4 * jj + 3] * rstd, g.w, bb.w)};
+    bf16x4 oh, ol;
+#pragma unroll
+    for (int i = 0; i < 4; ++i) { oh[i] = (bf16_t)o[i]; ol[i] = (bf16_t)(o[i] - (float)oh[i]); }
+    *(bf16x4*)(yh + row * D + c) = oh;
+    *(bf16x4*)(yl + row * D + c) = ol;
+  }
+}
 }
 bool layernorm_hilo_ok(int D) { return D == 512 || D == 768 || D == 1024; }
 int launch_layernorm_hilo_parts(const float* parts, int nparts, long part_stride, const float* pbias, const bf16_t* rh, const bf16_t* rl, int64_t rows,
@@ -374,4 +415,19 @@
   return 0;
 }
 
-}
+int g_posconv_ln_fused = 1;
+bool posconv_layernorm_hilo_ok(int D, int G) { return g_posconv_ln_fused && layernorm_hilo_ok(D) && G > 0 && D % G == 0 && (D / G) % 4 == 0; }
+int launch_posconv_add_layernorm_hilo(const float* h, const bf16_t* y, int B, int T, int D, int G, int P, int Tq, const float* gamma,
+                                      const float* beta, float eps, bf16_t* yh, bf16_t* yl, hipStream_t s) {
+  if (!posconv_layernorm_hilo_ok(D, G) || P < 1 || (int64_t)Tq * P < T || !aligned(15, h, gamma, beta) || !aligned(7, y, yh, yl)) {
+    set_error("posconv + layernorm: D in {512, 768, 1024}, groups of a multiple of 4 channels and aligned buffers"); return -1; }
+  const int64_t rows = (int64_t)B * T;
+  const dim3 grid((unsigned)((rows + 3) / 4)), block(256);
+  ln_width(D, [&](auto vpt) {
+    hipLaunchKernelGGL((posconv_add_layernorm_hilo_kernel<decltype(vpt)::value>), grid, block, 0, s, h, y, B, T, G, P, Tq, rows, gamma, beta, eps, yh, yl);
+  });
+  SVT_LAUNCH_CHECK();
+  return 0;
+}
+
+}
diff --git a/svt_speechbrain_amd/csrc/stats.hip b/svt_speechbrain_amd/csrc/stats.hip
--- a/svt_speechbrain_amd/csrc/stats.hip
+++ b/svt_speechbrain_amd/csrc/stats.hip
@@ -30,6 +30,7 @@
 }
 
 namespace {
+template <bool BATCH>
 __global__ __launch_bounds__(256) void moments_kernel(const float* x, int64_t n, double* mom, double* part, unsigned* ticket) {
   __shared__ double sh[2][4];
   x += (int64_t)blockIdx.y * n;
@@ -40,12 +41,22 @@
   const float4* x4 = (const float4*)x;
   int64_t i = (int64_t)blockIdx.x * blockDim.x + threadIdx.x;
   const int64_t stride = (int64_t)gridDim.x * blockDim.x;
-  for (; i < n4; i += stride) {
-    const float4 v = x4[i];
+  auto add4 = [&](const float4 v) {
     const float a = (v.x + v.y) + (v.z + v.w);
     const float b = (v.x * v.x + v.y * v.y) + (v.z * v.z + v.w * v.w);
     s += (double)a;
     ss += (double)b;
+  };
+  if constexpr (BATCH) {
+    for (; i < n4; i += 8 * stride) {
+      float4 v[8];
+#pragma unroll
+      for (int j = 0; j < 8; ++j) v[j] = i + j * stride < n4 ? x4[i + j * stride] : float4{0.f, 0.f, 0.f, 0.f};
+#pragma unroll
+      for (int j = 0; j < 8; ++j) if (i + j * stride < n4) add4(v[j]);
+    }
+  } else {
+    for (; i < n4; i += stride) add4(x4[i]);
   }
   if (blockIdx.x == 0 && threadIdx.x == 0) {
     for (int64_t j = n4 << 2; j < n; ++j) { s += (double)x[j]; ss += (double)x[j] * (double)x[j]; }
@@ -92,6 +103,7 @@
     for (int64_t j = n4 << 2; j < n; ++j) y[j] = (x[j] - mu) * rs;
 }
 }
+int g_stats_batched = 1;
 static int moments_grid(int64_t n, int groups) {
   return groups > 1 ? grid_for(n / 4 + 1, 256, 512 / (groups < 64 ? groups : 64) + 1) : grid_for(n / 4 + 1, 256, 512);
 }
@@ -108,7 +120,8 @@
   if (moments_ticket_bytes(groups_max) + (size_t)gx * groups * 2 * sizeof(double) > moments_scratch_bytes(groups_max)) { set_error("moments: scratch too small"); return -1; }
   unsigned* ticket = (unsigned*)scratch;
   double* part = (double*)((char*)scratch + moments_ticket_bytes(groups_max));
-  hipLaunchKernelGGL(moments_kernel, dim3(gx, groups), dim3(256), 0, s, x, n, moments, part, ticket);
+  if (g_stats_batched) hipLaunchKernelGGL(moments_kernel<true>, dim3(gx, groups), dim3(256), 0, s, x, n, moments, part, ticket);
+  else hipLaunchKernelGGL(moments_kernel<false>, dim3(gx, groups), dim3(256), 0, s, x, n, moments, part, ticket);
   SVT_LAUNCH_CHECK();
   return 0;
 }
@@ -122,22 +135,75 @@
 }
 
 namespace {
+template <int N, int BIT>
+__device__ __forceinline__ void wave_sum_halve(const double (&in)[N], double (&out)[(N + 1) / 2], bool up) {
+  constexpr int H = (N + 1) / 2;
+#pragma unroll
+  for (int k = 0; k < H; ++k) {
+    const double lo = in[k], hi = k + H < N ? in[k + H] : 0.0;
+    out[k] = (up ? hi : lo) + __shfl_xor(up ? lo : hi, BIT, 64);
+  }
+}
+template <int ST>
 __global__ __launch_bounds__(256) void conv0_window_moments_kernel(const float* wav, int64_t L, int stride, int64_t T1,
                                                                    double* wm, double* part, unsigned* ticket) {
   __shared__ double sh[4][NWM];
+  constexpr int WPT = 8;
+  constexpr int SPAN = WPT * (ST > 0 ? ST : 1);
+  constexpr int NS = (256 * WPT - 1) * ST + K0;
+  __shared__ float xs[ST > 0 ? NS + NS / SPAN + 1 : 1];
   const int b = blockIdx.y;
   const float* x = wav + (int64_t)b * L;
   double acc[NWM];
 #pragma unroll
   for (int i = 0; i < NWM; ++i) acc[i] = 0.0;
-  constexpr int WPT = 8;
   const int64_t t0 = ((int64_t)blockIdx.x * blockDim.x + threadIdx.x) * WPT;
+  if constexpr (ST > 0) {
+    const int64_t w0 = (int64_t)blockIdx.x * (256 * WPT);
+    const int nwin = (int)(T1 - w0 < 256 * WPT ? T1 - w0 : 256 * WPT);
+    const int ns = (nwin - 1) * ST + K0;
+    const float* xb = x + w0 * ST;
+    if (((uintptr_t)xb & 15) == 0) {
+      constexpr int NV = (NS / 4 + 255) / 256;
+      const int n4 = ns >> 2;
+      float4 v[NV];
+#pragma unroll
+      for (int j = 0; j < NV; ++j) {
+        const int i = (int)threadIdx.x + 256 * j;
+        v[j] = i < n4 ? ((const float4*)xb)[i] : float4{0.f, 0.f, 0.f, 0.f};
+      }
+#pragma unroll
+      for (int j = 0; j < NV; ++j) {
+        const int i = 4 * ((int)threadIdx.x + 256 * j);
+        if (i < 4 * n4) {
+          xs[i + i / SPAN] = v[j].x; xs[i + 1 + (i + 1) / SPAN] = v[j].y;
+          xs[i + 2 + (i + 2) / SPAN] = v[j].z; xs[i + 3 + (i + 3) / SPAN] = v[j].w;
+        }
+      }
+      for (int i = 4 * n4 + (int)threadIdx.x; i < ns; i += 256) xs[i + i / SPAN] = xb[i];
+    } else {
+      for (int i0 = 0; i0 < ns; i0 += 256 * 8) {
+        float v[8];
+#pragma unroll
+        for (int j = 0; j < 8; ++j) { const int i = i0 + 256 * j + (int)threadIdx.x; v[j] = i < ns ? xb[i] : 0.f; }
+#pragma unroll
+        for (int j = 0; j < 8; ++j) { const int i = i0 + 256 * j + (int)threadIdx.x; if (i < ns) xs[i + i / SPAN] = v[j]; }
+      }
+    }
+    __syncthreads();
+  }
   for (int w = 0; w < WPT; ++w) {
     const int64_t t = t0 + w;
     if (t >= T1) break;
     float v[K0];
+    if constexpr (ST > 0) {
+      const int base = ((int)threadIdx.x * WPT + w) * ST;
+#pragma unroll
+      for (int j = 0; j < K0; ++j) v[j] = xs[base + j + (base + j) / SPAN];
+    } else {
 #pragma unroll
     for (int j = 0; j < K0; ++j) v[j] = x[t * stride + j];
+    }
     int idx = K0;
 #pragma unroll
     for (int j = 0; j < K0; ++j) {
@@ -147,10 +213,30 @@
     }
   }
   const int lane = threadIdx.x & 63, wave = threadIdx.x >> 6;
+  if constexpr (ST > 0) {
+    static_assert(NWM == 65, "half sizes below");
+    double a33[33], a17[17], a9[9], a5[5], a3[3], a2[2];
+    wave_sum_halve<65, 32>(acc, a33, lane & 32);
+    wave_sum_halve<33, 16>(a33, a17, lane & 16);
+    wave_sum_halve<17, 8>(a17, a9, lane & 8);
+    wave_sum_halve<9, 4>(a9, a5, lane & 4);
+    wave_sum_halve<5, 2>(a5, a3, lane & 2);
+    wave_sum_halve<3, 1>(a3, a2, lane & 1);
+    int off = 0, nv = NWM;
+    constexpr int HS[6] = {33, 17, 9, 5, 3, 2};
+#pragma unroll
+    for (int l = 0; l < 6; ++l) {
+      if (lane & (32 >> l)) { off += HS[l]; nv -= HS[l]; }
+      else if (nv > HS[l]) nv = HS[l];
+    }
+    if (nv > 0) sh[wave][off] = a2[0];
+    if (nv > 1) sh[wave][off + 1] = a2[1];
+  } else {
 #pragma unroll
   for (int i = 0; i < NWM; ++i) {
     const double r = wave_sum(acc[i]);
     if (lane == 0) sh[wave][i] = r;
+  }
   }
   __syncthreads();
   part += (size_t)b * gridDim.x * NWM;
@@ -179,37 +265,10 @@
   if (wav_mom) wav_mom += 2 * (b / cpg);
   const int c = blockIdx.x * blockDim.x + threadIdx.x;
   if (c >= C) return;
-  double mu = 0.0, r = 1.0;
-  if (wav_mom) {
-    mu = wav_mom[0] / (double)n_wav;
-    const double var = wav_mom[1] / (double)n_wav - mu * mu;
-    r = 1.0 / sqrt(var + (double)eps_wav);
-  }
-  const double* m = wm + b * NWM;
-  const double invT = 1.0 / (double)T1;
-  double w[K0], mn[K0];
-  double wsum = 0.0;
-  for (int j = 0; j < K0; ++j) { w[j] = (double)w0[c * K0 + j]; wsum += w[j]; mn[j] = r * (m[j] * invT - mu); }
-  const double bias = b0 ? (double)b0[c] : 0.0;
-  double dot = 0.0;
-  for (int j = 0; j < K0; ++j) dot += w[j] * mn[j];
-  double quad = 0.0;
-  int idx = K0;
-  for (int j = 0; j < K0; ++j)
-    for (int j2 = j; j2 < K0; ++j2) {
-      const double R = r * r * (m[idx] * invT - mu * m[j] * invT - mu * m[j2] * invT + mu * mu);
-      quad += (j == j2 ? 1.0 : 2.0) * w[j] * w[j2] * R;
-      ++idx;
-    }
-  const double mean = dot + bias;
-  const double e2 = quad + 2.0 * bias * dot + bias * bias;
-  double var = e2 - mean * mean;
-  if (var < 0.0) var = 0.0;
-  const double a = (double)gamma[c] / sqrt(var + (double)eps_gn);
-  const double shift = (double)beta[c] - mean * a;
-  float* o = coef + ((int64_t)b * C + c) * (K0 + 1);
-  for (int j = 0; j < K0; ++j) o[j] = (float)(a * r * w[j]);
-  o[K0] = (float)(a * (bias - r * mu * wsum) + shift);
+  float o[K0 + 1];
+  conv0_group_coef_one(wav_mom, n_wav, wm + b * NWM, T1, w0 + c * K0, b0, gamma, beta, c, eps_wav, eps_gn, o);
+  float* dst = coef + ((int64_t)b * C + c) * (K0 + 1);
+  for (int j = 0; j <= K0; ++j) dst[j] = o[j];
 }
 }
 size_t conv0_window_moments_scratch_bytes(int B, int64_t T1) {
@@ -225,7 +284,9 @@
   dim3 grid((unsigned)((T1 + per_block - 1) / per_block), B);
   unsigned* ticket = (unsigned*)scratch;
   double* part = (double*)((char*)scratch + moments_ticket_bytes(B));
-  hipLaunchKernelGGL(conv0_window_moments_kernel, grid, dim3(256), 0, s, wav, L, stride, T1, wm, part, ticket);
+  if (g_stats_batched && stride == 5 && !((uintptr_t)wav & 3))
+    hipLaunchKernelGGL(conv0_window_moments_kernel<5>, grid, dim3(256), 0, s, wav, L, stride, T1, wm, part, ticket);
+  else hipLaunchKernelGGL(conv0_window_moments_kernel<0>, grid, dim3(256), 0, s, wav, L, stride, T1, wm, part, ticket);
   SVT_LAUNCH_CHECK();
   return 0;
 }
@@ -358,6 +419,161 @@
   }
 }
 
+template <int KC> struct HeadStats {
+  int64_t cur_g = -1, g_end = 0;
+  float la = 0.f, lq = 0.f;
+  __device__ __forceinline__ void flush(int lane, int W, int NW, int64_t rows_per_group, double* slots, int slots_per_group) {
+    if (cur_g < 0) return;
+    const double sa = wave_sum((double)la), sq = wave_sum((double)lq);
+    if (lane == 0) {
+      const int64_t ja = (cur_g * rows_per_group) >> 2;
+      const int p = (int)(((W - ja) % NW + NW) % NW);
+      double* sl = slots + ((size_t)cur_g * slots_per_group + p) * 2;
+      st_partial(sl, sa);
+      st_partial(sl + 1, sq);
+    }
+    la = 0.f; lq = 0.f;
+  }
+  __device__ __forceinline__ void rows4(const float4 (&xv)[4][KC], int64_t r0, int64_t rows, int lane, int W, int NW, int64_t rows_per_group,
+                                        double* slots, int slots_per_group) {
+#pragma unroll
+    for (int rr = 0; rr < 4; ++rr) {
+      if (r0 + rr >= rows) break;
+      if (r0 + rr >= g_end || cur_g < 0) {
+        flush(lane, W, NW, rows_per_group, slots, slots_per_group);
+        cur_g = (r0 + rr) / rows_per_group;
+        g_end = (cur_g + 1) * rows_per_group;
+      }
+      float a = 0.f, q = 0.f;
+#pragma unroll
+      for (int c = 0; c < KC; ++c) {
+        const float4 v = xv[rr][c];
+        a += (v.x + v.y) + (v.z + v.w);
+        q += (v.x * v.x + v.y * v.y) + (v.z * v.z + v.w * v.w);
+      }
+      la += a;
+      lq += q;
+    }
+  }
+};
+template <int KC> __device__ __forceinline__ void head_load_rows4(const float* x, int64_t r0, int64_t rows, int lane, float4 (&xv)[4][KC]) {
+  constexpr int K = KC * 256;
+  const auto xrs = __builtin_amdgcn_make_buffer_rsrc((void*)x, 0, 0x7FFFFFF0, 0x00020000);
+#pragma unroll
+  for (int rr = 0; rr < 4; ++rr) {
+    const int64_t row = r0 + rr < rows ? r0 + rr : rows - 1;
+#pragma unroll
+    for (int c = 0; c < KC; ++c) {
+      typedef float f4v __attribute__((ext_vector_type(4)));
+      const f4v t = __builtin_bit_cast(f4v, __builtin_amdgcn_raw_buffer_load_b128(xrs, (unsigned)((row * K + c * 256 + lane * 4) * 4), 0, 0));
+      xv[rr][c] = float4{t[0], t[1], t[2], t[3]};
+    }
+  }
+}
+template <int KC> __device__ __forceinline__ float head_dot4(const float4 (&xv)[4][KC], const float* wn, int lane, bool hi32, bool hi16) {
+  float sacc[4] = {0.f, 0.f, 0.f, 0.f};
+#pragma unroll
+  for (int c = 0; c < KC; ++c) {
+    const float4 wv = *(const float4*)(wn + c * 256 + lane * 4);
+#pragma unroll
+    for (int rr = 0; rr < 4; ++rr) {
+      sacc[rr] = fmaf(xv[rr][c].x, wv.x, sacc[rr]);
+      sacc[rr] = fmaf(xv[rr][c].y, wv.y, sacc[rr]);
+      sacc[rr] = fmaf(xv[rr][c].z, wv.z, sacc[rr]);
+      sacc[rr] = fmaf(xv[rr][c].w, wv.w, sacc[rr]);
+    }
+  }
+  float k0 = hi32 ? sacc[2] : sacc[0], k1 = hi32 ? sacc[3] : sacc[1];
+  const float g0 = hi32 ? sacc[0] : sacc[2], g1 = hi32 ? sacc[1] : sacc[3];
+  k0 += __shfl_xor(g0, 32, 64);
+  k1 += __shfl_xor(g1, 32, 64);
+  float v = hi16 ? k1 : k0;
+  v += __shfl_xor(hi16 ? k0 : k1, 16, 64);
+#pragma unroll
+  for (int o = 8; o > 0; o >>= 1) v += __shfl_xor(v, o, 64);
+  return v;
+}
+__device__ __forceinline__ void head_sum_slots(int64_t rows, int64_t rows_per_group, int NW, const double* slots, int slots_per_group,
+                                               double* mom, int lane, int wave) {
+  const int64_t n_groups = (rows + rows_per_group - 1) / rows_per_group;
+  for (int64_t g = wave; g < n_groups; g += 4) {
+    const int64_t a = g * rows_per_group, b = (g + 1) * rows_per_group < rows ? (g + 1) * rows_per_group : rows;
+    const int64_t nj = ((b - 1) >> 2) - (a >> 2) + 1;
+    const int n = (int)(nj < NW ? nj : NW);
+    const double* sl = slots + (size_t)g * slots_per_group * 2;
+    double ta = 0.0, tq = 0.0;
+    double va[32], vq[32];
+#pragma unroll
+    for (int j = 0; j < 32; ++j)
+      if (lane + 64 * j < n) { va[j] = ld_partial(sl + 2 * (lane + 64 * j)); vq[j] = ld_partial(sl + 2 * (lane + 64 * j) + 1); }
+#pragma unroll
+    for (int j = 0; j < 32; ++j)
+      if (lane + 64 * j < n) { ta += va[j]; tq += vq[j]; }
+    ta = wave_sum(ta);
+    tq = wave_sum(tq);
+    if (lane == 0) { mom[2 * g] = ta; mom[2 * g + 1] = tq; }
+  }
+}
+
+template <int KC>
+__global__ __launch_bounds__(256) void head_dots_pipe_kernel(const float* __restrict__ x, int64_t rows, const float* __restrict__ w, int N,
+                                                             float* __restrict__ dots, double* __restrict__ mom, int64_t rows_per_group,
+                                                             double* __restrict__ slots, unsigned* __restrict__ ticket, int slots_per_group) {
+  constexpr int K = KC * 256;
+  extern __shared__ __attribute__((aligned(16))) float wl[];
+  const int lane = threadIdx.x & 63, wave = threadIdx.x >> 6;
+  const bool hi32 = (lane & 32) != 0, hi16 = (lane & 16) != 0;
+  const int myrow = (hi32 ? 2 : 0) + (hi16 ? 1 : 0);
+  const int NW = (int)gridDim.x * 4, W = (int)blockIdx.x * 4 + wave;
+  const int64_t step = (int64_t)gridDim.x * 16;
+  int64_t r0 = (int64_t)W * 4;
+  float4 xv[4][KC];
+  if (r0 < rows) head_load_rows4<KC>(x, r0, rows, lane, xv);
+  for (int i0 = threadIdx.x * 4; i0 < N * K; i0 += 8 * 1024) {
+    float4 t[8];
+#pragma unroll
+    for (int j = 0; j < 8; ++j) t[j] = i0 + j * 1024 < N * K ? *(const float4*)(w + i0 + j * 1024) : float4{0.f, 0.f, 0.f, 0.f};
+#pragma unroll
+    for (int j = 0; j < 8; ++j) if (i0 + j * 1024 < N * K) *(float4*)(wl + i0 + j * 1024) = t[j];
+  }
+  __syncthreads();
+  HeadStats<KC> st;
+  for (; r0 < rows; r0 += step) {
+    float4 xn[4][KC];
+    const bool more = r0 + step < rows;
+    if (more) head_load_rows4<KC>(x, r0 + step, rows, lane, xn);
+    if (mom) st.rows4(xv, r0, rows, lane, W, NW, rows_per_group, slots, slots_per_group);
+    float out0 = 0.f, out1 = 0.f;
+    for (int n0 = 0; n0 < N; n0 += 4) {
+      float v[4];
+#pragma unroll
+      for (int j = 0; j < 4; ++j) v[j] = head_dot4<KC>(xv, wl + (n0 + j < N ? n0 + j : N - 1) * K, lane, hi32, hi16);
+#pragma unroll
+      for (int j = 0; j < 4; ++j) {
+        const int n = n0 + j;
+        if (n < N && (lane & 15) == (n & 15)) { if (n < 16) out0 = v[j]; else out1 = v[j]; }
+      }
+    }
+    const int64_t row = r0 + myrow;
+    if (row < rows) {
+      const int n0 = lane & 15;
+      if (n0 < N) dots[row * N + n0] = out0;
+      if (n0 + 16 < N) dots[row * N + n0 + 16] = out1;
+    }
+    if (more) {
+#pragma unroll
+      for (int rr = 0; rr < 4; ++rr)
+#pragma unroll
+        for (int c = 0; c < KC; ++c) xv[rr][c] = xn[rr][c];
+    }
+  }
+  if (mom) {
+    st.flush(lane, W, NW, rows_per_group, slots, slots_per_group);
+    if (!last_workgroup(ticket, gridDim.x)) return;
+    head_sum_slots(rows, rows_per_group, NW, slots, slots_per_group, mom, lane, wave);
+  }
+}
+
 __global__ void head_finish_kernel(const float* __restrict__ dots, int64_t rows, int N, const float* __restrict__ wsum,
                                    const float* __restrict__ bias, const double* __restrict__ mom, int64_t rows_per_group,
                                    double group_elems, float eps, float* __restrict__ logits, FrameOut* __restrict__ frames,
@@ -415,18 +631,20 @@
   return 256 + ((size_t)rows / 4 + 2 * (size_t)groups_max + 8) * 2 * sizeof(double);
 }
 
-template <int KC>
+int g_head_dots_pipe = 1;
+template <int KC, bool PIPE>
 static int launch_head_dots_kc(const float* x, int64_t rows, const float* w, int N, float* dots, double* mom, int64_t rpg, void* scratch,
                                hipStream_t s) {
   const size_t lds = (size_t)N * KC * 256 * 4;
-  if (int r_ = ensure_dyn_lds((const void*)head_dots_kernel<KC>, 32 * KC * 256 * 4)) return r_;
+  if (int r_ = ensure_dyn_lds(PIPE ? (const void*)head_dots_pipe_kernel<KC> : (const void*)head_dots_kernel<KC>, 32 * KC * 256 * 4)) return r_;
   const unsigned grid = head_dots_grid(rows);
   if (mom && (!scratch || ((uintptr_t)scratch & 7))) { set_error("head_fused: scratch"); return -1; }
   if ((unsigned long)rows * KC * 256 * 4 > 0x7FFFFFF0ul) { set_error("head_fused: more than 2 GiB of encoder output (32-bit buffer offsets)"); return -1; }
   unsigned* ticket = (unsigned*)scratch;
   double* slots = scratch ? (double*)((char*)scratch + 256) : nullptr;
-  hipLaunchKernelGGL((head_dots_kernel<KC>), dim3(grid), dim3(256), lds, s, x, rows, w, N, dots, mom, rpg, slots, ticket,
-                     mom ? head_slots_per_group(rows, rpg) : 0);
+  const int spg = mom ? head_slots_per_group(rows, rpg) : 0;
+  if constexpr (PIPE) hipLaunchKernelGGL((head_dots_pipe_kernel<KC>), dim3(grid), dim3(256), lds, s, x, rows, w, N, dots, mom, rpg, slots, ticket, spg);
+  else hipLaunchKernelGGL((head_dots_kernel<KC>), dim3(grid), dim3(256), lds, s, x, rows, w, N, dots, mom, rpg, slots, ticket, spg);
   SVT_LAUNCH_CHECK();
   return 0;
 }
@@ -440,9 +658,13 @@
     const int64_t groups = (rows + rows_per_group - 1) / rows_per_group;
     if (256 + (size_t)groups * head_slots_per_group(rows, rows_per_group) * 16 > head_scratch_bytes(rows, (int)groups)) { set_error("head_fused: scratch too small"); return -1; }
   }
-  int r = K == 512 ? launch_head_dots_kc<2>(x, rows, w, N, dots, mom, rows_per_group, scratch, s)
-        : K == 768 ? launch_head_dots_kc<3>(x, rows, w, N, dots, mom, rows_per_group, scratch, s)
-                   : launch_head_dots_kc<4>(x, rows, w, N, dots, mom, rows_per_group, scratch, s);
+  auto dots_kc = [&](auto kc) {
+    constexpr int KC = decltype(kc)::value;
+    return g_head_dots_pipe ? launch_head_dots_kc<KC, true>(x, rows, w, N, dots, mom, rows_per_group, scratch, s)
+                            : launch_head_dots_kc<KC, false>(x, rows, w, N, dots, mom, rows_per_group, scratch, s);
+  };
+  int r = K == 512 ? dots_kc(std::integral_constant<int, 2>{}) : K == 768 ? dots_kc(std::integral_constant<int, 3>{})
+                                                                            : dots_kc(std::integral_constant<int, 4>{});
   if (r) return r;
   if (between) { if (int rb = between(between_arg)) return rb; }
   hipLaunchKernelGGL(head_finish_kernel, dim3((unsigned)((rows + 255) / 256)), dim3(256), 0, s, dots, rows, N, wsum, b, mom,
```

Measured after the change: 6192 clips/s (median of 3 runs). About the same (+0.2%).
